# tusen-ai/MV2D

Hardware: AMD Instinct MI355X
Metric: multi-view samples/sec (6-cam frames) through the MV2D RoI-head hot path (higher is better)
Workload: dtype f16x3: every operand an fp16 hi + lo pair, three MFMAs per product, fp32 accumulation (fp32-class, index-exact route; the lo halves of the key / value rows are STORED as e4m3 bytes); 1 GPU; cfg2_s: MV2D-S head, 6 views 1408x512; global_batch=384, streams_per_gpu=4, samples_per_launch=16, pe_sine_branch=folded into a per-(weights, geometry) table, FLOPs not counted, parallelism=dp1, hipgraph=True

## Files before the change

include/mv2d_hip.h:

```cpp
#ifndef MV2D_HIP_H
#define MV2D_HIP_H
#ifdef __cplusplus
extern "C" {
#endif

const char* mv2d_last_error(void);
int mv2d_abi_version(void);
int mv2d_key16_format(void);
int mv2d_f32_to_key16(const float* x, void* hi, void* lo, long long n, void* stream);
int mv2d_device_arch(char* buf, int buflen);
int mv2d_spin(int usec, void* stream);


int mv2d_gemm_bf16(const void* A, const void* A2, int n_split, int a_mode, const void* W, const float* bias, int M, int N,
                   int K, int lda, const int* m_dev, int act, const float* mul, int ldmul, const float* add, int ldadd,
                   void* C, int c_bf16, int ldc, long long c_blk_stride, int c_blk_cols, void* C2, const float* add2,
                   int ldc2, int ldadd2, void* stream);
int mv2d_gemm_bf16_ex(const void* A, const void* A2, int n_split, int a_mode, const void* W, const float* bias, int M, int N, int K, int lda,
                      const int* m_dev, int act, const float* mul, int ldmul, const float* add, int ldadd, void* C, int c_bf16, int ldc,
                      long long c_blk_stride, int c_blk_cols, void* C2, const float* add2, int ldc2, int ldadd2, int c_split3, const int* add_idx , int add_period,
                      int k_splits , long long c_split_stride, void* stream);
int mv2d_split3_rows(const float* a, const float* b, void* out, int M, int cols, const int* m_dev, void* stream);

int mv2d_gemm_f32(const float* A, const float* A2, int n_split, const float* W, const float* bias, int M, int N, int K,
                  int lda, int ldw, int split_k, int act, float scale, float clamp, void* C, int c_bf16, int ldc,
                  long long c_slice_stride, int groups, long long a_gs, long long w_gs, long long b_gs, long long c_gs,
                  void* stream);

int mv2d_attn_out_fused(const float* ctx, const float* resid, const float* Wo, const float* bo, const float* ln_w, const float* ln_b,
                        float* x_out, const float* qpos, const float* Wq, const float* bq, float qscale, float* q_out, int M, float eps,
                        void* stream);

int mv2d_pe_fused_tab(const void* A1, const void* Xfb, const float* Xf32, const int* row_index, const int* m_dev, int M,
                      const void* W1a, const float* b1a, const void* W1b, const float* b1b,
                      const void* Wr, const float* br, const void* We, const float* be,
                      const float* sine_tab, int tab_period, float* pe, void* Xk, void* stream);
int mv2d_pe_fused_tab2(const void* A1, const void* Xfb, const float* Xf32, const int* row_index, const int* m_dev, int M,
                       const void* W1a, const float* b1a, const void* W1b, const float* b1b,
                       const void* Wr, const float* br, const void* We, const float* be,
                       const float* sine_tab, int tab_period, float* pe, void* Xk, int shape, void* stream);

int mv2d_pe_fused_tab_fmt(const void* A1, const void* Xfb, const void* Xf32, const int* row_index, const int* m_dev, int M,
                          const void* W1a, const float* b1a, const void* W1b, const float* b1b,
                          const void* Wr, const float* br, const void* We, const float* be,
                          const float* sine_tab, int tab_period, float* pe, void* Xk, int shape, int map_fmt, void* stream);

int mv2d_pe_fused_x3(const float* A1, const float* Xmap, const int* row_index, const int* m_dev, int M,
                     const void* W1a_hi, const void* W1a_lo, const float* b1a, const void* W1b_hi, const void* W1b_lo, const float* b1b,
                     const void* Wr_hi, const void* Wr_lo, const float* br, const void* We_hi, const void* We_lo, const float* be,
                     const float* sine_tab, int tab_period, float* pe, void* Xk_hi, void* Xk_lo, void* Xv_hi, void* Xv_lo, int lo_fmt, int pe_at_index,
                     int* lo8_flag, void* stream);
int mv2d_pe_fused_x3_fmt(const float* A1, const void* Xmap, const int* row_index, const int* m_dev, int M,
                         const void* W1a_hi, const void* W1a_lo, const float* b1a, const void* W1b_hi, const void* W1b_lo, const float* b1b,
                         const void* Wr_hi, const void* Wr_lo, const float* br, const void* We_hi, const void* We_lo, const float* be,
                         const float* sine_tab, int tab_period, float* pe, void* Xk_hi, void* Xk_lo, void* Xv_hi, void* Xv_lo, int lo_fmt, int pe_at_index,
                         int* lo8_flag, int map_fmt, void* stream);
int mv2d_pe_fused_x3_k(const float* A1, const void* Xmap, const int* row_index, const int* m_dev, int M,
                       const void* W1a_hi, const void* W1a_lo, const float* b1a, const void* W1b_hi, const void* W1b_lo, const float* b1b,
                       const void* Wr_hi, const void* Wr_lo, const float* br, const void* We_hi, const void* We_lo, const float* be,
                       const float* sine_tab, int tab_period, float* pe, void* Xk_hi, void* Xk_lo, void* Xv_hi, void* Xv_lo, int lo_fmt, int pe_at_index,
                       int* lo8_flag, int map_fmt, int Kp, void* stream);
int mv2d_pe_fused_x3_ng(const float* A1, const void* Xmap, const int* row_index, const int* m_dev, int M,
                        const void* W1a_hi, const void* W1a_lo, const float* b1a, const void* W1b_hi, const void* W1b_lo, const float* b1b,
                        const float* sine_tab, int tab_period, float* pe, void* Xk_hi, void* Xk_lo, void* Xv_hi, void* Xv_lo,
                        int lo_fmt, int pe_at_index, int* lo8_flag, int map_fmt, int Kp, void* stream);
int mv2d_pe_gate_x3(const float* Q, const void* Xmap, const int* row_index, const int* m_dev, int M,
                    const void* Wr_hi, const void* Wr_lo, const float* br, const void* We_hi, const void* We_lo, const float* be,
                    const float* sine_tab, int tab_period, float* pe, void* Xk_hi, void* Xk_lo, void* Xv_hi, void* Xv_lo, int pe_at_index,
                    int map_fmt, void* stream);
int mv2d_pe_gate_rows_x3(const float* Q, const void* Xmap, const int* row_index, const int* m_dev, int M,
                         const void* Wr_hi, const void* Wr_lo, const float* br, const void* We_hi, const void* We_lo, const float* be,
                         const float* sine_tab, int tab_period, float* pe, void* Xk_hi, void* Xk_lo, void* Xv_hi, void* Xv_lo, int lo_fmt,
                         int* lo8_flag, int map_fmt, const unsigned* view_mask, int hw, int take_set, void* stream);
int mv2d_pe_fused_x3_k_sel(const float* A1, const void* Xmap, const int* row_index, const int* m_dev, int M,
                           const void* W1a_hi, const void* W1a_lo, const float* b1a, const void* W1b_hi, const void* W1b_lo, const float* b1b,
                           const void* Wr_hi, const void* Wr_lo, const float* br, const void* We_hi, const void* We_lo, const float* be,
                           const float* sine_tab, int tab_period, float* pe, void* Xk_hi, void* Xk_lo, void* Xv_hi, void* Xv_lo, int lo_fmt,
                           int* lo8_flag, int map_fmt, int Kp, const unsigned* view_mask, int hw, int take_set, void* stream);
int mv2d_pe_fused_x3b(const float* A1, const float* Xmap, const int* row_index, const int* m_dev, int M,
                     const void* W1a_hi, const void* W1a_lo, const float* b1a, const void* W1b_hi, const void* W1b_lo, const float* b1b,
                     const void* Wr_hi, const void* Wr_lo, const float* br, const void* We_hi, const void* We_lo, const float* be,
                     const float* sine_tab, int tab_period, float* pe, void* Xk_hi, void* Xk_lo, void* Xv_hi, void* Xv_lo, int lo_fmt, int pe_at_index,
                     int* lo8_flag, void* stream);

int mv2d_pack_wfrag_bf16(const void* W, void* Wp, int N, int K, void* stream);
int mv2d_qg_conv_pool(const void* roi_feat, const void* W, const float* bias, float* out, int ld_out, int R, void* stream);
int mv2d_qg_conv_pool_x3(const void* roi_feat_hi, const void* roi_feat_lo, const void* W_hi, const void* W_lo, const float* bias, float* out,
                         int ld_out, int R, void* stream);
int mv2d_qg_conv_pool_s(const void* roi_feat, const void* W, const float* bias, float* out, int ld_out, int R, int roi_size, void* stream);
int mv2d_qg_conv_pool_x3_s(const void* roi_feat_hi, const void* roi_feat_lo, const void* W_hi, const void* W_lo, const float* bias, float* out,
                           int ld_out, int R, int roi_size, void* stream);

int mv2d_qg_conv_cells(const void* roi_feat, const void* W, const float* bias, void* out_hi, void* out_lo, float* out_f32, int R, int roi_size,
                       void* stream);
int mv2d_qg_conv_cells_x3(const void* roi_feat_hi, const void* roi_feat_lo, const void* W_hi, const void* W_lo, const float* bias, void* out_hi,
                          void* out_lo, float* out_f32, int R, int roi_size, void* stream);
int mv2d_avgpool_cells(const void* hi, const void* lo, float* out, int ld_out, int R, int cells, void* stream);

int mv2d_attn_out_fused_x3(const float* ctx, const float* resid, const void* Wo_hi, const void* Wo_lo, const float* bo,
                           const float* ln_w, const float* ln_b, float* x_out, const float* qpos, const void* Wq_hi,
                           const void* Wq_lo, const float* bq, float qscale, float* q_out, int M, float eps, void* stream);

int mv2d_sa_block_fused_x3(const float* qkv, const float* resid, const void* Wo_hi, const void* Wo_lo, const float* bo,
                           const float* ln_w, const float* ln_b, float* x_out, const float* qpos, const void* Wq_hi,
                           const void* Wq_lo, const float* bq, float qscale, float* q_out, int M, float eps, void* stream);

int mv2d_query_embed_fused_x3(const float* enc2, const float* Wc, const float* bc, const float* minv, const float* dim_t,
                              const float* pc_range, const void* W0_hi, const void* W0_lo, const float* b0, const void* W2_hi,
                              const void* W2_lo, const float* b2, float* center, float* xyz, float* ref, float* posemb,
                              float* qpos, int R, void* stream);

int mv2d_qg_tail_x3(const float* x2, const float* enc, int ld_enc, const void* fc_hi, const void* fc_lo, const float* fc_b,
                    const void* e0_hi, const void* e0_lo, const float* e0_b, const void* e2_hi, const void* e2_lo, const float* e2_b,
                    const float* Wc, const float* bc, const float* minv, const float* dim_t, const float* pc_range, const void* W0_hi,
                    const void* W0_lo, const float* b0, const void* W2_hi, const void* W2_lo, const float* b2, float* center, float* xyz,
                    float* ref, float* posemb, float* qpos, int R, void* stream);

int mv2d_ffn_out_fused_x3(const float* parts, int n_parts, long long part_stride, const float* b2, const float* resid,
                          const float* ln_w, const float* ln_b, const float* post_w, const float* post_b, float* x_out,
                          const float* qpos, float* xq_out, float* outs, const void* Win_hi, const void* Win_lo,
                          const float* b_in, float* qkv, int M, float eps, void* stream);

int mv2d_pack_wfrag_f32(const float* W, float* Wp, int N, int K, int ldw, void* stream);
int mv2d_heads_fused(const float* outs, const float* const* cls_w, const float* const* reg_w, const float* ref, float* cls, float* reg,
                     int M, int L, float eps, const float* pc_range, float dt, const float* dt_rows , void* stream);

int mv2d_linear_x3(const float* A, const float* A2, int n_split, int lda, const void* Whi, const void* Wlo, const float* bias,
                   float* C, int ldc, int M, int N, int K, int act, float clamp, int groups, long long a_gs, long long w_gs,
                   long long b_gs, long long c_gs, void* stream);
int mv2d_linear_x3_ex(const float* A, const float* A2, int n_split, int lda, const void* Whi, const void* Wlo, const float* bias,
                      float* C, int ldc, int M, int N, int K, int act, float clamp, int groups, long long a_gs, long long w_gs,
                      long long b_gs, long long c_gs, const int* m_dev, int conv3x3, const float* mul, const float* add, int ld_ma,
                      void* stream);
int mv2d_split_rows_key16(const float* a, const float* b, void* hi, void* lo, int M, int cols, const int* m_dev, void* stream);

int mv2d_heads_fused_x3(const float* outs, const void* const* cls_w, const void* const* reg_w, const float* ref, float* cls, float* reg,
                        int M, int L, float eps, const float* pc_range, float dt, const float* dt_rows, void* stream);
int mv2d_heads_fused_x3_nc(const float* outs, const void* const* cls_w, const void* const* reg_w, const float* ref, float* cls, float* reg,
                           int M, int L, int num_classes, float eps, const float* pc_range, float dt, const float* dt_rows, void* stream);
int mv2d_heads_cls_x3_nc(const float* outs, const void* const* cls_w, float* cls, int M, int L, int num_classes, float eps, void* stream);
int mv2d_reg_layer_x3(const float* outs, const void* const* w, const float* ref, float* reg, int M, int L, int n_groups, const int* group_dims,
                      const float* pc_range, float dt, const float* dt_rows, void* stream);

int mv2d_heads_depth_x3(const float* outs, const void* const* cls_w, const void* const* reg_w, const float* ref, float* cls, float* reg,
                        int M, int L, int n_fcs, int num_classes, float eps, const float* pc_range, float dt, const float* dt_rows, void* stream);
int mv2d_heads_cls_depth_x3(const float* outs, const void* const* cls_w, float* cls, int M, int L, int n_fcs, int num_classes, float eps,
                            void* stream);
int mv2d_reg_layer_depth_x3(const float* outs, const void* const* w, const float* ref, float* reg, int M, int L, int n_fcs, int n_groups,
                            const int* group_dims, const float* pc_range, float dt, const float* dt_rows, void* stream);

int mv2d_ffn_pack_weights(const float* W1, const float* W2, float* W1p, float* W2p, int hidden, void* stream);
int mv2d_ffn_fused(const float* X, const float* W1, const float* b1, const float* W2, float* slabs, int M, int hidden, void* stream);

int mv2d_ffn_fused_x3(const float* X, const void* W1hi, const void* W1lo, const float* b1, const void* W2hi, const void* W2lo,
                      float* slabs, int M, int hidden, int slices_per_block, void* stream);

int mv2d_split_bf16x2(const float* x, void* hi, void* lo, long long n, void* stream);
int mv2d_q16_format(void);
int mv2d_split_q16x2(const float* x, void* hi, void* lo, long long n, void* stream);


int mv2d_row_ln(const float* parts, int n_parts, long long part_stride, const float* bias, const float* residual,
                const float* ln_w, const float* ln_b, int relu, float* out, const float* addvec, float* out_plus,
                const float* ln2_w, const float* ln2_b, float* out2, int M, float eps, int rows_per_group, void* stream);

int mv2d_finalize_reg(float* reg, const float* ref, int L, int R, const float* pc_range, float dt, void* stream);

int mv2d_avgpool49(const float* x, float* out, int ld_out, int R, void* stream);

int mv2d_f32_to_bf16(const float* x, void* y, long long n, void* stream);

int mv2d_nchw_to_nhwc(const float* x, float* y, int V, int C, int HW, void* stream);
int mv2d_nchw_to_nhwc_masked(const float* x, float* y, const unsigned char* mask, int V, int C, int HW, void* stream);
int mv2d_nchw_to_nhwc_fmt(const void* x, void* y, int V, int C, int HW, int map_fmt, void* stream);
int mv2d_nchw_to_nhwc_masked_fmt(const void* x, void* y, const unsigned char* mask, int V, int C, int HW, int map_fmt, void* stream);

int mv2d_nchw_to_nhwc_bf16(const float* x, void* y, int V, int C, int HW, void* stream);
int mv2d_map_conv3x3(const void* in, const void* Wp, const float* bias, float* out, int V, int h, int w, void* stream);



int mv2d_self_attn_fwd(const float* qkv, float* ctx, int R, const int* grp_start, int n_samples, void* stream);

int mv2d_self_attn_x3_fwd(const float* qkv, float* ctx, int R, const int* grp_start, int n_samples, int max_grp_rows, int dn_pad,
                          int dn_single, void* stream);

int mv2d_self_attn_dn_fwd(const float* qkv, float* ctx, int R, int dn_pad, int dn_single, void* stream);

int mv2d_sparse_xattn_fwd(const float* q, const void* K, const void* V, const int* row_ptr, const int* col_idx, float* ctx,
                          float* dbg_logits, long long dbg_stride, int R, int empty_nan, void* stream);

int mv2d_xattn_qmap(const float* q, const void* WA_hi, const void* WA_lo, void* Qt, int R, void* stream);
int mv2d_xattn_tile_fwd(const void* Qt, const void* Xk, const void* Xv, const void* Xk_lo, const void* Xv_lo, const int* row_ptr,
                        const int* col_idx, float* z, float* dbg_logits, long long dbg_stride, int R, int empty_nan, int waves, void* stream);
int mv2d_xattn_tile_fwd_ordered(const void* Qt, const void* Xk, const void* Xv, const void* Xk_lo, const void* Xv_lo, const int* row_ptr,
                                const int* col_idx, float* z, float* dbg_logits, long long dbg_stride, int R, int empty_nan, int waves,
                                const int* order, int lo_fmt, void* stream);
int mv2d_xattn_fused_fwd(const float* q, const void* WA_hi, const void* WA_lo, const void* WB_hi, const void* WB_lo, const float* bv, const void* Xk,
                         const void* Xv, const void* Xk_lo, const void* Xv_lo, const int* row_ptr, const int* col_idx, float* ctx, int R, int empty_nan,
                         const int* order, int lo_fmt, void* stream);
int mv2d_xattn_fused_fwd_p(const float* q, const void* WA_hi, const void* WA_lo, const void* WB_hi, const void* WB_lo, const float* bv, const void* Xk,
                           const void* Xv, const void* Xk_lo, const void* Xv_lo, const int* row_ptr, const int* col_idx, float* ctx, int R, int empty_nan,
                           const int* order, int lo_fmt, int deal, void* stream);
int mv2d_xattn_group_max(int R, int n_samples);
int mv2d_xattn_group_tables(const int* row_ptr, const int* col_idx, const int* order, const int* grp_start, int n_samples, int R, int ng_max, int* g_slot,
                            int* g_cnt, int* g_ptr, int* g_len, int* ucol, unsigned char* umask, int ucap, int* u_total, int* flags, void* stream);
int mv2d_xattn_group_fwd(const float* q, const void* WA_hi, const void* WA_lo, const void* WB_hi, const void* WB_lo, const float* bv, const void* Xk,
                         const void* Xv, const void* Xk_lo, const void* Xv_lo, const int* row_ptr, const int* order, const int* g_slot, const int* g_cnt,
                         const int* g_ptr, const int* g_len, const int* ucol, const unsigned char* umask, float* ctx, int ng_max, int empty_nan,
                         void* stream);
int mv2d_xattn_ctxmap(const float* z, const void* WB_hi, const void* WB_lo, const float* bv, const int* row_ptr, float* ctx, int R,
                      int empty_nan, void* stream);

int mv2d_xattn_query_order(const int* row_ptr, const int* col_idx, const int* grp_start, int n_samples, int R, int* perm, int* flags, int stride,
                           void* stream);
int mv2d_attn_out_qmap_x3(const float* ctx, const float* resid, const void* Wo_hi, const void* Wo_lo, const float* bo, const float* ln_w,
                          const float* ln_b, float* x_out, const float* qpos, const void* Wq_hi, const void* Wq_lo, const float* bq,
                          float qscale, const void* WA_hi, const void* WA_lo, void* Qt, int M, float eps, void* stream);
int mv2d_attn_out_zmap_x3(const float* z, const void* WB_hi, const void* WB_lo, const float* bv, const int* row_ptr, int empty_nan,
                          const float* resid, const void* Wo_hi, const void* Wo_lo, const float* bo, const float* ln_w, const float* ln_b,
                          float* x_out, int M, float eps, void* stream);

int mv2d_sparse_xattn_bwd(const float* q, const void* K, const void* V, const int* row_ptr, const int* col_idx, const float* ctx,
                          const float* dctx, const int* key_ptr, const int* pair_idx, const int* pair_row, float* pair_ws,
                          float* dq, float* dK, float* dV, int R, int S, void* stream);
int mv2d_sparse_xattn_fwd_drop(const float* q, const void* K, const void* V, const int* row_ptr, const int* col_idx, float* ctx, float* dbg_logits,
                               long long dbg_stride, int R, int empty_nan, float p_drop, unsigned int seed, void* stream);
int mv2d_sparse_xattn_bwd_drop(const float* q, const void* K, const void* V, const int* row_ptr, const int* col_idx, const float* ctx,
                               const float* dctx, const int* key_ptr, const int* pair_idx, const int* pair_row, float* pair_ws, float* dq, float* dK,
                               float* dV, int R, int S, float p_drop, unsigned int seed, void* stream);
int mv2d_sparse_xattn_bwd_ex(const float* q, const void* K, const void* V, const int* row_ptr, const int* col_idx, const float* ctx, const float* dctx,
                             const int* key_ptr, const int* pair_idx, const int* pair_row, float* pair_ws, float* dq, float* dK, float* dV, int R,
                             int S, float p_drop, unsigned int seed, int long_rows, float dq_scale, void* stream);


int mv2d_box_params(const float* rois, const double* viewK, const double* viewE, double* K_roi, float* intr, int ld_intr,
                    float* minv, int R, float roi_size, float intr_scale, float min_size, void* stream);

int mv2d_refpoint_posemb(const float* center_pred, int ld_cp, const float* minv, const float* dim_t, float* xyz, float* ref,
                         float* posemb, int R, const float* pc_range, void* stream);

int mv2d_lidar2img_inverse(const double* K_roi, const double* E, float* minv, int R, void* stream);

int mv2d_posemb3d(const float* ref, const float* dim_t, float* posemb, int R, void* stream);

int mv2d_roi_align(const float* map0, const float* map1, const float* rois, void* out0, void* out1, float* out0_f32,
                   float* out1_f32, int R, int H, int W, int channels, float spatial_scale, int sampling_ratio,
                   const int* map1_index, int out1_is_sum, void* stream);
int mv2d_roi_align_ex(const float* map0, const float* map1, const float* rois, void* out0, void* out1, float* out0_f32, float* out1_f32,
                      int R, int H, int W, int channels, float spatial_scale, int sampling_ratio, const int* map1_index, int out1_is_sum,
                      void* out0_lo, void* out1_lo, void* out0_lo8, void* out1_lo8, int* lo8_flag, void* stream);
int mv2d_roi_align_s(const float* map0, const float* map1, const float* rois, void* out0, void* out1, float* out0_f32, float* out1_f32,
                     int R, int H, int W, int channels, float spatial_scale, int sampling_ratio, const int* map1_index, int out1_is_sum,
                     void* out0_lo, void* out1_lo, void* out0_lo8, void* out1_lo8, int* lo8_flag, int roi_size, void* stream);
int mv2d_roi_align_fmt(const void* map0, const float* map1, const float* rois, void* out0, void* out1, float* out0_f32, float* out1_f32,
                       int R, int H, int W, int channels, float spatial_scale, int sampling_ratio, const int* map1_index, int out1_is_sum,
                       void* out0_lo, void* out1_lo, void* out0_lo8, void* out1_lo8, int* lo8_flag, int roi_size, int map_fmt, void* stream);

int mv2d_box_correlation(const float* rois, const int* view_start, const double* trans, const float* lin, const float* depths,
                         int* match, int R, int V, int sample_size, int num_depth, int topk, int pad_h, int pad_w,
                         float depth_start, float iou_thr, float ratio, int max_per_view, void* stream);
int mv2d_frame_geometry(const float* rois, const double* viewK, const double* viewE, double* K_roi, float* intr, int ld_intr, float* minv,
                        float roi_size, float intr_scale, float min_size, const int* view_start, const double* trans, const float* lin,
                        const float* depths, int* match, int R, int V, int sample_size, int num_depth, int topk, int pad_h, int pad_w,
                        float depth_start, float iou_thr, float ratio, int max_per_view, void* zero_ptr, long long zero_bytes, void* stream);
int mv2d_box_correlation_ex(const float* rois, const int* view_start, const double* trans, const float* lin, const float* depths,
                            int* match, int R, int V, int sample_size, int num_depth, int topk, int pad_h, int pad_w,
                            double depth_start, float iou_thr, float ratio, int max_per_view, void* stream);
int mv2d_frame_geometry_ex(const float* rois, const double* viewK, const double* viewE, double* K_roi, float* intr, int ld_intr, float* minv,
                           float roi_size, float intr_scale, float min_size, const int* view_start, const double* trans, const float* lin,
                           const float* depths, int* match, int R, int V, int sample_size, int num_depth, int topk, int pad_h, int pad_w,
                           double depth_start, float iou_thr, float ratio, int max_per_view, void* zero_ptr, long long zero_bytes, void* stream);

long long mv2d_csr_workspace_bytes(int R, int V, int h, int w);

int mv2d_mask_compact(const float* rois, const int* match, const unsigned char* pad_mask, unsigned char* roi_mask, int* rect,
                      int* pos2s, int* s2pos, int* S_out, unsigned int* bits_ws, int* row_count, int* row_ptr, int* col_idx,
                      int* nnz_out, int col_cap, int R, int V, int h, int w, int topk, float stride, float expand_stride,
                      int n_samples , void* stream);

int mv2d_roi_positions(const float* rois, const unsigned char* pad_mask, unsigned char* roi_mask, int* rect, int* pos2s,
                       int* s2pos, int* S_out, int R, int V, int h, int w, float stride, float expand_stride, void* stream);

int mv2d_csr_from_corr(const int* match, int* row_ptr, int* col_idx, int* nnz_out, int R, int V, int topk, void* stream);
int mv2d_roi_positions_csr(const float* rois, const unsigned char* pad_mask, unsigned char* roi_mask, int* rect, int* pos2s, int* s2pos,
                           int* S_out, int R, int V, int h, int w, float stride, float expand_stride, const int* match, int* row_ptr,
                           int* col_idx, int* nnz_out, int Vg, int topk, const int* grp_start, int n_samples, int* order, int* order_flags, void* stream);
int mv2d_csr_from_corr_s(const int* match, int* row_ptr, int* col_idx, int* nnz_out, int R, int V, int topk, int roi_size, void* stream);
int mv2d_roi_positions_csr_s(const float* rois, const unsigned char* pad_mask, unsigned char* roi_mask, int* rect, int* pos2s, int* s2pos,
                             int* S_out, int R, int V, int h, int w, float stride, float expand_stride, const int* match, int* row_ptr,
                             int* col_idx, int* nnz_out, int Vg, int topk, const int* grp_start, int n_samples, int* order, int* order_flags,
                             int roi_size, void* stream);

int mv2d_pe_frustum_f32(const int* s2pos, const int* S_dev, int S_max, const double* img2lidar, const double* coords_w, const double* coords_h,
                        const double* coords_d, float* out, int V, int h, int w, int depth_num, const double* position_range, void* stream);
int mv2d_pe_frustum_f32_ld(const int* s2pos, const int* S_dev, int S_max, const double* img2lidar, const double* coords_w, const double* coords_h,
                           const double* coords_d, float* out, int V, int h, int w, int depth_num, const double* position_range, int ld, void* stream);
int mv2d_pe_frustum_f32_sel(const int* s2pos, const int* S_dev, int S_max, const double* img2lidar, const double* coords_w, const double* coords_h,
                            const double* coords_d, float* out, int V, int h, int w, int depth_num, const double* position_range, int ld,
                            const unsigned* view_mask, int tab_period, void* stream);

int mv2d_pe_inputs(const int* s2pos, const int* S_dev, int S_max, const float* featcl, const double* img2lidar,
                   const double* coords_w, const double* coords_h, const double* coords_d, const float* embeds,
                   const float* dim_t, void* A_frustum, void* A_sine, void* Xf_k16, float* Xf_f32, float* A_frustum_f32,
                   float* A_sine_f32, int V, int h, int w, int depth_num, const double* position_range, void* stream);
int mv2d_pe_inputs_fmt(const int* s2pos, const int* S_dev, int S_max, const void* featcl, const double* img2lidar,
                       const double* coords_w, const double* coords_h, const double* coords_d, const float* embeds,
                       const float* dim_t, void* A_frustum, void* A_sine, void* Xf_k16, float* Xf_f32, float* A_frustum_f32,
                       float* A_sine_f32, int V, int h, int w, int depth_num, const double* position_range, int map_fmt, void* stream);
int mv2d_pe_inputs_ld(const int* s2pos, const int* S_dev, int S_max, const void* featcl, const double* img2lidar,
                      const double* coords_w, const double* coords_h, const double* coords_d, const float* embeds,
                      const float* dim_t, void* A_frustum, void* A_sine, void* Xf_k16, float* Xf_f32, float* A_frustum_f32,
                      float* A_sine_f32, int V, int h, int w, int depth_num, const double* position_range, int map_fmt, int ld, void* stream);

int mv2d_decode_topk(const float* cls, const float* reg, int R, int num_classes, int max_num, const float* post_center_range,
                     float* boxes, float* scores, long long* labels, long long* bbox_index, int* count_out,
                     long long* topk_index_dbg, const int* grp_start, int n_samples, int max_grp_rows, float* payload, void* stream);

int mv2d_nms_bev(const float* boxes, const float* scores, const long long* labels, const int* count, float nms_thr, float* scores_out,
                 int n_samples, int in_stride, void* stream);

int mv2d_result_pack(const float* boxes, const float* scores, const long long* labels, const int* count, float score_thr, int max_num,
                     float* out_boxes, float* out_scores, long long* out_labels, int* out_count,
                     int n_samples , int in_stride,
                     void* stream);

int mv2d_pack_detections(const float* boxes, const float* scores, const long long* labels, const int* count, float* out, int n_samples,
                         int max_num, int in_stride, void* stream);

int mv2d_match_cost(const float* cls, const float* box, const float* gt, const int* gt_labels, float* cost, int n_layers, int R, int G,
                    int C, float cls_weight, float reg_weight, float alpha, float gamma, void* stream);

int mv2d_set_loss(const float* cls, const float* box, const int* match, const float* gt, const int* gt_labels, const float* code_weights,
                  const float* layer_weights, float* loss, float* dcls, float* dbox, int n_layers, int R, int G, int C,
                  float cls_avg_factor, float box_avg_factor, float alpha, float gamma, float loss_cls_weight, float loss_bbox_weight,
                  int skip_background_boxes, void* stream);

int mv2d_dn_queries(const float* gt, const int* gt_labels, const float* rnd, int G, int scalar, float noise_scale, float noise_trans, float split,
                    int num_classes, const float* pc_range_host, float eps, float* ref, long long* labels, float* boxes, void* stream);

int mv2d_colsum_scratch_rows(int rows);
int mv2d_colsum(const float* x, long long ld, int rows, int cols, float* out, float* scratch, void* stream);
int mv2d_layer_norm_bwd_blocks(int M);
int mv2d_layer_norm_bwd(const float* x, const float* dy, const float* w, float* dx, float* dw_part, float* db_part, float* dw, float* db, int M,
                        float eps, void* stream);
long long mv2d_gemm_f32x3_ws_bytes(int M, int N, int K);
int mv2d_gemm_f32x3(const float* A, long long lda, int trans_a, const float* B, long long ldb, int trans_b, const float* bias, int act, float* C,
                    long long ldc, int M, int N, int K, void* ws, long long ws_bytes, void* stream);
long long mv2d_linear_bwd_x3_ws_bytes(int M, int N, int K);
int mv2d_linear_bwd_x3(const float* x, const float* W, const float* y, const float* dy, float* dx, float* dW, float* db, int M, int N, int K, void* ws,
                       long long ws_bytes, void* stream);

int mv2d_gemm_f32x3_ex(const float* A, long long lda, int trans_a, const float* B, long long ldb, int trans_b, const float* bias, int act, float alpha,
                       int accumulate, int out_bf16, void* C, long long ldc, int M, int N, int K, void* ws, long long ws_bytes, void* stream);
int mv2d_colsum_add(const float* x, long long ld, int rows, int cols, float* out, float* scratch, const float* add, void* stream);
int mv2d_softmax_bwd_rows(const float* P, const float* Pd, float* dP, long long ld, int rows, int cols, float keep_scale, void* stream);
long long mv2d_gemm_f32x3_batched_ws_bytes(int M, int N, int K, int batch);
int mv2d_gemm_f32x3_batched(const float* A, long long lda, long long batch_a, int trans_a, const float* B, long long ldb, long long batch_b, int trans_b,
                            float* C, long long ldc, long long batch_c, int M, int N, int K, int batch, float alpha, void* ws, long long ws_bytes,
                            void* stream);
int mv2d_dgrad_relu_f32x3(const float* g, const float* W, const float* relu_y, float alpha, float* dx, int M, int N, int K, void* stream);
int mv2d_wgrad_f32x3(const float* g, const float* x, float* dW, float* db, int M, int N, int K, void* ws, long long ws_bytes, float* cs_scratch,
                     void* stream);

typedef struct mv2d_td_dims {
    int T, S, L, F;
    int sa_nnz, ca_nnz;
    float p_sa_attn, p_sa_out, p_ca_attn, p_ca_out, p_ffn_act, p_ffn_out;
    unsigned int seed;
    float eps;
    int pad, nk;
} mv2d_td_dims;
long long mv2d_train_decoder_act_bytes(const mv2d_td_dims* d);
long long mv2d_train_decoder_ws_bytes(const mv2d_td_dims* d, int backward);
int mv2d_train_decoder_fwd(const mv2d_td_dims* d, const float* const* params, const float* qpos, const float* key_in, const float* val_in,
                           const int* sa_row_ptr, const int* sa_col, const int* ca_row_ptr, const int* ca_col, const int* dn_keys, float* outs, void* act,
                           void* ws, void* stream);
int mv2d_train_decoder_bwd(const mv2d_td_dims* d, const float* const* params, float* const* grads, const float* qpos, const float* key_in,
                           const float* val_in, const int* sa_row_ptr, const int* sa_col, const int* sa_key_ptr, const int* sa_pair_idx,
                           const int* sa_pair_row, const int* ca_row_ptr, const int* ca_col, const int* ca_key_ptr, const int* ca_pair_idx,
                           const int* ca_pair_row, const int* dn_keys, const float* d_outs, const void* act, void* ws, float* d_qpos, float* d_key_in,
                           float* d_val_in, void* stream);

typedef struct mv2d_th_dims { int T, L, NC; float eps; } mv2d_th_dims;
long long mv2d_train_heads_act_bytes(const mv2d_th_dims* d);
long long mv2d_train_heads_ws_bytes(const mv2d_th_dims* d, int backward);
int mv2d_train_heads_fwd(const mv2d_th_dims* d, const float* const* params, const float* outs, float* cls, float* reg, void* act, void* ws,
                         void* stream);
int mv2d_train_heads_bwd(const mv2d_th_dims* d, const float* const* params, float* const* grads, const float* outs, const float* d_cls,
                         const float* d_reg, const void* act, void* ws, float* d_outs, void* stream);

int mv2d_box_code_fwd(const float* t, const float* ref, float* out, int L, int T, int pad, float dt, const float* pc_range, void* stream);
int mv2d_box_code_bwd(const float* g, const float* out, const float* ref, float* d_t, float* d_ref, int L, int T, int pad, float dt,
                      const float* pc_range, void* stream);

int mv2d_lsap_layers(const float* cost, int L, int R, int G, int* match, int threads);

int mv2d_im2col3x3(const float* x, float* cols, int R, void* stream);
int mv2d_col2im3x3(const float* dcols, float* dx, int R, void* stream);
int mv2d_im2col3x3_s(const float* x, float* cols, int R, int roi_size, void* stream);
int mv2d_col2im3x3_s(const float* dcols, float* dx, int R, int roi_size, void* stream);

int mv2d_center2lidar_fwd(const float* c, const float* minv, float* ref, int R, const float* pc_range, void* stream);
int mv2d_center2lidar_bwd(const float* g, const float* c, const float* minv, float* dc, int R, const float* pc_range, void* stream);

long long mv2d_dense_attn_ws_bytes(int n, int nk, int backward);
int mv2d_dense_attn_fwd(const float* q, const float* k, const float* v, int n, int nk, float p_drop, unsigned int seed, float* ctx, float* lse, void* ws,
                        void* stream);
int mv2d_dense_attn_bwd(const float* q, const float* k, const float* v, const float* ctx, const float* dctx, const float* lse, int n, int nk, float p_drop,
                        unsigned int seed, float dq_scale, float* dq, float* dk, float* dv, void* ws, void* stream);
int mv2d_dense_attn_bwd_parts(const float* q, const float* k, const float* v, const float* ctx, const float* dctx, const float* lse, int n, int nk,
                              float p_drop, unsigned int seed, float dq_scale, float* dq, float* dk, float* dv, void* ws, int parts, void* stream);

int mv2d_roi_align_bwd(const float* grad_out, const float* rois, float* grad_map, const int* index, int R, int H, int W, int channels,
                       float spatial_scale, int sampling_ratio, void* stream);
int mv2d_roi_align_bwd_s(const float* grad_out, const float* rois, float* grad_map, const int* index, int R, int H, int W, int channels,
                         float spatial_scale, int sampling_ratio, int roi_size, void* stream);

#ifdef __cplusplus
}
#endif
#endif
```

mv2d_amd/_lib.py:

```python
import ctypes as C
import os

HERE = os.path.dirname(os.path.abspath(__file__))
LIB_PATH = os.path.join(HERE, 'lib', 'libmv2d_hip.so')


class Mv2dHipError(RuntimeError):
    pass


P, I, LL, F, D = C.c_void_p, C.c_int, C.c_longlong, C.c_float, C.c_double
ABI_VERSION = 6

class TdDims(C.Structure):
    _fields_ = [('T', I), ('S', I), ('L', I), ('F', I), ('sa_nnz', I), ('ca_nnz', I), ('p_sa_attn', F), ('p_sa_out', F), ('p_ca_attn', F),
                ('p_ca_out', F), ('p_ffn_act', F), ('p_ffn_out', F), ('seed', C.c_uint), ('eps', F), ('pad', I), ('nk', I)]


class ThDims(C.Structure):
    _fields_ = [('T', I), ('L', I), ('NC', I), ('eps', F)]


SIGNATURES = {
    'mv2d_last_error': (C.c_char_p, []),
    'mv2d_abi_version': (I, []),
    'mv2d_device_arch': (I, [C.c_char_p, I]),
    'mv2d_spin': (I, [I, P]),
    'mv2d_gemm_bf16': (I, [P, P, I, I, P, P, I, I, I, I, P, I, P, I, P, I, P, I, I, LL, I, P, P, I, I, P]),
    'mv2d_gemm_bf16_ex': (I, [P, P, I, I, P, P, I, I, I, I, P, I, P, I, P, I, P, I, I, LL, I, P, P, I, I, I, P, I, I, LL, P]),
    'mv2d_split3_rows': (I, [P, P, P, I, I, P, P]),
    'mv2d_pe_fused_tab': (I, [P, P, P, P, P, I] + [P] * 9 + [I, P, P, P]),
    'mv2d_pe_fused_tab2': (I, [P, P, P, P, P, I] + [P] * 9 + [I, P, P, I, P]),
    'mv2d_pe_fused_x3': (I, [P, P, P, P, I] + [P] * 13 + [I] + [P] * 5 + [I, I, P, P]),
    'mv2d_pe_fused_tab_fmt': (I, [P, P, P, P, P, I] + [P] * 9 + [I, P, P, I, I, P]),
    'mv2d_pe_fused_x3_fmt': (I, [P, P, P, P, I] + [P] * 13 + [I] + [P] * 5 + [I, I, P, I, P]),
    'mv2d_pe_fused_x3_k': (I, [P, P, P, P, I] + [P] * 13 + [I] + [P] * 5 + [I, I, P, I, I, P]),
    'mv2d_pe_fused_x3_ng': (I, [P, P, P, P, I] + [P] * 7 + [I] + [P] * 5 + [I, I, P, I, I, P]),
    'mv2d_pe_gate_x3': (I, [P, P, P, P, I] + [P] * 7 + [I] + [P] * 5 + [I, I, P]),
    'mv2d_pe_gate_rows_x3': (I, [P, P, P, P, I] + [P] * 7 + [I] + [P] * 5 + [I, P, I, P, I, I, P]),
    'mv2d_pe_fused_x3_k_sel': (I, [P, P, P, P, I] + [P] * 13 + [I] + [P] * 5 + [I, P, I, I, P, I, I, P]),
    'mv2d_pe_fused_x3b': (I, [P, P, P, P, I] + [P] * 13 + [I] + [P] * 5 + [I, I, P, P]),
    'mv2d_key16_format': (I, []),
    'mv2d_f32_to_key16': (I, [P, P, P, LL, P]),
    'mv2d_split_rows_key16': (I, [P, P, P, P, I, I, P, P]),
    'mv2d_qg_conv_pool': (I, [P, P, P, P, I, I, P]),
    'mv2d_qg_conv_pool_x3': (I, [P, P, P, P, P, P, I, I, P]),
    'mv2d_qg_conv_pool_s': (I, [P, P, P, P, I, I, I, P]),
    'mv2d_qg_conv_pool_x3_s': (I, [P, P, P, P, P, P, I, I, I, P]),
    'mv2d_qg_conv_cells': (I, [P, P, P, P, P, P, I, I, P]),
    'mv2d_qg_conv_cells_x3': (I, [P, P, P, P, P, P, P, P, I, I, P]),
    'mv2d_avgpool_cells': (I, [P, P, P, I, I, I, P]),
    'mv2d_pack_wfrag_bf16': (I, [P, P, I, I, P]),
    'mv2d_gemm_f32': (I, [P, P, I, P, P, I, I, I, I, I, I, I, F, F, P, I, I, LL, I, LL, LL, LL, LL, P]),
    'mv2d_attn_out_fused': (I, [P, P, P, P, P, P, P, P, P, P, F, P, I, F, P]),
    'mv2d_sa_block_fused_x3': (I, [P, P, P, P, P, P, P, P, P, P, P, P, F, P, I, F, P]),
    'mv2d_query_embed_fused_x3': (I, [P] * 17 + [I, P]),
    'mv2d_qg_tail_x3': (I, [P, P, I] + [P] * 25 + [I, P]),
    'mv2d_ffn_out_fused_x3': (I, [P, I, LL, P, P, P, P, P, P, P, P, P, P, P, P, P, P, I, F, P]),
    'mv2d_attn_out_fused_x3': (I, [P, P, P, P, P, P, P, P, P, P, P, P, F, P, I, F, P]),
    'mv2d_pack_wfrag_f32': (I, [P, P, I, I, I, P]),
    'mv2d_heads_fused': (I, [P, P, P, P, P, P, I, I, F, P, F, P, P]),
    'mv2d_linear_x3': (I, [P, P, I, I, P, P, P, P, I, I, I, I, I, F, I, LL, LL, LL, LL, P]),
    'mv2d_linear_x3_ex': (I, [P, P, I, I, P, P, P, P, I, I, I, I, I, F, I, LL, LL, LL, LL, P, I, P, P, I, P]),
    'mv2d_heads_fused_x3': (I, [P, P, P, P, P, P, I, I, F, P, F, P, P]),
    'mv2d_heads_fused_x3_nc': (I, [P, P, P, P, P, P, I, I, I, F, P, F, P, P]),
    'mv2d_heads_cls_x3_nc': (I, [P, P, P, I, I, I, F, P]),
    'mv2d_reg_layer_x3': (I, [P, P, P, P, I, I, I, P, P, F, P, P]),
    'mv2d_heads_depth_x3': (I, [P, P, P, P, P, P, I, I, I, I, F, P, F, P, P]),
    'mv2d_heads_cls_depth_x3': (I, [P, P, P, I, I, I, I, F, P]),
    'mv2d_reg_layer_depth_x3': (I, [P, P, P, P, I, I, I, I, P, P, F, P, P]),
    'mv2d_ffn_fused': (I, [P, P, P, P, P, I, I, P]),
    'mv2d_ffn_pack_weights': (I, [P, P, P, P, I, P]),
    'mv2d_ffn_fused_x3': (I, [P, P, P, P, P, P, P, I, I, I, P]),
    'mv2d_split_bf16x2': (I, [P, P, P, LL, P]),
    'mv2d_split_q16x2': (I, [P, P, P, LL, P]),
    'mv2d_q16_format': (I, []),
    'mv2d_row_ln': (I, [P, I, LL, P, P, P, P, I, P, P, P, P, P, P, I, F, I, P]),
    'mv2d_finalize_reg': (I, [P, P, I, I, P, F, P]),
    'mv2d_avgpool49': (I, [P, P, I, I, P]),
    'mv2d_f32_to_bf16': (I, [P, P, LL, P]),
    'mv2d_nchw_to_nhwc': (I, [P, P, I, I, I, P]),
    'mv2d_nchw_to_nhwc_masked': (I, [P, P, P, I, I, I, P]),
    'mv2d_nchw_to_nhwc_fmt': (I, [P, P, I, I, I, I, P]),
    'mv2d_nchw_to_nhwc_masked_fmt': (I, [P, P, P, I, I, I, I, P]),
    'mv2d_nchw_to_nhwc_bf16': (I, [P, P, I, I, I, P]),
    'mv2d_map_conv3x3': (I, [P, P, P, P, I, I, I, P]),
    'mv2d_self_attn_fwd': (I, [P, P, I, P, I, P]),
    'mv2d_self_attn_dn_fwd': (I, [P, P, I, I, I, P]),
    'mv2d_self_attn_x3_fwd': (I, [P, P, I, P, I, I, I, I, P]),
    'mv2d_dn_queries': (I, [P, P, P, I, I, F, F, F, I, P, F, P, P, P, P]),
    'mv2d_sparse_xattn_fwd': (I, [P, P, P, P, P, P, P, LL, I, I, P]),
    'mv2d_sparse_xattn_bwd': (I, [P] * 14 + [I, I, P]),
    'mv2d_sparse_xattn_fwd_drop': (I, [P, P, P, P, P, P, P, LL, I, I, F, C.c_uint, P]),
    'mv2d_sparse_xattn_bwd_drop': (I, [P] * 14 + [I, I, F, C.c_uint, P]),
    'mv2d_sparse_xattn_bwd_ex': (I, [P] * 14 + [I, I, F, C.c_uint, I, F, P]),
    'mv2d_dgrad_relu_f32x3': (I, [P, P, P, F, P, I, I, I, P]),
    'mv2d_xattn_qmap': (I, [P, P, P, P, I, P]),
    'mv2d_attn_out_qmap_x3': (I, [P] * 12 + [F, P, P, P, I, F, P]),
    'mv2d_attn_out_zmap_x3': (I, [P, P, P, P, P, I, P, P, P, P, P, P, P, I, F, P]),
    'mv2d_xattn_tile_fwd': (I, [P, P, P, P, P, P, P, P, P, LL, I, I, I, P]),
    'mv2d_xattn_tile_fwd_ordered': (I, [P, P, P, P, P, P, P, P, P, LL, I, I, I, P, I, P]),
    'mv2d_xattn_fused_fwd': (I, [P, P, P, P, P, P, P, P, P, P, P, P, P, I, I, P, I, P]),
    'mv2d_xattn_fused_fwd_p': (I, [P, P, P, P, P, P, P, P, P, P, P, P, P, I, I, P, I, I, P]),
    'mv2d_xattn_group_max': (I, [I, I]),
    'mv2d_xattn_group_tables': (I, [P, P, P, P, I, I, I, P, P, P, P, P, P, I, P, P, P]),
    'mv2d_xattn_group_fwd': (I, [P] * 19 + [I, I, P]),
    'mv2d_xattn_query_order': (I, [P, P, P, I, I, P, P, I, P]),
    'mv2d_xattn_ctxmap': (I, [P, P, P, P, P, P, I, I, P]),
    'mv2d_box_params': (I, [P, P, P, P, P, I, P, I, F, F, F, P]),
    'mv2d_refpoint_posemb': (I, [P, I, P, P, P, P, P, I, P, P]),
    'mv2d_lidar2img_inverse': (I, [P, P, P, I, P]),
    'mv2d_posemb3d': (I, [P, P, P, I, P]),
    'mv2d_roi_align': (I, [P, P, P, P, P, P, P, I, I, I, I, F, I, P, I, P]),
    'mv2d_roi_align_ex': (I, [P, P, P, P, P, P, P, I, I, I, I, F, I, P, I, P, P, P, P, P, P]),
    'mv2d_roi_align_s': (I, [P, P, P, P, P, P, P, I, I, I, I, F, I, P, I, P, P, P, P, P, I, P]),
    'mv2d_roi_align_fmt': (I, [P, P, P, P, P, P, P, I, I, I, I, F, I, P, I, P, P, P, P, P, I, I, P]),
    'mv2d_box_correlation': (I, [P, P, P, P, P, P, I, I, I, I, I, I, I, F, F, F, I, P]),
    'mv2d_box_correlation_ex': (I, [P, P, P, P, P, P, I, I, I, I, I, I, I, D, F, F, I, P]),
    'mv2d_csr_workspace_bytes': (LL, [I, I, I, I]),
    'mv2d_mask_compact': (I, [P, P, P, P, P, P, P, P, P, P, P, P, P, I, I, I, I, I, I, F, F, I, P]),
    'mv2d_roi_positions': (I, [P, P, P, P, P, P, P, I, I, I, I, F, F, P]),
    'mv2d_csr_from_corr': (I, [P, P, P, P, I, I, I, P]),
    'mv2d_csr_from_corr_s': (I, [P, P, P, P, I, I, I, I, P]),
    'mv2d_roi_positions_csr': (I, [P, P, P, P, P, P, P, I, I, I, I, F, F, P, P, P, P, I, I, P, I, P, P, P]),
    'mv2d_roi_positions_csr_s': (I, [P, P, P, P, P, P, P, I, I, I, I, F, F, P, P, P, P, I, I, P, I, P, P, I, P]),
    'mv2d_frame_geometry': (I, [P, P, P, P, P, I, P, F, F, F, P, P, P, P, P, I, I, I, I, I, I, I, F, F, F, I, P, LL, P]),
    'mv2d_frame_geometry_ex': (I, [P, P, P, P, P, I, P, F, F, F, P, P, P, P, P, I, I, I, I, I, I, I, D, F, F, I, P, LL, P]),
    'mv2d_pe_inputs': (I, [P, P, I, P, P, P, P, P, P, P, P, P, P, P, P, P, I, I, I, I, P, P]),
    'mv2d_pe_inputs_fmt': (I, [P, P, I, P, P, P, P, P, P, P, P, P, P, P, P, P, I, I, I, I, P, I, P]),
    'mv2d_pe_frustum_f32': (I, [P, P, I, P, P, P, P, P, I, I, I, I, P, P]),
    'mv2d_pe_frustum_f32_ld': (I, [P, P, I, P, P, P, P, P, I, I, I, I, P, I, P]),
    'mv2d_pe_frustum_f32_sel': (I, [P, P, I, P, P, P, P, P, I, I, I, I, P, I, P, I, P]),
    'mv2d_pe_inputs_ld': (I, [P, P, I, P, P, P, P, P, P, P, P, P, P, P, P, P, I, I, I, I, P, I, I, P]),
    'mv2d_result_pack': (I, [P, P, P, P, F, I, P, P, P, P, I, I, P]),
    'mv2d_nms_bev': (I, [P, P, P, P, F, P, I, I, P]),
    'mv2d_pack_detections': (I, [P, P, P, P, P, I, I, I, P]),
    'mv2d_roi_align_bwd': (I, [P, P, P, P, I, I, I, I, F, I, P]),
    'mv2d_roi_align_bwd_s': (I, [P, P, P, P, I, I, I, I, F, I, I, P]),
    'mv2d_colsum_scratch_rows': (I, [I]),
    'mv2d_colsum': (I, [P, LL, I, I, P, P, P]),
    'mv2d_gemm_f32x3_ws_bytes': (LL, [I, I, I]),
    'mv2d_gemm_f32x3': (I, [P, LL, I, P, LL, I, P, I, P, LL, I, I, I, P, LL, P]),
    'mv2d_gemm_f32x3_ex': (I, [P, LL, I, P, LL, I, P, I, F, I, I, P, LL, I, I, I, P, LL, P]),
    'mv2d_colsum_add': (I, [P, LL, I, I, P, P, P, P]),
    'mv2d_softmax_bwd_rows': (I, [P, P, P, LL, I, I, F, P]),
    'mv2d_gemm_f32x3_batched_ws_bytes': (LL, [I, I, I, I]),
    'mv2d_gemm_f32x3_batched': (I, [P, LL, LL, I, P, LL, LL, I, P, LL, LL, I, I, I, I, F, P, LL, P]),
    'mv2d_wgrad_f32x3': (I, [P, P, P, P, I, I, I, P, LL, P, P]),
    'mv2d_train_decoder_act_bytes': (LL, [P]),
    'mv2d_train_decoder_ws_bytes': (LL, [P, I]),
    'mv2d_train_decoder_fwd': (I, [P] * 14),
    'mv2d_train_decoder_bwd': (I, [P] * 24),
    'mv2d_box_code_fwd': (I, [P, P, P, I, I, I, F, P, P]),
    'mv2d_box_code_bwd': (I, [P, P, P, P, P, I, I, I, F, P, P]),
    'mv2d_im2col3x3': (I, [P, P, I, P]),
    'mv2d_col2im3x3': (I, [P, P, I, P]),
    'mv2d_im2col3x3_s': (I, [P, P, I, I, P]),
    'mv2d_col2im3x3_s': (I, [P, P, I, I, P]),
    'mv2d_center2lidar_fwd': (I, [P, P, P, I, P, P]),
    'mv2d_center2lidar_bwd': (I, [P, P, P, P, I, P, P]),
    'mv2d_dense_attn_ws_bytes': (LL, [I, I, I]),
    'mv2d_dense_attn_fwd': (I, [P, P, P, I, I, F, C.c_uint, P, P, P, P]),
    'mv2d_dense_attn_bwd': (I, [P, P, P, P, P, P, I, I, F, C.c_uint, F, P, P, P, P, P]),
    'mv2d_dense_attn_bwd_parts': (I, [P, P, P, P, P, P, I, I, F, C.c_uint, F, P, P, P, P, I, P]),
    'mv2d_lsap_layers': (I, [P, I, I, I, P, I]),
    'mv2d_train_heads_act_bytes': (LL, [P]),
    'mv2d_train_heads_ws_bytes': (LL, [P, I]),
    'mv2d_train_heads_fwd': (I, [P] * 8),
    'mv2d_train_heads_bwd': (I, [P] * 10),
    'mv2d_linear_bwd_x3_ws_bytes': (LL, [I, I, I]),
    'mv2d_linear_bwd_x3': (I, [P, P, P, P, P, P, P, I, I, I, P, LL, P]),
    'mv2d_layer_norm_bwd_blocks': (I, [I]),
    'mv2d_layer_norm_bwd': (I, [P, P, P, P, P, P, P, P, I, F, P]),
    'mv2d_match_cost': (I, [P, P, P, P, P, I, I, I, I, F, F, F, F, P]),
    'mv2d_set_loss': (I, [P, P, P, P, P, P, P, P, P, P, I, I, I, I, F, F, F, F, F, F, I, P]),
    'mv2d_decode_topk': (I, [P, P, I, I, I, P, P, P, P, P, P, P, P, I, I, P, P]),
}

_lib = None


def load(path=None):
    global _lib
    if _lib is not None:
        return _lib
    path = path or os.environ.get('MV2D_HIP_LIB', LIB_PATH)
    if not os.path.exists(path):
        raise Mv2dHipError(
            f'{path} not found: the MV2D HIP extension is not built.  Run `python -m mv2d_amd.build` '
            '(or __graft_entry__.build()).  There is no CPU/PyTorch fallback for the product path.')
    lib = C.CDLL(path)
    for name, (res, args) in SIGNATURES.items():
        fn = getattr(lib, name, None)
        if fn is None:
            raise Mv2dHipError(f'{path} does not export {name}; rebuild with `python -m mv2d_amd.build --force`')
        fn.restype = res
        fn.argtypes = args
    if lib.mv2d_abi_version() != ABI_VERSION:
        raise Mv2dHipError(f'{path} implements ABI version {lib.mv2d_abi_version()}, this package needs {ABI_VERSION}: rebuild with `python -m mv2d_amd.build --force`')
    _lib = lib
    return lib


def check(rc, what):
    if rc != 0:
        msg = load().mv2d_last_error()
        raise Mv2dHipError(f'{what} failed (rc={rc}): {msg.decode() if msg else ""}')
```

mv2d_amd/csrc/xattn_fused.hip:

```cpp
#include "xattn_walk.h"
#include <stdlib.h>
#ifndef MV2D_XF_QB_DEFAULT
#define MV2D_XF_QB_DEFAULT 8
#endif
enum { XF_DEAL_ROUNDS = 1, XF_DEAL_FULL = 2 };
#ifndef MV2D_XF_DEAL_DEFAULT
#define MV2D_XF_DEAL_DEFAULT XF_DEAL_FULL
#endif
constexpr int XF_DEAL_DEFAULT = MV2D_XF_DEAL_DEFAULT;

#ifdef MV2D_XF_TRACE
__device__ long long g_xf_trace[32];
#define XF_STAMP(i) do { if (blockIdx.x == MV2D_XF_TRACE && threadIdx.x == 0) g_xf_trace[i] = (long long)__builtin_amdgcn_s_memtime(); } while (0)
#else
#define XF_STAMP(i) do {} while (0)
#endif

namespace {

constexpr int WAVE_LDS = 16384;

template <int XLO, int QB>
__global__ __launch_bounds__(64 * QB, 2) void xattn_fused_kernel(const float* __restrict__ q, const uint4* __restrict__ WA_hi, const uint4* __restrict__ WA_lo,
                                                                const uint4* __restrict__ WB_hi, const uint4* __restrict__ WB_lo, const float* __restrict__ bv,
                                                                const unsigned short* __restrict__ Xk, const unsigned short* __restrict__ Xv,
                                                                const unsigned short* __restrict__ Xk_lo, const unsigned short* __restrict__ Xv_lo,
                                                                const int* __restrict__ row_ptr, const int* __restrict__ col_idx, float* __restrict__ ctx,
                                                                int R, int empty_nan, const int* __restrict__ order, int nblk) {
    constexpr int SMEM = QB * WAVE_LDS + QB * 512 + QB * HEADS * 4 + 3 * QB * 4;
    __shared__ __attribute__((aligned(16))) unsigned char smem[SMEM];
    const int tid = threadIdx.x, lane = tid & 63, wave = tid >> 6, n = lane & 15, g = lane >> 4;
    float* lsum = reinterpret_cast<float*>(smem + QB * WAVE_LDS + QB * 512);
    int* rq = reinterpret_cast<int*>(smem + QB * WAVE_LDS + QB * 512 + QB * HEADS * 4);
    int* rbeg = rq + QB;
    int* rend = rq + 2 * QB;
    const int blk = xcd_chunked(blockIdx.x, nblk);
    const int slot0 = (int)((long long)blk * R / nblk), nq = (int)((long long)(blk + 1) * R / nblk) - slot0;
    if (nq <= 0) return;
    XF_STAMP(0);
    if (tid < QB) {
        const int s = slot0 + min(tid, nq - 1);
        const int r_ = order ? order[s] : s;
        rq[tid] = r_;
        rbeg[tid] = row_ptr[r_];
        rend[tid] = row_ptr[r_ + 1];
    }
    __syncthreads();
    XF_STAMP(1);
    const int beg = rbeg[wave], end = rend[wave];
    const int ntile = wave < nq ? (end - beg + 15) >> 4 : 0;
    int idx_next = ntile > 0 ? col_idx[min(beg + n, end - 1)] : 0;
    typedef XattnWalk<XLO, false> Walk;
    Walk walk(Xk, Xv, Xk_lo, Xv_lo, lane, beg, end, reinterpret_cast<uint4*>(smem + wave * WAVE_LDS), reinterpret_cast<uint4*>(smem + wave * WAVE_LDS) + 512,
           reinterpret_cast<float*>(smem + QB * WAVE_LDS) + wave * 128);
    typename Walk::KRows k0;
    for (int h = wave; h < HEADS; h += QB) {
        const int r = rq[n & (QB - 1)];
        const float* qp = q + (long long)r * C + 32 * h + 8 * g;
        const float4 q0 = *reinterpret_cast<const float4*>(qp), q1 = *reinterpret_cast<const float4*>(qp + 4);
        const uint4* wh = WA_hi + (long long)h * 16 * 64 + lane;
        const uint4* wl = WA_lo + (long long)h * 16 * 64 + lane;
        uint4* qt = reinterpret_cast<uint4*>(smem + (n & (QB - 1)) * WAVE_LDS) + h * 64;
        u32x4 wa_h[16], wa_l[16];
#pragma unroll
        for (int t = 0; t < 16; ++t) {
            wa_h[t] = *reinterpret_cast<const u32x4*>(wh + t * 64);
            wa_l[t] = *reinterpret_cast<const u32x4*>(wl + t * 64);
        }
        __builtin_amdgcn_sched_barrier(0);
        XF_STAMP(20);
        Frag bh, bl;
        split8(q0, q1, bh, bl);
#pragma unroll
        for (int u = 0; u < 8; ++u) {
            if (u == 1) XF_STAMP(21);
            if (u == 4) XF_STAMP(22);
            f32x4_t a[2];
#pragma unroll
            for (int k = 0; k < 2; ++k) {
                f32x4_t c = {0.f, 0.f, 0.f, 0.f};
                c = mfma_q16_16x16x32(wa_l[2 * u + k], bh.v, c);
                c = mfma_q16_16x16x32(wa_h[2 * u + k], bl.v, c);
                c = mfma_q16_16x16x32(wa_h[2 * u + k], bh.v, c);
                a[k] = c;
            }
            Frag hi, lo;
            split8_k16(make_float4(a[0][0], a[0][1], a[0][2], a[0][3]), make_float4(a[1][0], a[1][1], a[1][2], a[1][3]), hi, lo);
            if (n < QB) {
                qt[u * 8 + g * 2] = hi.u;
                qt[u * 8 + g * 2 + 1] = lo.u;
            }
            if (u == (XLO ? 5 : 3) && h == wave && ntile > 0) walk.request_k(idx_next, k0);
        }
    }
    XF_STAMP(23);
    asm volatile("s_waitcnt lgkmcnt(0)" ::: "memory");
    __builtin_amdgcn_s_barrier();
    XF_STAMP(2);
    {
        const uint4* qp = reinterpret_cast<const uint4*>(smem + wave * WAVE_LDS) + (n & 7) * 64 + g * 2 + (n >> 3);
#pragma unroll
        for (int s = 0; s < 8; ++s) walk.qa[s].u = qp[s * 8];
    }
    walk.reset();
    if (ntile > 0) walk.stage_k(k0);
#pragma nounroll
    for (int tt = 0; tt < ntile; ++tt) {
        const int myidx = idx_next;
        if (tt + 1 < ntile) idx_next = col_idx[min(beg + 16 * (tt + 1) + n, end - 1)];
        typename Walk::VRows v;
        walk.gather(myidx, tt > 0, v);
        XF_STAMP(3 + 2 * min(tt, 5));
        walk.compute(tt, v);
        XF_STAMP(4 + 2 * min(tt, 5));
    }
    walk.row_sums();
    if (n == 0 && g < 2) {
#pragma unroll
        for (int i = 0; i < 4; ++i) lsum[wave * HEADS + 4 * g + i] = walk.l_run[i];
    }
    walk.store_z(reinterpret_cast<float*>(smem + wave * WAVE_LDS));
    XF_STAMP(15);
    __syncthreads();
    XF_STAMP(16);
    for (int h = wave; h < HEADS; h += QB) {
        const int j = n & (QB - 1);
        const float* zp = reinterpret_cast<const float*>(smem + j * WAVE_LDS) + h * C + 8 * g;
        const float rl = __builtin_amdgcn_rcpf(lsum[j * HEADS + h]);
        const uint4* wh = WB_hi + (long long)h * 16 * 64 + lane;
        const uint4* wl = WB_lo + (long long)h * 16 * 64 + lane;
        f32x4_t acc[2] = {{0.f, 0.f, 0.f, 0.f}, {0.f, 0.f, 0.f, 0.f}};
        u32x4 wb_h[16], wb_l[16];
#pragma unroll
        for (int t = 0; t < 16; ++t) {
            wb_h[t] = *reinterpret_cast<const u32x4*>(wh + t * 64);
            wb_l[t] = *reinterpret_cast<const u32x4*>(wl + t * 64);
        }
        int rr_[4], rp0_[4], rp1_[4];
#pragma unroll
        for (int i = 0; i < 4; ++i) {
            rr_[i] = rq[(4 * g + i) & (QB - 1)];
            rp0_[i] = rbeg[(4 * g + i) & (QB - 1)];
            rp1_[i] = rend[(4 * g + i) & (QB - 1)];
        }
        const float bv0 = bv[32 * h + n], bv1 = bv[32 * h + 16 + n];
        __builtin_amdgcn_sched_barrier(0);
#pragma unroll
        for (int s = 0; s < 8; ++s) {
            float4 x0 = *reinterpret_cast<const float4*>(zp + 32 * s);
            float4 x1 = *reinterpret_cast<const float4*>(zp + 32 * s + 4);
            x0 = make_float4(x0.x * rl, x0.y * rl, x0.z * rl, x0.w * rl);
            x1 = make_float4(x1.x * rl, x1.y * rl, x1.z * rl, x1.w * rl);
            Frag ah, al;
            split8(x0, x1, ah, al);
#pragma unroll
            for (int nt = 0; nt < 2; ++nt) {
                acc[nt] = mfma_q16_16x16x32(al.v, wb_h[s * 2 + nt], acc[nt]);
                acc[nt] = mfma_q16_16x16x32(ah.v, wb_l[s * 2 + nt], acc[nt]);
                acc[nt] = mfma_q16_16x16x32(ah.v, wb_h[s * 2 + nt], acc[nt]);
            }
        }
        if (4 * g < QB) {
#pragma unroll
            for (int i = 0; i < 4; ++i) {
                const int js = 4 * g + i;
                if (js < nq) {
                    const int rr = rr_[i];
                    const bool empty = rp1_[i] <= rp0_[i];
#pragma unroll
                    for (int nt = 0; nt < 2; ++nt) {
                        const int col = 32 * h + 16 * nt + n;
                        float v = acc[nt][i] + (nt ? bv1 : bv0);
                        if (empty) v = empty_nan ? __uint_as_float(0x7fc00000u) : 0.f;
                        ctx[(long long)rr * C + col] = v;
                    }
                }
            }
        }
    }
    XF_STAMP(17);
}

}

#ifdef MV2D_XF_TRACE
extern "C" int mv2d_xf_trace_read(long long* host, int n) { return hipMemcpyFromSymbol(host, HIP_SYMBOL(g_xf_trace), n * sizeof(long long)) == hipSuccess ? 0 : -2; }
#endif

extern "C" int mv2d_xattn_fused_fwd_p(const float* q, const void* WA_hi, const void* WA_lo, const void* WB_hi, const void* WB_lo, const float* bv,
                                      const void* Xk, const void* Xv, const void* Xk_lo, const void* Xv_lo, const int* row_ptr, const int* col_idx,
                                      float* ctx, int R, int empty_nan, const int* order, int lo_fmt, int deal, void* stream) {
    MV2D_CHECK_ARG(deal >= 0 && deal <= 2, "mv2d_xattn_fused_fwd_p: deal is 0 (default), 1 (whole rounds) or 2 (full blocks)");
    MV2D_CHECK_ARG(lo_fmt == 0 || (lo_fmt == 1 && Xk_lo), "mv2d_xattn_fused_fwd: lo_fmt is 0 (key16 lo rows) or 1 (e4m3 lo rows; needs the lo rows)");
    MV2D_CHECK_ARG(q && WA_hi && WA_lo && WB_hi && WB_lo && bv && Xk && Xv && row_ptr && col_idx && ctx && R >= 0, "mv2d_xattn_fused_fwd: bad args");
    MV2D_CHECK_ARG((Xk_lo == nullptr) == (Xv_lo == nullptr), "mv2d_xattn_fused_fwd: Xk_lo and Xv_lo come together");
    MV2D_CHECK_ARG(((uintptr_t)q & 15) == 0 && ((uintptr_t)WA_hi & 15) == 0 && ((uintptr_t)WA_lo & 15) == 0 && ((uintptr_t)WB_hi & 15) == 0 &&
                       ((uintptr_t)WB_lo & 15) == 0 && ((uintptr_t)Xk & 15) == 0 && ((uintptr_t)Xv & 15) == 0 && ((uintptr_t)Xk_lo & 15) == 0 &&
                       ((uintptr_t)Xv_lo & 15) == 0, "mv2d_xattn_fused_fwd: operands must be 16-byte aligned");
    if (R == 0) return MV2D_OK;
    static int n_cu = 0;
    if (n_cu == 0) {
        hipDeviceProp_t prop;
        int dev = 0;
        n_cu = (hipGetDevice(&dev) == hipSuccess && hipGetDeviceProperties(&prop, dev) == hipSuccess && prop.multiProcessorCount > 0) ? prop.multiProcessorCount : 256;
    }
    static const int qb_env = [] { const char* e = getenv("MV2D_XF_QB"); return e ? atoi(e) : 0; }();
    const int QB = qb_env == 4 || qb_env == 8 ? qb_env : MV2D_XF_QB_DEFAULT;
    const int slots = n_cu * (QB == 4 ? 2 : 1);
    int nblk = (R + QB - 1) / QB;
    if (nblk > slots) {
        static const int deal_env = [] { const char* e = getenv("MV2D_XF_DEAL"); return e ? atoi(e) : 0; }();
        const int policy = deal ? deal : (deal_env == XF_DEAL_ROUNDS || deal_env == XF_DEAL_FULL ? deal_env : XF_DEAL_DEFAULT);
        if (policy == XF_DEAL_ROUNDS) {
            const int up = (nblk + slots - 1) / slots * slots;
            if ((long long)up * (QB / 2) <= R) nblk = up;
        }
    } else {
        const int spread = R / 2 < n_cu ? R / 2 : n_cu;
        if (spread > nblk) nblk = spread;
    }
    const dim3 grid(nblk), block(64 * QB);
#define MV2D_XF(XLO_, QB_) hipLaunchKernelGGL((xattn_fused_kernel<XLO_, QB_>), grid, block, 0, (hipStream_t)stream, q, (const uint4*)WA_hi, (const uint4*)WA_lo, \
                                              (const uint4*)WB_hi, (const uint4*)WB_lo, bv, (const unsigned short*)Xk, (const unsigned short*)Xv,                     \
                                              (const unsigned short*)Xk_lo, (const unsigned short*)Xv_lo, row_ptr, col_idx, ctx, R, empty_nan, order, nblk)
    if (Xk_lo && lo_fmt == 1) { if (QB == 4) MV2D_XF(2, 4); else MV2D_XF(2, 8); }
    else if (Xk_lo) { if (QB == 4) MV2D_XF(1, 4); else MV2D_XF(1, 8); }
    else { if (QB == 4) MV2D_XF(0, 4); else MV2D_XF(0, 8); }
#undef MV2D_XF
    MV2D_LAUNCH_CHECK();
    return MV2D_OK;
}

extern "C" int mv2d_xattn_fused_fwd(const float* q, const void* WA_hi, const void* WA_lo, const void* WB_hi, const void* WB_lo, const float* bv,
                                    const void* Xk, const void* Xv, const void* Xk_lo, const void* Xv_lo, const int* row_ptr, const int* col_idx,
                                    float* ctx, int R, int empty_nan, const int* order, int lo_fmt, void* stream) {
    return mv2d_xattn_fused_fwd_p(q, WA_hi, WA_lo, WB_hi, WB_lo, bv, Xk, Xv, Xk_lo, Xv_lo, row_ptr, col_idx, ctx, R, empty_nan, order, lo_fmt, 0, stream);
}
```

mv2d_amd/csrc/xattn_walk.h:

```cpp
#pragma once
#include "common.h"
#include <type_traits>

namespace {

constexpr int C = 256, HEADS = 8;
constexpr float LOG2E = 1.4426950408889634f;

typedef q16x8_t q16x8;
union Frag { uint4 u; q16x8 v; };
typedef unsigned int u32x4 __attribute__((ext_vector_type(4)));
typedef unsigned int u32x2 __attribute__((ext_vector_type(2)));

__device__ __forceinline__ void split8(const float4& x0, const float4& x1, Frag& hi, Frag& lo) {
    const float f[8] = {x0.x, x0.y, x0.z, x0.w, x1.x, x1.y, x1.z, x1.w};
    unsigned int h[4], l[4];
#pragma unroll
    for (int i = 0; i < 4; ++i) split_q16x2(f[2 * i], f[2 * i + 1], h[i], l[i]);
    hi.u = make_uint4(h[0], h[1], h[2], h[3]);
    lo.u = make_uint4(l[0], l[1], l[2], l[3]);
}
__device__ __forceinline__ void split8_k16(const float4& x0, const float4& x1, Frag& hi, Frag& lo) {
    const float f[8] = {x0.x, x0.y, x0.z, x0.w, x1.x, x1.y, x1.z, x1.w};
    unsigned int h[4], l[4];
#pragma unroll
    for (int i = 0; i < 4; ++i) split_k16x2(f[2 * i], f[2 * i + 1], h[i], l[i]);
    hi.u = make_uint4(h[0], h[1], h[2], h[3]);
    lo.u = make_uint4(l[0], l[1], l[2], l[3]);
}

__device__ __forceinline__ unsigned int lo_pair(unsigned int a, unsigned int b) { return __builtin_amdgcn_perm(b, a, 0x05040100u); }
__device__ __forceinline__ unsigned int hi_pair(unsigned int a, unsigned int b) { return __builtin_amdgcn_perm(b, a, 0x07060302u); }

#define XATTN_DPP(v, ctrl) __uint_as_float((unsigned)__builtin_amdgcn_update_dpp(0, (int)__float_as_uint(v), ctrl, 0xF, 0xF, true))
__device__ __forceinline__ float row16_max(float v) {
    v = fmaxf(v, XATTN_DPP(v, 0xB1));
    v = fmaxf(v, XATTN_DPP(v, 0x4E));
    v = fmaxf(v, XATTN_DPP(v, 0x141));
    v = fmaxf(v, XATTN_DPP(v, 0x140));
    return v;
}

template <int XLO, bool DBG>
struct XattnWalk {
    typedef std::conditional_t<XLO == 2, u32x2, u32x4> lo_t;
    struct KRows { u32x4 hi[8]; lo_t lo[XLO ? 8 : 1]; };
    struct VRows { u32x4 hi[4][2]; lo_t lo[XLO ? 4 : 1][2]; };

    const unsigned short *Xk, *Xv, *Xk_lo, *Xv_lo;
    int lane, n, g, beg, end;
    uint4 *kt, *kt2;
    float* pl;
    float* dbg_logits;
    long long dbg_stride;
    Frag qa[8];
    float m_run[4], l_run[4];
    f32x4_t Z[16];

    __device__ __forceinline__ XattnWalk(const unsigned short* Xk_, const unsigned short* Xv_, const unsigned short* Xk_lo_, const unsigned short* Xv_lo_,
                                         int lane_, int beg_, int end_, uint4* kt_, uint4* kt2_, float* pl_, float* dbg_logits_ = nullptr,
                                         long long dbg_stride_ = 0)
        : Xk(Xk_), Xv(Xv_), Xk_lo(Xk_lo_), Xv_lo(Xv_lo_), lane(lane_), n(lane_ & 15), g(lane_ >> 4), beg(beg_), end(end_), kt(kt_), kt2(kt2_), pl(pl_),
          dbg_logits(dbg_logits_), dbg_stride(dbg_stride_) {}

    __device__ __forceinline__ void reset() {
#pragma unroll
        for (int i = 0; i < 4; ++i) { m_run[i] = -INFINITY; l_run[i] = 0.f; }
#pragma unroll
        for (int u = 0; u < 16; ++u) Z[u] = f32x4_t{0.f, 0.f, 0.f, 0.f};
    }

    __device__ __forceinline__ void load_v(const unsigned short* V_, int myidx, u32x4 (&dst)[4][2]) const {
#pragma unroll
        for (int e = 0; e < 4; ++e) {
            const unsigned int vidx = (unsigned int)__shfl(myidx, 4 * g + e, 64);
            const char* vp = reinterpret_cast<const char*>(V_) + ((vidx << 9) + 16u * (unsigned)n);
            dst[e][0] = *reinterpret_cast<const u32x4*>(vp);
            dst[e][1] = *reinterpret_cast<const u32x4*>(vp + 256);
        }
    }
    __device__ __forceinline__ void load_k(const unsigned short* K_, int myidx, u32x4 (&dst)[8]) const {
#pragma unroll
        for (int i = 0; i < 8; ++i) {
            const unsigned int ridx = (unsigned int)__shfl(myidx, 2 * i + (lane >> 5), 64);
            dst[i] = *reinterpret_cast<const u32x4*>(reinterpret_cast<const char*>(K_) + ((ridx << 9) + (unsigned)(lane & 31) * 16u));
        }
    }
    __device__ __forceinline__ void store_k(uint4* tile, const u32x4 (&src)[8]) const {
#pragma unroll
        for (int i = 0; i < 8; ++i) {
            const int rowi = 2 * i + (lane >> 5);
            reinterpret_cast<u32x4*>(tile)[rowi * 32 + ((lane & 31) ^ (rowi & 15))] = src[i];
        }
    }
    __device__ __forceinline__ void load_v8(const unsigned short* V_, int myidx, u32x2 (&dst)[4][2]) const {
#pragma unroll
        for (int e = 0; e < 4; ++e) {
            const unsigned int vidx = (unsigned int)__shfl(myidx, 4 * g + e, 64);
            const char* vp = reinterpret_cast<const char*>(V_) + ((vidx << 8) + 8u * (unsigned)n);
            dst[e][0] = *reinterpret_cast<const u32x2*>(vp);
            dst[e][1] = *reinterpret_cast<const u32x2*>(vp + 128);
        }
    }
    __device__ __forceinline__ void load_k8(const unsigned short* K_, int myidx, u32x2 (&dst)[8]) const {
#pragma unroll
        for (int i = 0; i < 8; ++i) {
            const unsigned int ridx = (unsigned int)__shfl(myidx, 2 * i + (lane >> 5), 64);
            dst[i] = *reinterpret_cast<const u32x2*>(reinterpret_cast<const char*>(K_) + ((ridx << 8) + (unsigned)(lane & 31) * 8u));
        }
    }
    __device__ __forceinline__ void store_k8(uint4* tile, const u32x2 (&src)[8]) const {
#pragma unroll
        for (int i = 0; i < 8; ++i) {
            const int rowi = 2 * i + (lane >> 5);
            tile[rowi * 32 + ((lane & 31) ^ (rowi & 15))] = lo8_chunk(make_uint2(src[i].x, src[i].y));
        }
    }
    __device__ __forceinline__ void request_k(int myidx, KRows& k) const {
        load_k(Xk, myidx, k.hi);
        if constexpr (XLO == 1) load_k(Xk_lo, myidx, k.lo);
        if constexpr (XLO == 2) load_k8(Xk_lo, myidx, k.lo);
    }
    __device__ __forceinline__ void stage_k(const KRows& k) const {
        store_k(kt, k.hi);
        if constexpr (XLO == 1) store_k(kt2, k.lo);
        if constexpr (XLO == 2) store_k8(kt2, k.lo);
    }
    __device__ __forceinline__ void request_v(int myidx, VRows& v) const {
        load_v(Xv, myidx, v.hi);
        if constexpr (XLO == 1) load_v(Xv_lo, myidx, v.lo);
        if constexpr (XLO == 2) load_v8(Xv_lo, myidx, v.lo);
    }

    __device__ __forceinline__ void gather(int myidx, bool with_k, VRows& v) const {
        if constexpr (XLO != 0) {
            if (with_k) {
                KRows k;
                request_k(myidx, k);
                stage_k(k);
            }
            request_v(myidx, v);
        } else if (with_k) {
            KRows k;
            request_k(myidx, k);
            request_v(myidx, v);
            stage_k(k);
        } else {
            request_v(myidx, v);
        }
        __builtin_amdgcn_wave_barrier();
    }

    __device__ __forceinline__ void compute(int tt, const VRows& v) {
        const int kbase = beg + 16 * tt;
        f32x4_t sacc = {0.f, 0.f, 0.f, 0.f};
#pragma unroll
        for (int s = 0; s < 8; ++s) {
            Frag kb;
            kb.u = kt[n * 32 + ((4 * s + g) ^ n)];
            sacc = mfma_k16_16x16x32(qa[s].u, kb.u, sacc);
            if (XLO) {
                Frag kl, qh;
                kl.u = kt2[n * 32 + ((4 * s + g) ^ n)];
                qh.u = n < 8 ? qa[s].u : make_uint4(0u, 0u, 0u, 0u);
                sacc = mfma_k16_16x16x32(qh.u, kl.u, sacc);
            }
        }
        const bool valid = kbase + n < end;
        float sv[4], p[4], alpha[4];
#pragma unroll
        for (int i = 0; i < 4; ++i) {
            const auto sw = __builtin_amdgcn_permlane32_swap(__float_as_uint(sacc[i]), __float_as_uint(sacc[i]), false, false);
            const float full = __uint_as_float(sw[0]) + __uint_as_float(sw[1]);
            if (DBG && dbg_logits && g < 2 && valid) dbg_logits[(long long)(4 * g + i) * dbg_stride + kbase + n] = full;
            sv[i] = valid ? full * LOG2E : -INFINITY;
        }
#pragma unroll
        for (int i = 0; i < 4; ++i) {
            float tm = sv[i];
            tm = row16_max(tm);
            const float m_new = fmaxf(m_run[i], tm);
            alpha[i] = __builtin_amdgcn_exp2f(m_run[i] - m_new);
            p[i] = __builtin_amdgcn_exp2f(sv[i] - m_new);
            l_run[i] = l_run[i] * alpha[i] + p[i];
            m_run[i] = m_new;
        }
        if (g < 2) {
#pragma unroll
            for (int i = 0; i < 4; ++i) pl[(4 * g + i) * 16 + n] = p[i];
        }
        __builtin_amdgcn_wave_barrier();
        uint2 pa, pah;
        {
            const float4 pv = *reinterpret_cast<const float4*>(pl + (n & 7) * 16 + 4 * g);
            unsigned int h0, h1, l0, l1;
            split_k16x2_bounded(pv.x, pv.y, h0, l0);
            split_k16x2_bounded(pv.z, pv.w, h1, l1);
            pa = n < 8 ? make_uint2(h0, h1) : make_uint2(l0, l1);
            pah = n < 8 ? make_uint2(h0, h1) : make_uint2(0u, 0u);
        }
#pragma unroll
        for (int u = 0; u < 16; ++u)
#pragma unroll
            for (int i = 0; i < 4; ++i) Z[u][i] *= alpha[i];
#pragma unroll
        for (int H = 0; H < 2; ++H) {
            const unsigned int r0[4] = {v.hi[0][H].x, v.hi[0][H].y, v.hi[0][H].z, v.hi[0][H].w};
            const unsigned int r1[4] = {v.hi[1][H].x, v.hi[1][H].y, v.hi[1][H].z, v.hi[1][H].w};
            const unsigned int r2[4] = {v.hi[2][H].x, v.hi[2][H].y, v.hi[2][H].z, v.hi[2][H].w};
            const unsigned int r3[4] = {v.hi[3][H].x, v.hi[3][H].y, v.hi[3][H].z, v.hi[3][H].w};
#pragma unroll
            for (int w = 0; w < 8; ++w) {
                const int d = w >> 1;
                const uint2 vb = (w & 1) ? make_uint2(hi_pair(r0[d], r1[d]), hi_pair(r2[d], r3[d]))
                                         : make_uint2(lo_pair(r0[d], r1[d]), lo_pair(r2[d], r3[d]));
                f32x4_t zc = Z[H * 8 + w];
                zc = mfma_k16_16x16x16(pa, vb, zc);
                if constexpr (XLO != 0) {
                    auto lo_pair_of = [&](int e) -> unsigned int {
                        if constexpr (XLO == 2) {
                            const unsigned int b = v.lo[e][H][d >> 1];
                            return (d & 1) ? lo8_pair<1>(b) : lo8_pair<0>(b);
                        } else {
                            return v.lo[e][H][d];
                        }
                    };
                    const unsigned int q0 = lo_pair_of(0), q1 = lo_pair_of(1), q2 = lo_pair_of(2), q3 = lo_pair_of(3);
                    const uint2 vl = (w & 1) ? make_uint2(hi_pair(q0, q1), hi_pair(q2, q3)) : make_uint2(lo_pair(q0, q1), lo_pair(q2, q3));
                    zc = mfma_k16_16x16x16(pah, vl, zc);
                }
                Z[H * 8 + w] = zc;
            }
        }
        __builtin_amdgcn_wave_barrier();
    }

    __device__ __forceinline__ void row_sums() {
#pragma unroll
        for (int i = 0; i < 4; ++i) {
            float l = l_run[i];
            l += __shfl_xor(l, 1, 64);
            l += __shfl_xor(l, 2, 64);
            l += __shfl_xor(l, 4, 64);
            l += __shfl_xor(l, 8, 64);
            l_run[i] = l;
        }
    }
    __device__ __forceinline__ void store_z(float* szw) const {
#pragma unroll
        for (int H = 0; H < 2; ++H)
#pragma unroll
            for (int i = 0; i < 4; ++i) {
                float v[4];
#pragma unroll
                for (int w = 0; w < 4; ++w) {
                    const auto sw = __builtin_amdgcn_permlane32_swap(__float_as_uint(Z[H * 8 + w][i]), __float_as_uint(Z[H * 8 + w + 4][i]), false, false);
                    v[w] = __uint_as_float(sw[0]) + __uint_as_float(sw[1]);
                }
                float* dst = szw + (4 * (g & 1) + i) * C + 128 * H + 8 * n + 4 * (g >> 1);
                *reinterpret_cast<float4*>(dst) = make_float4(v[0], v[1], v[2], v[3]);
            }
    }
};

}
```

mv2d_amd/engine.py:

```python
import math
import os

import numpy as np
import torch

from . import calib, ops, pe_cache, qg_shape, route

BF16 = torch.bfloat16
F32 = torch.float32
C = 256
L_DEFAULT = 6


def _t(x, device, dtype=None):
    if isinstance(x, np.ndarray):
        x = torch.from_numpy(np.ascontiguousarray(x))
    x = x.detach()
    if dtype is not None:
        x = x.to(dtype)
    return x.to(device).contiguous()


def native_map(feat):
    return feat if feat.dtype in ops.MAP_FMT else feat.float()
# ... 593 lines not shown
            ev = torch.cuda.Event(enable_timing=True)
            ev.record()
            self.prof.setdefault(name, []).append(ev)

    def _enqueue(self, ws, feat, R, V, h, w, sc):
        o, W_, rt = ops, self.w, ws['route']
        P, L, T = ws['P'], self.L, ws['tab']
        B, Vg = ws['B'], ws['Vg']
        grp = ws['grp_start']
        tk = self._tick
        tk('h2d')
        rois = ws['rois']
        forked = rt.forked
        masked = (rt.masked and (rt.kind == 'S' or self.expand >= 1.0) and (h * w) % 4 == 0 and not (torch.is_tensor(feat) and feat.is_contiguous(memory_format=torch.channels_last) and not feat.is_contiguous()))

        def transpose(mask):
            if isinstance(feat, (list, tuple)):
                fcl, Pg = ws['featcl'], P // B
                for b_, f in enumerate(feat):
                    o.nchw_to_nhwc(f, fcl[b_ * Pg:(b_ + 1) * Pg], mask=None if mask is None else mask[b_ * Pg:(b_ + 1) * Pg])
                return fcl
            if feat.is_contiguous(memory_format=torch.channels_last) and not feat.is_contiguous():
                return feat.permute(0, 2, 3, 1).reshape(P, C)
            return o.nchw_to_nhwc(feat, ws['featcl'], mask=mask)
        tk('transpose')
        featcl = ws['featcl'] if masked else transpose(None)
        ws['featcl_cur'], ws['map_shape'], ws['max_rows'] = featcl, (V, h, w), sc['max_rows']
        ws['feat_in'], ws['featcl_masked'] = feat, masked
        tk('box_params'); tk('box_corr')
        o.frame_geometry(rois, T['viewK'], T['viewE'], ws['intr'], ws['ld_intr'], ws['minv'], ws['view_start'], T['trans'], self.const['lin'],
                         self.const['depths'], ws['match'], Vg, self.topk, sc['pad_h'], sc['pad_w'], sc['max_per_view'], iou_thr=self.iou_thr,
                         ratio=self.ratio, zero=ws['zbuf'], roi_size=float(self.roi_size), intr_scale=self.intrins_feat_scale,
                         sample_size=self.sample_size, num_depth=self.num_depth, depth_start=self.corr_depth_start)
        tk('csr')
        if forked:
            side = ws.get('side_stream')
            if side is None:
                side = ws['side_stream'] = torch.cuda.Stream(device=self.dev)
            side.wait_stream(torch.cuda.current_stream())
            with torch.cuda.stream(side):
                o.roi_align(featcl, rois, h, w, out0=ws['roi_feat'], R=R, roi_size=self.roi_size)
                self._enqueue_qg(ws, R)
        order = ws['q_order']
        if rt.kind == 'T':
            o.mask_compact(rois, ws['match'], T['pad_mask'], ws['roi_mask'], ws['rect'], ws['pos2s'], ws['s2pos'], ws['S_dev'],
                           ws['bits'], ws['row_count'], ws['row_ptr'], ws['col_idx'], ws['nnz'], R, Vg, h, w, self.topk,
                           self.stride, self.expand, col_cap=ws['col_cap'], n_samples=B)
            if rt.q_order:
                o.xattn_query_order(ws['row_ptr'], ws['col_idx'], grp, R, order, ws['qt_ctl'][1:])
        else:
            if rt.force_nc is not None:
                fm = ws.get('forced_match')
                if fm is None or fm.shape != ws['match'].shape:
                    assert rt.force_nc - 1 <= Vg * self.topk, 'raise corr_topk for this n_c'
                    fmh = torch.full((R, Vg * self.topk), -1, dtype=torch.int32)
                    ar = torch.arange(R, dtype=torch.int32)
                    for j in range(1, rt.force_nc):
                        fmh[:, j - 1] = (ar + 37 * j) % R
                    fm = ws['forced_match'] = fmh.view(R, Vg, self.topk).to(self.dev)
                ws['match'].copy_(fm)
            o.roi_positions_csr(rois, ws['zero_mask'], ws['roi_mask'], ws['rect'], ws['pos2s'], ws['s2pos'], ws['S_dev'], R, V, h, w, ws['match'],
                                ws['row_ptr'], ws['col_idx'], ws['nnz'], Vg, self.topk, stride=self.stride, expand_stride=-1.0, grp_start=grp,
                                order=order, order_flags=ws['qt_ctl'][1:] if rt.q_order else None, roi_size=self.roi_size)
        if rt.grouped:
            o.xattn_group_tables(ws['row_ptr'], ws['col_idx'], grp, R, ws['grp_tab'], order=order)
        if masked:
            transpose(ws['roi_mask'])
        if rt.kind == 'T' and not forked:
            tk('roi_align')
            o.roi_align(featcl, rois, h, w, out0=ws['roi_feat'], out0_lo=ws['roi_lo'] if rt.conv_x3 else None, R=R, roi_size=self.roi_size)
        md = ws['S_dev']
        if rt.pe_x3:
            tk('pe_inputs'); tk('pe_fused')
            self._exact_pe(ws, featcl, P, V, h, w)
        else:
            tk('pe_inputs')
            o.pe_inputs(ws['s2pos'], md, P, featcl, T['img2lidar'], T['coords_w'], T['coords_h'], T['coords_d'], T['embeds'],
                        self.const['dim_t'], ws['A1'], ws['A2'] if rt.keep_sine_rows else None, ws['Xf_b'], None,
                        V, h, w, self.depth_num, self.pe_range_h64, ld=self.pe_kp)
            tk('pe_fused')
            dbg = rt.stages or rt.exact
            o.pe_fused_tab(ws['A1'], ws['Xf_b'], featcl, md, W_['pe_pack'], ws['shared']['sine_tab'], ws['shared']['sine_period'],
                           ws['pe'] if (rt.kind == 'S' or dbg) else None, ws['Xk'] if (rt.kind == 'T' or dbg) else None, M=P,
                           row_index=ws['s2pos'])
        if rt.kind == 'S':
            tk('roi_align')
            pe_map, pe_idx = (ws['pe_pos'], None) if rt.pe_at_pos else (ws['pe'], ws['pos2s'])
            if rt.lo8:
                lo = dict(out0_lo=ws['roi_lo'] if rt.conv_x3 else None, out0_lo8=ws['xv_lo'], out1_lo8=ws['xk_lo'], lo8_flag=ws['lo8_flag'])
            else:
                lo = dict(out0_lo=ws['xv_lo'], out1_lo=ws['xk_lo']) if rt.exact else {}
            o.roi_align(featcl, rois, h, w, map1=pe_map, out0=ws['roi_feat'], out1=ws['roi_sum'], map1_index=pe_idx, out1_is_sum=True, R=R,
                        roi_size=self.roi_size, **lo)
        if rt.ablate_zero_lo:
            zero = rt.ablate_zero_lo
            for c_ in 'vk':
                if c_ in zero:
                    ws[f'x{c_}_lo'].zero_()
            if '8' in zero:
                for t in (ws['xk_lo'], ws['xv_lo']):
                    if '8f' in zero:
                        t.copy_(((t.float() * 4096.0).clamp(-448.0, 448.0).to(torch.float8_e4m3fn).float() / 4096.0).to(t.dtype))
                        continue
                    f8 = torch.float8_e4m3fnuz if '8z' in zero else torch.float8_e5m2fnuz
                    m = t.float().abs().max().clamp_min(1e-30)
                    q8 = torch.exp2(torch.floor(torch.log2((100.0 if f8 == torch.float8_e4m3fnuz else 16000.0) / m)))
                    t.copy_(((t.float() * q8).to(f8).float() / q8).to(t.dtype))
        if forked:
            torch.cuda.current_stream().wait_stream(side)
        else:
            self._enqueue_qg(ws, R)
        if rt.stop_before_decoder:
            tk('end')
            return
        tk('decoder')
        self._enqueue_decoder(ws, R)
        tk('heads')
        self._enqueue_heads(ws, R, sc['dt'])
        tk('decode')
        o.decode_topk(ws['cls'][L - 1], ws['reg'][L - 1], R, self.num_classes, self.max_num, self.post_range_h, ws['boxes'], ws['scores'],
                      ws['labels'], ws['bbox_index'], ws['count'], grp_start=grp, max_grp_rows=sc['max_rows'], payload=ws.get('payload_out'))
        tk('end')

    def _exact_pe(self, ws, featcl, P, V, h, w):
        o, W_, T, rt = ops, self.w, ws['tab'], ws['route']
        md = ws['S_dev']
        if ws.get('pe_hit') and rt.pe_cache_views:
            sh = ws['shared']
            hw, period, vm = h * w, sh['sine_period'], sh['pe_vmask']
            flag = ws['lo8_flag'] if rt.lo8 else None
            o.pe_frustum_f32(ws['s2pos'], md, P, T['img2lidar'], T['coords_w'], T['coords_h'], T['coords_d'], ws['xa1'], V, h, w, self.depth_num,
                             self.pe_range_h64, ld=self.pe_kp, view_mask=vm, tab_period=period)
            o.pe_fused_x3(ws['xa1'], featcl, md, W_['pe_x3'], sh['sine_tab'], period, Xk=(ws['Xk'], ws['xk_lo']), Xv=(ws['Xf_b'], ws['xv_lo']), M=P,
                          row_index=ws['s2pos'], lo8_flag=flag, Kp=self.pe_kp, view_mask=vm, hw=hw)
            o.pe_gate_rows_x3(sh['pe_q'], featcl, md, W_['pe_x3'], sh['sine_tab'], period, (ws['Xk'], ws['xk_lo']), (ws['Xf_b'], ws['xv_lo']), P, vm, hw,
                              row_index=ws['s2pos'], lo8_flag=flag)
            return
        if ws.get('pe_hit'):
            sh = ws['shared']
            o.pe_gate_x3(sh['pe_q'], featcl, md, W_['pe_x3'], sh['sine_tab'], sh['sine_period'], ws['pe_pos'] if rt.pe_at_pos else ws['pe'], P,
                         row_index=ws['s2pos'], pe_at_index=rt.pe_at_pos)
            return
        if rt.keep_sine_rows:
            o.pe_inputs(ws['s2pos'], md, P, featcl, T['img2lidar'], T['coords_w'], T['coords_h'], T['coords_d'], T['embeds'],
                        self.const['dim_t'], ws['A1'], ws['A2'], ws['Xf_b'], None, V, h, w, self.depth_num,
                        self.pe_range_h64, A_frustum_f32=ws['xa1'], A_sine_f32=ws['xa2'], ld=self.pe_kp)
        else:
            o.pe_frustum_f32(ws['s2pos'], md, P, T['img2lidar'], T['coords_w'], T['coords_h'], T['coords_d'], ws['xa1'], V, h, w, self.depth_num,
                             self.pe_range_h64, ld=self.pe_kp)
        sh = ws['shared']
        rows = rt.kind == 'T'
        at_pos = rt.pe_at_pos
        size = {} if rt.pe_rows_in_waves else dict(Kp=self.pe_kp, gate=self.with_fpe)
        (o.pe_fused_x3b if rt.pe_rows_in_waves else o.pe_fused_x3)(
            ws['xa1'], featcl, md, W_['pe_x3'], sh['sine_tab'], sh['sine_period'], pe=(ws['pe_pos'] if at_pos else ws['pe']) if (not rows or rt.stages) else None,
            Xk=(ws['Xk'], ws['xk_lo']) if rows else None, Xv=(ws['Xf_b'], ws['xv_lo']) if rows else None, M=P, row_index=ws['s2pos'], pe_at_index=at_pos, lo8_flag=ws['lo8_flag'] if (rows and rt.lo8) else None,
            **size)

    def _build_pe_q(self, ws, sh, Pt, V, h, w):
        T, o, d = ws['tab'], ops, self.dev
        a1 = torch.zeros((Pt, self.pe_kp), device=d, dtype=F32)
        o.pe_frustum_f32(torch.arange(Pt, dtype=torch.int32, device=d), torch.tensor([Pt], dtype=torch.int32, device=d), Pt, T['img2lidar'], T['coords_w'],
                         T['coords_h'], T['coords_d'], a1, V, h, w, self.depth_num, self.pe_range_h64, ld=self.pe_kp)
        q = sh.get('pe_q')
        if q is None or tuple(q.shape) != (Pt, C):
            if q is not None:
                sh['pe_q_gen'] = sh.get('pe_q_gen', 0) + 1
            q = sh['pe_q'] = torch.empty((Pt, C), device=d, dtype=F32)
        if sh.get('pe_q_zero') is None:
            sh['pe_q_zero'] = torch.zeros((1, C), device=d, dtype=F32)
        o.pe_fused_x3(a1, None, None, self.w['pe_x3'], sh['pe_q_zero'], 1, pe=q, M=Pt, Kp=self.pe_kp, gate=False)
        self.pe_cache_builds = getattr(self, 'pe_cache_builds', 0) + 1

    def _build_pe_q_views(self, ws, sh, Pt, V, h, w, views):
        T, o, d, hw = ws['tab'], ops, self.dev, h * w
        pos = torch.cat([torch.arange(v * hw, (v + 1) * hw, dtype=torch.int32) for v in views]).to(d)
        n = int(pos.numel())
        a1 = torch.empty((n, self.pe_kp), device=d, dtype=F32)
        o.pe_frustum_f32(pos, torch.tensor([n], dtype=torch.int32, device=d), n, T['img2lidar'], T['coords_w'], T['coords_h'], T['coords_d'], a1, V, h, w,
                         self.depth_num, self.pe_range_h64, ld=self.pe_kp)
        q = sh.get('pe_q')
        if q is None or tuple(q.shape) != (Pt, C):
            if q is not None:
                sh['pe_q_gen'] = sh.get('pe_q_gen', 0) + 1
            q = sh['pe_q'] = torch.zeros((Pt, C), device=d, dtype=F32)
        if sh.get('pe_q_zero') is None:
            sh['pe_q_zero'] = torch.zeros((1, C), device=d, dtype=F32)
        o.pe_fused_x3(a1, None, None, self.w['pe_x3'], sh['pe_q_zero'], 1, pe=q, M=n, row_index=pos, pe_at_index=True, Kp=self.pe_kp, gate=False)
        self.pe_cache_builds = getattr(self, 'pe_cache_builds', 0) + 1

    def pe_input_rows(self, ws, positions, V, h, w, f32=False):
        n = int(positions.numel())
        T, d = ws['tab'], self.dev
        a1 = torch.empty((n, self.pe_kp), device=d, dtype=self.K16)
        a2 = None if self.no_sin_enc else torch.empty((n, 384), device=d, dtype=self.K16)
        xb = torch.empty((n, C), device=d, dtype=self.K16)
        a1f = torch.empty((n, self.pe_kp), device=d, dtype=F32) if f32 else None
        a2f = torch.empty((n, 384), device=d, dtype=F32) if (f32 and not self.no_sin_enc) else None
        ops.pe_inputs(positions.contiguous(), torch.tensor([n], dtype=torch.int32, device=d), n, ws['featcl'], T['img2lidar'], T['coords_w'],
                      T['coords_h'], T['coords_d'], T['embeds'], self.const['dim_t'], a1, a2, xb, None, V, h, w, self.depth_num, self.pe_range_h64,
                      A_frustum_f32=a1f, A_sine_f32=a2f, ld=self.pe_kp)
        return (a1f, a2f) if f32 else (a1, a2)

    def _enqueue_qg(self, ws, R):
        o, W_, tk = ops, self.w, self._tick
        if not self.qg.is_default:
            return self._enqueue_qg_shape(ws, R)
        tk('qg_conv_gemm')
        if ws['route'].conv_x3:
            o.qg_conv_pool_x3(ws['roi_feat'], ws['roi_lo'], W_['qg_conv_wx3'], W_['qg_conv_b'], ws['x2'], R=R, roi_size=self.roi_size)
        else:
            o.qg_conv_pool(ws['roi_feat'], W_['qg_conv_wp'], W_['qg_conv_b'], ws['x2'], R=R, roi_size=self.roi_size)
        tk('qg_rest')
        rt = ws['route']
        if rt.qg_tail_fused and self._qg_tail_dims and not rt.keep_sine_rows:
            o.qg_tail_x3(ws['x2'], ws['enc'], W_['qg_fc_wx'], W_['qg_fc_b'], W_['qg_e0_wx'], W_['qg_e0_b'], W_['qg_e2_wx'], W_['qg_e2_b'],
                         W_['qg_c_w'], W_['qg_c_b'], ws['minv'], self.const['dim_t'], self.pc_range_h, W_['qe_w0x'], W_['qe_b0'], W_['qe_w2x'],
                         W_['qe_b2'], ws['center'], ws['xyz'], ws['ref'], ws['posemb'], ws['qpos'], R=R)
            return
        o.linear_x3(ws['x2'], W_['qg_fc_wx'], W_['qg_fc_b'], N=1024, K=256, act=1, clamp=5e3, out=ws['enc'], ldc=1056, M=R)
        o.linear_x3(ws['enc'], W_['qg_e0_wx'], W_['qg_e0_b'], N=512, K=1056, act=1, out=ws['enc1'], M=R)
        o.linear_x3(ws['enc1'], W_['qg_e2_wx'], W_['qg_e2_b'], N=256, K=512, act=1, out=ws['enc2'], M=R)
        o.query_embed_fused_x3(ws['enc2'], W_['qg_c_w'], W_['qg_c_b'], ws['minv'], self.const['dim_t'], self.pc_range_h, W_['qe_w0x'],
                               W_['qe_b0'], W_['qe_w2x'], W_['qe_b2'], ws['center'], ws['xyz'], ws['ref'], ws['posemb'], ws['qpos'], R=R)

    def _enqueue_qg_shape(self, ws, R):
        o, W_, tk, qs, s = ops, self.w, self._tick, self.qg, self.roi_size
        tk('qg_conv_gemm')
        hi, lo = ws['roi_feat'], ws['roi_lo']
        for i, (wx3, b) in enumerate(W_['qg_convs']):
            if i < qs.convs - 1:
                nh, nl = ws[f'qg_cells_hi{i & 1}'], ws[f'qg_cells_lo{i & 1}']
                o.qg_conv_cells(hi, lo, wx3, b, out_hi=nh, out_lo=nl, R=R, roi_size=s)
                hi, lo = nh, nl
            elif qs.pooled:
                o.qg_conv_pool_x3(hi, lo, wx3, b, ws['x2'], R=R, roi_size=s)
            else:
                o.qg_conv_cells(hi, lo, wx3, b, out_f32=ws['qg_flat'], R=R, roi_size=s)
        if qs.convs == 0:
            if qs.pooled:
                o.avgpool_cells(hi, lo, ws['x2'], R, self.cells)
            else:
                o.avgpool_cells(hi, lo, ws['qg_flat'].view(R * self.cells, C), R * self.cells, 1)
        tk('qg_rest')
        for l in W_['qg_lin']:
            o.linear_x3(ws[l['src']], l['wx'], l['b'], N=l['N'], K=l['K'], act=1, clamp=l['clamp'], out=ws[l['dst']], ldc=l['ldc'], M=R)
        last = ws[W_['qg_last']]
        if qs.center_in == C:
            o.query_embed_fused_x3(last, W_['qg_c_w'], W_['qg_c_b'], ws['minv'], self.const['dim_t'], self.pc_range_h, W_['qe_w0x'],
                                   W_['qe_b0'], W_['qe_w2x'], W_['qe_b2'], ws['center'], ws['xyz'], ws['ref'], ws['posemb'], ws['qpos'], R=R)
            return
        o.linear_x3(last, W_['qg_c_wx'], W_['qg_c_b16'], N=16, K=last.shape[1], out=ws['qg_center16'], M=R)
        o.refpoint_posemb(ws['qg_center16'], 16, ws['minv'], self.const['dim_t'], ws['xyz'], ws['ref'], ws['posemb'], R, self.pc_range_h)
        o.linear_x3(ws['posemb'], W_['qe_w0x'], W_['qe_b0'], N=C, K=384, act=1, out=ws['qe1'], M=R)
        o.linear_x3(ws['qe1'], W_['qe_w2x'], W_['qe_b2'], N=C, K=C, out=ws['qpos'], M=R)

    def _enqueue_decoder(self, ws, R):
        o, W_, L, rt = ops, self.w, self.L, ws['route']
        x = ws['x']
        dn = ws.get('dn')
        dbg = ws['dbg_logits'] if rt.debug_attn else None
        maps_fused = not (rt.grouped or rt.xattn_fused) and rt.maps_fused(R)
        xk_rows, xv_rows = ws['xk_rows'], ws['xv_rows']
        lo_k, lo_v = (ws['xk_lo'], ws['xv_lo']) if rt.attn_lo else (None, None)
        rows = dict(Xk_lo=lo_k, Xv_lo=lo_v, empty_nan=self.empty_nan, order=ws['q_order'] if rt.q_order else None)

        def tile_attn(i):
            if dbg is not None:
                ws['dbg_q'][i].copy_(ws['q'])
            o.xattn_tile(ws['Qt'], xk_rows, xv_rows, ws['row_ptr'], ws['col_idx'], ws['zh'], R, waves=rt.xattn_waves,
                         dbg_logits=None if dbg is None else dbg[i], **rows)

        x_in, xq_in = ws['zero_rows'], ws['qpos']
        fold0 = rt.fold_sa0
        if fold0 and ws.get('sa0_ver') != self._weights_version:
            ws['sa0_ctx'].copy_(W_['sa_in_b0'][2 * C:].expand(ws['sa0_ctx'].shape[0], C))
            ws['sa0_ver'] = self._weights_version
        for i in range(L):
            if i == 1:
                x_in = x
            sa_ctx = ws['ctx']
            if i == 0 and fold0:
                sa_ctx = ws['sa0_ctx']
            else:
                if i == 0:
                    o.linear_x3(xq_in, W_['sa_in_wx0'], W_['sa_in_b0'], N=3 * C, K=C, A2=x_in, n_split=2 * C, out=ws['qkv'], M=R)
                if dn:
                    o.self_attn_dn(ws['qkv'], dn[0], dn[1], out=ws['ctx'])
                else:
                    o.self_attn(ws['qkv'], ws['ctx'], R, grp_start=ws['grp_start'], max_grp_rows=ws.get('max_rows', 0))
            sa_args = (sa_ctx, x_in, W_[f'sa_out_wx{i}'], W_[f'sa_out_b{i}'], (W_[f'ln0_w{i}'], W_[f'ln0_b{i}']), ws['x1'])
            q_args = dict(qpos=ws['qpos'], Wq_x3=W_[f'ca_q_wx{i}'], bq=W_[f'ca_q_b{i}'], qscale=ops.SCALE_Q, M=R)
            out_args = (ws['x1'], W_[f'ca_out_wx{i}'], W_[f'ca_out_b{i}'], (W_[f'ln1_w{i}'], W_[f'ln1_b{i}']), ws['x2'])
            mapA, mapB, bv = W_[f'ca_mapA{i}'], W_[f'ca_mapB{i}'], W_[f'ca_v_b{i}']
            if maps_fused:
                o.attn_out_qmap_x3(*sa_args, WA=mapA, Qt=ws['Qt'], **q_args)
                tile_attn(i)
                o.attn_out_zmap_x3(ws['zh'], mapB, bv, ws['row_ptr'], *out_args, empty_nan=self.empty_nan, M=R)
            else:
                o.attn_out_fused_x3(*sa_args, q_out=ws['q'], **q_args)
                if rt.grouped:
                    o.xattn_group(ws['q'], mapA, mapB, bv, xk_rows, xv_rows, ws['row_ptr'], ws['grp_tab'], out=ws['ctx'], R=R, **rows)
                elif rt.xattn_fused:
                    o.xattn_fused(ws['q'], mapA, mapB, bv, xk_rows, xv_rows, ws['row_ptr'], ws['col_idx'], out=ws['ctx'], R=R, deal=rt.xattn_deal, **rows)
                else:
                    o.xattn_qmap(ws['q'], mapA, ws['Qt'], R=R)
                    tile_attn(i)
                    o.xattn_ctxmap(ws['zh'], mapB, bv, ws['row_ptr'], ws['ctx'], R, empty_nan=self.empty_nan)
                o.attn_out_fused_x3(ws['ctx'], *out_args, M=R)
            G = ops.FFN_GROUPS
            parts = ws['parts']
            o.ffn_fused_x3(ws['x2'], W_[f'ffn_w1x{i}'], W_[f'ffn_b1{i}'], W_[f'ffn_w2x{i}'], parts, R, groups=G)
            nxt = i + 1 < L
            o.ffn_out_fused_x3(parts, W_[f'ffn_b2{i}'], ws['x2'], (W_[f'ln2_w{i}'], W_[f'ln2_b{i}']), (W_['post_w'], W_['post_b']),
                               x, ws['qpos'], None, outs=ws['outs'][i], Win_x3=W_[f'sa_in_wx{i + 1}'] if nxt else None,
                               b_in=W_[f'sa_in_b{i + 1}'] if nxt else None, qkv=ws['qkv'] if nxt else None, M=R)

    def _enqueue_heads(self, ws, R, dt):
        dt_rows = ws['dt_rows'] if self.kind == 'T' else None
        last = ws['route'].last_stage_heads
        ll, n = (self.L - 1, 1) if last else (0, self.L)
        cls_p, reg_p = (self.cls_ptrs_x3_last, self.reg_ptrs_x3_last) if last else (self.cls_ptrs_x3, self.reg_ptrs_x3)
        outs, cls, reg = ws['outs'][ll:], ws['cls'][ll:], ws['reg'][ll:]
        nf = self.num_reg_fcs
        if self.use_reg_layer:
            ops.heads_cls_depth_x3(outs, cls_p, cls, R, n, nf, num_classes=self.num_classes)
            ops.reg_layer_depth_x3(outs, reg_p, ws['ref'], reg, R, n, nf, self.group_reg_dims, self.pc_range_h, dt, dt_rows=dt_rows)
        else:
            ops.heads_depth_x3(outs, cls_p, reg_p, ws['ref'], cls, reg, R, n, nf, self.pc_range_h, dt, dt_rows=dt_rows, num_classes=self.num_classes)

    def _result(self, ws, R, batch=False):
        sel = (lambda t: t) if batch else (lambda t: t[0])
        out = dict(R=R, ws=ws, cls=ws['cls'][:, :R], reg=ws['reg'][:, :R], boxes=sel(ws['boxes']), scores=sel(ws['scores']), labels=sel(ws['labels']),
                   bbox_index=sel(ws['bbox_index']), count=ws['count'] if batch else ws['count'][:1], grp_start=ws['grp_start_h'].clone(),
                   pe_cache=ws.get('pe_cache_state', 'off'),
                   pe_cache_views=ws.get('pe_views', ()))
        if ws['route'].stages:
            rows0 = ('rois', 'minv', 'enc', 'roi_feat', 'center', 'xyz', 'ref', 'posemb', 'qpos', 'match')
            st = {}
            for kk in rows0 + ('roi_mask', 'pos2s', 's2pos', 'S_dev', 'col_idx', 'pe', 'Xk', 'Xf_b', 'dbg_logits', 'dbg_q'):
                if ws.get(kk) is not None:
                    st[kk] = (ws[kk][:R] if kk in rows0 else ws[kk]).clone()
            for kk in ('outs', 'cls', 'reg'):
                st[kk] = ws[kk][:, :R].clone()
            st['row_ptr'] = ws['row_ptr'][:R + 1].clone()
            st['nnz'] = torch.stack([ws['row_ptr'][R], ws['nnz'][1]])
            out['stages'] = st
        return out

    def run(self, feat, proposals, img_metas, keep_stages=False, use_graph=False, payload=None):
        return self._run([feat], [proposals], [img_metas], keep_stages, use_graph, batch=False, payload=payload)

    def run_batch(self, feats, proposals_list, metas_list, keep_stages=False, use_graph=False, payload=None):
        return self._run(feats, proposals_list, metas_list, keep_stages, use_graph, batch=True, payload=payload)

    def _run(self, feats, proposals_list, metas_list, keep_stages, use_graph, batch, payload=None):
        B = len(proposals_list)
        if payload is not None:
            assert payload.is_cuda and payload.dtype == F32 and payload.is_contiguous() and tuple(payload.shape) == (B, self.max_num * 11 + 1), \
                'payload: fp32 [samples, max_num * 11 + 1] on the GPU'
        stacked = torch.is_tensor(feats)
        fl = [feats] if stacked else list(feats)
        for f in fl:
            assert f.is_cuda and f.dim() == 4 and f.shape[1] == C
        map_dtype = fl[0].dtype
        ops.map_format(map_dtype)
        if any(f.dtype != map_dtype for f in fl):
            raise ValueError(f'mv2d engine: the feature maps of a batch must share one dtype, got {sorted({str(f.dtype) for f in fl})}')
        rt = route.resolve(self, self.kind, self.exact, self.depth_num, map_dtype, keep_stages, use_graph,
                           pe_options=dict(with_fpe=self.with_fpe, no_sin_enc=self.no_sin_enc, LID=self.LID))
        if not self.qg.is_default and not rt.conv_x3:
            raise ValueError('mv2d engine: a query generator of other than the shipped shape runs on the index-exact route only (exact=True, the default, '
                             "without 'conv' in exact_skip): the engine has no key16-mode plan for " + repr(tuple(self.qg)))
        if stacked or B == 1:
            feat = fl[0]
            if not (feat.is_contiguous(memory_format=torch.channels_last) and not feat.is_contiguous()):
                feat = feat.contiguous()
            V, _, h, w = feat.shape
            ptrs = (feat.data_ptr(),)
        else:
            assert len(fl) == B
            feat = [f.contiguous() for f in fl]
            Vg, _, h, w = feat[0].shape
            assert all(tuple(f.shape) == tuple(feat[0].shape) for f in feat), 'samples of a batch share one map shape'
            V = Vg * B
            ptrs = tuple(f.data_ptr() for f in feat)
        assert V % B == 0
        ws, R, sc = self._host_prepare(proposals_list, metas_list, V, h, w, rt)
        ws['dyn_d'].copy_(ws['dyn_h'], non_blocking=True)
        ws['payload_out'], ws['route'] = payload, rt
        Rc = sc['cap']
        if rt.debug_attn:
            ws['dbg_logits'] = torch.zeros((self.L, 8, ws['col_cap']), device=self.dev, dtype=F32)
            ws['dbg_q'] = torch.zeros((self.L, Rc, C), device=self.dev, dtype=F32)
        else:
            ws.pop('dbg_logits', None); ws.pop('dbg_q', None)
        if not use_graph:
            self._enqueue(ws, feat, Rc, V, h, w, sc)
            self._mark_done(ws)
            return dict(self._result(ws, R, batch), dt=sc['dt'])
        gkey = (ptrs, 0 if payload is None else payload.data_ptr(), sc['pad_h'], sc['pad_w'], sc['max_rows'], self.num_classes, self.roi_size,
                self.use_reg_layer, self.group_reg_dims, self.num_reg_fcs, self._weights_version, rt)
        graphs = ws.setdefault('graphs', {})
        g = graphs.get(gkey)
        hit, parked = ws['pe_hit'], ws.setdefault('graphs_other_pe_form', {})
        if g is not None and g[2] != hit:
            other = parked.pop(gkey, None)
            if len(parked) >= 32:
                parked.pop(next(iter(parked)))
            parked[gkey] = graphs.pop(gkey)
            g = other
            if g is not None:
                graphs[gkey] = g
        if ws.pop('graph_stale', False):
            graphs.clear(); parked.clear()
            g = None
        if g is None:
            prof, self.prof = self.prof, None
            side = torch.cuda.Stream()
            side.wait_stream(torch.cuda.current_stream())
            with torch.cuda.stream(side):
                self._enqueue(ws, feat, Rc, V, h, w, sc)
            torch.cuda.current_stream().wait_stream(side)
            torch.cuda.synchronize()
            g = torch.cuda.CUDAGraph()
            with torch.cuda.graph(g, capture_error_mode='thread_local'):
                self._enqueue(ws, feat, Rc, V, h, w, sc)
            self.prof = prof
            if len(graphs) >= 32:
                graphs.pop(next(iter(graphs)))
            graphs[gkey] = (g, feat, hit)
        else:
            g = g[0]
        g.replay()
        self._mark_done(ws)
        return dict(self._result(ws, R, batch), dt=sc['dt'])

    def train_forward(self, out, dn_ref=None, dn_single=0):
        ws, R = out['ws'], out['R']
        L, d, o, W_ = self.L, self.dev, ops, self.w
        if ws['B'] != 1:
            raise ValueError('train_forward: one sample per run (the reference asserts the same, RH/mv2d_s_head.py:249)')
        row_ptr = ws['row_ptr'][:R + 1]
        nnz = int(row_ptr[R].item())
        if int(ws['nnz'][1].item()) != 0:
            raise RuntimeError('mv2d engine: CSR capacity exceeded (raise col_cap_per_query)')
        col_fb = None
        if self.kind == 'T' and bool((row_ptr[1:] == row_ptr[:-1]).any().item()):
            from .train import fallback_key_csr
            s0 = int(ws['pos2s'][0].item())
            if s0 < 0:
                s0 = int(ws['S_dev'].item())
                V_, h_, w_ = ws['map_shape']
                a1f, a2f = self.pe_input_rows(ws, torch.zeros(1, dtype=torch.int32, device=d), V_, h_, w_, f32=True)
                fin = ws['feat_in']
                fin0 = fin[0] if isinstance(fin, (list, tuple)) else fin
                if fin0.is_contiguous(memory_format=torch.channels_last) and not fin0.is_contiguous():
                    f0 = fin0.permute(0, 2, 3, 1).reshape(-1, C)[:1].float().contiguous()
                else:
                    f0 = fin0[0, :, 0, 0].reshape(1, C).float().contiguous()
                def mlp1(x32, n1, n2, **kw):
                    h3 = o.gemm_bf16(o.split3_rows(x32), self._c3(n1), W_['pe_b' + n1[1:]], act=1, split3=True)
                    return o.gemm_bf16(h3, self._c3(n2), W_['pe_b' + n2[1:]], out_dtype=F32, **kw)
                pg = mlp1(a1f, 'w1a', 'w1b', **(dict(mul=mlp1(f0, 'wr', 'we', act=2)) if self.with_fpe else {}))
                pe0 = pg if self.no_sin_enc else mlp1(a2f, 'w2a', 'w2b', add=pg)
                ws['Xk'][s0:s0 + 1].copy_(o.f32_to_key16(pe0 + f0)); ws['Xf_b'][s0:s0 + 1].copy_(o.f32_to_key16(f0))
            row_ptr, col_fb, _ = fallback_key_csr(row_ptr.clone(), ws['col_idx'][:int(row_ptr[R].item())].clone(), s0)
        no_dn = dn_ref is None or dn_ref.shape[0] == 0
        if no_dn and col_fb is None:
            return ws['cls'][:, :R].clone(), ws['reg'][:, :R].clone()
        if no_dn:
            dn_ref = torch.zeros((0, 3), device=d, dtype=F32)
        pad = int(dn_ref.shape[0])
        T = pad + R
        col = ws['col_idx'][:nnz] if col_fb is None else col_fb
        nnz = int(col.numel())
        keys = torch.unique(col).to(torch.int32)
        nk = int(keys.numel())
        e = lambda *shape: torch.empty(shape, device=d, dtype=F32)
        posemb = o.posemb3d(dn_ref.to(F32).contiguous(), self.const['dim_t'])
        q1 = o.linear_x3(posemb, W_['qe_w0x'], W_['qe_b0'], N=C, K=384, act=1)
        qdn = o.linear_x3(q1, W_['qe_w2x'], W_['qe_b2'], N=C, K=C)
        tws = dict(B=1, Vg=ws['Vg'], dn=(pad, max(int(dn_single), 1)), route=ws['route'].denoising(), grp_start=None, xk_rows=ws['xk_rows'], xv_rows=ws['xv_rows'],
                   Qt=torch.empty((T, 16 * C), device=d, dtype=self.K16), zh=e(T, 8 * C),
                   row_ptr=torch.cat([torch.arange(pad, device=d, dtype=torch.int32) * nk, row_ptr + pad * nk]),
                   col_idx=torch.cat([keys.repeat(pad), col]).contiguous(),
                   ref=torch.cat([dn_ref.to(F32), ws['ref'][:R]]).contiguous(), qpos=torch.cat([qdn, ws['qpos'][:R]]).contiguous(),
                   zero_rows=torch.zeros(T, C, device=d), qkv=e(T, 3 * C), parts=e(self.ffn_slabs, T, C), outs=e(L, T, C), cls=e(L, T, self.num_classes),
                   reg=e(L, T, 10), dt_rows=torch.cat([torch.zeros(pad, device=d), torch.full((R,), float(out.get('dt', 0.0)), device=d)]))
        for n in ('x', 'x1', 'x2', 'ctx', 'q'):
            tws[n] = e(T, C)
        self._enqueue_decoder(tws, T)
        self._enqueue_heads(tws, T, float(out.get('dt', 0.0)))
        return tws['cls'], tws['reg']

    @staticmethod
    def _mark_done(ws):
        sh = ws['shared']
        if 'done_ev' not in sh:
            sh['done_ev'] = torch.cuda.Event()
        sh['done_ev'].record()

    def clone_shared(self):
        other = object.__new__(HeadEngine)
        other.__dict__.update(self.__dict__)
        other._ws = {}
        other._ws_base = {}
        other._shape_cache = self._shape_cache
        other.prof = None
        return other

    @staticmethod
    def _check_capacity(ws):
        _, nnz_over, _, _, _, grp_over, lo8_sat, _ = ws['ctl'].tolist()
        if nnz_over != 0:
            raise RuntimeError('mv2d engine: CSR capacity exceeded (raise col_cap_per_query)')
        if grp_over != 0:
            raise RuntimeError('mv2d engine: union-list capacity of the shared-tile cross attention exceeded (a CSR row lists a key twice?)')
        if lo8_sat != 0:
            import warnings
            warnings.warn('mv2d engine: key / value rows beyond +-224 in this frame: their 8-bit lo halves saturated (those elements keep key16 precision); '
                          'set HeadEngine.lo8_rows = False for fp16 lo rows', RuntimeWarning, stacklevel=3)

    def results(self, out):
        n = int(out['count'][0].item())
        self._check_capacity(out['ws'])
        return out['boxes'][:n], out['scores'][:n], out['labels'][:n]

    def results_batch(self, out):
        counts = out['count'].tolist()
        self._check_capacity(out['ws'])
        return [(out['boxes'][b, :n], out['scores'][b, :n], out['labels'][b, :n]) for b, n in enumerate(counts)]
```

mv2d_amd/ops.py:

```python
import math
import numbers

import numpy as np
import torch

from . import _lib
from ._lib import check

BF16 = torch.bfloat16
_K16 = None


def key16_dtype():
    global _K16
    if _K16 is None:
        _K16 = torch.float16 if _lib.load().mv2d_key16_format() == 1 else torch.bfloat16
    return _K16


_RAW_STREAM, _GET_DEV = getattr(torch._C, '_cuda_getCurrentRawStream', None), getattr(torch._C, '_cuda_getDevice', None)


def _stream():
    if _RAW_STREAM is not None and _GET_DEV is not None:
# ... 592 lines not shown


def pe_fused_x3(A1, Xmap, m_dev, wx, sine_tab, tab_period, pe=None, Xk=None, Xv=None, M=None, row_index=None, pe_at_index=False, lo8_flag=None,
                map_fmt=None, Kp=None, gate=True, view_mask=None, hw=None, take_set=False):
    _req(A1, torch.float32, 'A1'); _req(sine_tab, torch.float32, 'sine_tab'); _req(pe, torch.float32, 'pe')
    fmt = 0 if (Xmap is None and not gate) else _req_map(Xmap, 'Xmap', map_fmt)
    _req(row_index, torch.int32, 'row_index'); _req(m_dev, torch.int32, 'm_dev')
    for pair in (Xk, Xv):
        if pair is not None:
            _req16(pair[0], 'hi')
    lo_fmt = _lo_fmt(Xk[1] if Xk else None, Xv[1] if Xv else None)
    for k in ('w1a', 'w1b', 'wr', 'we') if gate else ('w1a', 'w1b'):
        _req(wx[k][0], q16_dtype(), k); _req(wx[k][1], q16_dtype(), k)
    M = A1.shape[0] if M is None else M
    xk, xv = Xk or (None, None), Xv or (None, None)
    Kp = A1.shape[-1] if Kp is None else Kp
    if A1.dim() != 2 or A1.shape[1] != Kp or wx['w1a'][0].numel() != 1024 * Kp:
        raise _lib.Mv2dHipError(f'pe_fused_x3: A1 {tuple(A1.shape)} / w1a ({wx["w1a"][0].numel()} elements) do not have Kp = {Kp} columns')
    rows = (_p(A1), _p(Xmap), _p(row_index), _p(m_dev), M, _p(wx['w1a'][0]), _p(wx['w1a'][1]), _p(wx['b1a']), _p(wx['w1b'][0]), _p(wx['w1b'][1]), _p(wx['b1b']))
    if view_mask is not None:
        name = 'mv2d_pe_fused_x3_k_sel'
        vm, hw = _view_sel(name, view_mask, hw, tab_period)
        if not gate or Xk is None or Xv is None or pe_at_index:
            raise _lib.Mv2dHipError(name + ': the filtered form is the gated kernel with key / value row outputs (Xk and Xv), pe in row order')
        check(_lib.load().mv2d_pe_fused_x3_k_sel(*rows, _p(wx['wr'][0]), _p(wx['wr'][1]), _p(wx['br']), _p(wx['we'][0]), _p(wx['we'][1]), _p(wx['be']),
                                                 _p(sine_tab), int(tab_period), _p(pe), _p(xk[0]), _p(xk[1]), _p(xv[0]), _p(xv[1]), lo_fmt, _p(lo8_flag), fmt,
                                                 int(Kp), vm, hw, 1 if take_set else 0, _stream()), name)
        return pe
    outs = (_p(sine_tab), int(tab_period), _p(pe), _p(xk[0]), _p(xk[1]), _p(xv[0]), _p(xv[1]), lo_fmt, 1 if (pe_at_index and row_index is not None) else 0,
            _p(lo8_flag), fmt, int(Kp), _stream())
    if gate:
        check(_lib.load().mv2d_pe_fused_x3_k(*rows, _p(wx['wr'][0]), _p(wx['wr'][1]), _p(wx['br']), _p(wx['we'][0]), _p(wx['we'][1]), _p(wx['be']), *outs),
              'mv2d_pe_fused_x3')
    else:
        check(_lib.load().mv2d_pe_fused_x3_ng(*rows, *outs), 'mv2d_pe_fused_x3_ng')
    return pe


def pe_gate_x3(Q, Xmap, m_dev, wx, sine_tab, tab_period, pe, M, row_index=None, pe_at_index=False, map_fmt=None, Xk=None, Xv=None):
    name = 'mv2d_pe_gate_x3'
    _req(Q, torch.float32, name + ': Q'); _req(sine_tab, torch.float32, name + ': sine_tab'); _req(pe, torch.float32, name + ': pe')
    if Q is None or pe is None or Xmap is None:
        raise _lib.Mv2dHipError(name + ': Q, Xmap and pe are required')
    fmt = _req_map(Xmap, name + ': Xmap', map_fmt)
    _req(row_index, torch.int32, name + ': row_index'); _req(m_dev, torch.int32, name + ': m_dev')
    for k in ('wr', 'we'):
        _req(wx[k][0], q16_dtype(), name + ': ' + k); _req(wx[k][1], q16_dtype(), name + ': ' + k)
    if int(tab_period) > 0 and (tuple(Q.shape) != (int(tab_period), 256) or sine_tab.dim() != 2 or sine_tab.shape[0] < int(tab_period) or sine_tab.shape[1] != 256):
        raise _lib.Mv2dHipError(f'{name}: Q {tuple(Q.shape)} / sine_tab {tuple(sine_tab.shape)} do not hold tab_period = {tab_period} rows of 256')
    xk, xv = Xk or (None, None), Xv or (None, None)
    check(_lib.load().mv2d_pe_gate_x3(_p(Q), _p(Xmap), _p(row_index), _p(m_dev), int(M), _p(wx['wr'][0]), _p(wx['wr'][1]), _p(wx['br']), _p(wx['we'][0]),
                                      _p(wx['we'][1]), _p(wx['be']), _p(sine_tab), int(tab_period), _p(pe), _p(xk[0]), _p(xk[1]), _p(xv[0]), _p(xv[1]),
                                      1 if (pe_at_index and row_index is not None) else 0, fmt, _stream()), name)
    return pe


def pe_gate_rows_x3(Q, Xmap, m_dev, wx, sine_tab, tab_period, Xk, Xv, M, view_mask, hw, row_index=None, pe=None, lo8_flag=None, map_fmt=None, take_set=True):
    name = 'mv2d_pe_gate_rows_x3'
    _req(Q, torch.float32, name + ': Q'); _req(sine_tab, torch.float32, name + ': sine_tab'); _req(pe, torch.float32, name + ': pe')
    if Q is None or Xmap is None or Xk is None or Xv is None:
        raise _lib.Mv2dHipError(name + ': Q, Xmap, Xk and Xv are required')
    fmt = _req_map(Xmap, name + ': Xmap', map_fmt)
    _req(row_index, torch.int32, name + ': row_index'); _req(m_dev, torch.int32, name + ': m_dev')
    for pair in (Xk, Xv):
        _req16(pair[0], name + ': hi rows')
    lo_fmt = _lo_fmt(Xk[1], Xv[1])
    for k in ('wr', 'we'):
        _req(wx[k][0], q16_dtype(), name + ': ' + k); _req(wx[k][1], q16_dtype(), name + ': ' + k)
    vm, hw = _view_sel(name, view_mask, hw, tab_period)
    if tuple(Q.shape) != (int(tab_period), 256) or sine_tab.dim() != 2 or sine_tab.shape[0] < int(tab_period) or sine_tab.shape[1] != 256:
        raise _lib.Mv2dHipError(f'{name}: Q {tuple(Q.shape)} / sine_tab {tuple(sine_tab.shape)} do not hold tab_period = {tab_period} rows of 256')
    check(_lib.load().mv2d_pe_gate_rows_x3(_p(Q), _p(Xmap), _p(row_index), _p(m_dev), int(M), _p(wx['wr'][0]), _p(wx['wr'][1]), _p(wx['br']), _p(wx['we'][0]),
                                           _p(wx['we'][1]), _p(wx['be']), _p(sine_tab), int(tab_period), _p(pe), _p(Xk[0]), _p(Xk[1]), _p(Xv[0]), _p(Xv[1]),
                                           lo_fmt, _p(lo8_flag), fmt, vm, hw, 1 if take_set else 0, _stream()), name)


def pe_fused_x3b(A1, Xmap, m_dev, wx, sine_tab, tab_period, pe=None, Xk=None, Xv=None, M=None, row_index=None, pe_at_index=False, lo8_flag=None):
    _req(A1, torch.float32, 'A1'); _req(Xmap, torch.float32, 'Xmap (pe_fused_x3b has no 16-bit-map instance)'); _req(sine_tab, torch.float32, 'sine_tab'); _req(pe, torch.float32, 'pe')
    _req(row_index, torch.int32, 'row_index'); _req(m_dev, torch.int32, 'm_dev')
    for pair in (Xk, Xv):
        if pair is not None:
            _req16(pair[0], 'hi')
    lo_fmt = _lo_fmt(Xk[1] if Xk else None, Xv[1] if Xv else None)
    for k in ('w1a_p', 'w1b', 'wr_p', 'we'):
        _req(wx[k][0], q16_dtype(), k); _req(wx[k][1], q16_dtype(), k)
    M = A1.shape[0] if M is None else M
    xk, xv = Xk or (None, None), Xv or (None, None)
    check(_lib.load().mv2d_pe_fused_x3b(_p(A1), _p(Xmap), _p(row_index), _p(m_dev), M, _p(wx['w1a_p'][0]), _p(wx['w1a_p'][1]), _p(wx['b1a']),
                                        _p(wx['w1b'][0]), _p(wx['w1b'][1]), _p(wx['b1b']), _p(wx['wr_p'][0]), _p(wx['wr_p'][1]), _p(wx['br']),
                                        _p(wx['we'][0]), _p(wx['we'][1]), _p(wx['be']), _p(sine_tab), int(tab_period), _p(pe), _p(xk[0]), _p(xk[1]),
                                        _p(xv[0]), _p(xv[1]), lo_fmt, 1 if (pe_at_index and row_index is not None) else 0, _p(lo8_flag), _stream()), 'mv2d_pe_fused_x3b')
    return pe


def pack_wfrag(W):
    if W.dtype not in (BF16, torch.float16):
        raise _lib.Mv2dHipError(f'pack_wfrag: expected a 16-bit weight, got {W.dtype}')
    _req(W, W.dtype, 'W')
    N, K = W.shape
    Wp = torch.empty(N * K, device=W.device, dtype=W.dtype)
    check(_lib.load().mv2d_pack_wfrag_bf16(_p(W), _p(Wp), N, K, _stream()), 'mv2d_pack_wfrag_bf16')
    return Wp


def _roi_size(s):
    s = int(s)
    if not 1 <= s <= 14:
        raise ValueError(f'roi_size must be in [1, 14], got {s}')
    return s


def qg_conv_pool(roi_feat, W, bias, out, R=None, ld_out=None, roi_size=7):
    _req16(roi_feat, 'roi_feat'); _req16(W, 'W'); _req(bias, torch.float32, 'bias'); _req(out, torch.float32, 'out')
    R = roi_feat.shape[0] if R is None else R
    s = _roi_size(roi_size)
    check(_lib.load().mv2d_qg_conv_pool_s(_p(roi_feat), _p(W), _p(bias), _p(out), out.stride(0) if ld_out is None else ld_out, R, s, _stream()),
          'mv2d_qg_conv_pool')
    return out


def qg_conv_pool_x3(roi_hi, roi_lo, W_x3, bias, out, R=None, ld_out=None, roi_size=7):
    _req16(roi_hi, 'roi_hi'); _req16(roi_lo, 'roi_lo'); _req16(W_x3[0], 'W_hi'); _req16(W_x3[1], 'W_lo'); _req(bias, torch.float32, 'bias'); _req(out, torch.float32, 'out')
    R = roi_hi.shape[0] if R is None else R
    s = _roi_size(roi_size)
    check(_lib.load().mv2d_qg_conv_pool_x3_s(_p(roi_hi), _p(roi_lo), _p(W_x3[0]), _p(W_x3[1]), _p(bias), _p(out),
                                             out.stride(0) if ld_out is None else ld_out, R, s, _stream()), 'mv2d_qg_conv_pool_x3')
    return out


def qg_conv_cells(roi_hi, roi_lo, W, bias, out_hi=None, out_lo=None, out_f32=None, R=None, roi_size=7):
    _req16(roi_hi, 'roi_hi'); _req16(roi_lo, 'roi_lo'); _req(bias, torch.float32, 'bias')
    _req16(out_hi, 'out_hi'); _req16(out_lo, 'out_lo'); _req(out_f32, torch.float32, 'out_f32')
    for w_, n_ in ((W, 'W'),) if roi_lo is None else ((W[0], 'W_hi'), (W[1], 'W_lo')):
        _req16(w_, n_)
    R = roi_hi.shape[0] if R is None else R
    s = _roi_size(roi_size)
    n = R * s * s * 256
    ins = [t for t in (roi_hi, roi_lo) if t is not None]
    for t in ins:
        if not t.is_contiguous() or t.numel() < n:
            raise ValueError('qg_conv_cells: the RoI cells are contiguous [R, s*s, 256] key16 tensors')
    if bias.numel() < 256:
        raise ValueError('qg_conv_cells: bias holds 256 values')
    for t in (out_hi, out_lo, out_f32):
        if t is None:
            continue
        if not t.is_contiguous() or t.numel() < n:
            raise ValueError('qg_conv_cells: outputs are contiguous [R, s*s, 256] tensors, key16 (out_hi, out_lo) / fp32 (out_f32)')
        if any(t.untyped_storage().data_ptr() == i.untyped_storage().data_ptr() for i in ins):
            raise ValueError('qg_conv_cells: an output may not share storage with the input cells')
    if roi_lo is None:
        check(_lib.load().mv2d_qg_conv_cells(_p(roi_hi), _p(W), _p(bias), _p(out_hi), _p(out_lo), _p(out_f32), R, s, _stream()), 'mv2d_qg_conv_cells')
    else:
        check(_lib.load().mv2d_qg_conv_cells_x3(_p(roi_hi), _p(roi_lo), _p(W[0]), _p(W[1]), _p(bias), _p(out_hi), _p(out_lo), _p(out_f32), R, s, _stream()),
              'mv2d_qg_conv_cells_x3')


def avgpool_cells(hi, lo, out, R, cells, ld_out=None):
    _req16(hi, 'hi'); _req16(lo, 'lo'); _req(out, torch.float32, 'out')
    if not hi.is_contiguous() or (lo is not None and not lo.is_contiguous()):
        raise ValueError('avgpool_cells: hi / lo are contiguous key16 rows')
    if hi.numel() < R * cells * 256 or (lo is not None and lo.numel() < R * cells * 256):
        raise ValueError('avgpool_cells: hi / lo hold R * cells rows of 256 channels')
    ld = out.stride(0) if ld_out is None else ld_out
    if out.dtype != torch.float32 or out.numel() < (R - 1) * ld + 256:
        raise ValueError('avgpool_cells: out is an fp32 [R, ld_out >= 256] tensor')
    check(_lib.load().mv2d_avgpool_cells(_p(hi), 0 if lo is None else _p(lo), _p(out), ld, R, cells, _stream()), 'mv2d_avgpool_cells')
    return out


def avgpool49(x, out, ld_out, R):
    check(_lib.load().mv2d_avgpool49(_p(x), _p(out), ld_out, R, _stream()), 'mv2d_avgpool49')
    return out


def f32_to_bf16(x, out=None):
    _req(x, torch.float32, 'x')
    if out is None:
        out = torch.empty(x.shape, device=x.device, dtype=BF16)
    check(_lib.load().mv2d_f32_to_bf16(_p(x), _p(out), x.numel(), _stream()), 'mv2d_f32_to_bf16')
    return out


def nchw_to_nhwc_bf16(x, out=None):
    _req(x, torch.float32, 'x')
    V, Cn, h, w = x.shape
    if out is None:
        out = torch.empty((V * h * w, Cn), device=x.device, dtype=BF16)
    check(_lib.load().mv2d_nchw_to_nhwc_bf16(_p(x), _p(out), V, Cn, h * w, _stream()), 'mv2d_nchw_to_nhwc_bf16')
    return out


def map_conv3x3(x_cl, Wp, bias, V, h, w, out=None):
    _req(x_cl, BF16, 'x_cl'); _req(Wp, BF16, 'Wp'); _req(bias, torch.float32, 'bias')
    if out is None:
        out = torch.empty((V * h * w, 256), device=x_cl.device, dtype=torch.float32)
    check(_lib.load().mv2d_map_conv3x3(_p(x_cl), _p(Wp), _p(bias), _p(out), V, h, w, _stream()), 'mv2d_map_conv3x3')
    return out


def nchw_to_nhwc(x, out=None, mask=None, map_fmt=None):
    fmt = _req_map(x, 'x', map_fmt)
    _req(mask, torch.uint8, 'mask')
    V, Cn, h, w = x.shape
    if out is None:
        if mask is not None:
            raise _lib.Mv2dHipError('nchw_to_nhwc: the masked form writes into a caller-owned buffer')
        out = torch.empty((V * h * w, Cn), device=x.device, dtype=x.dtype)
    _req(out, x.dtype, 'out')
    if mask is not None:
        check(_lib.load().mv2d_nchw_to_nhwc_masked_fmt(_p(x), _p(out), _p(mask), V, Cn, h * w, fmt, _stream()), 'mv2d_nchw_to_nhwc_masked')
    else:
        check(_lib.load().mv2d_nchw_to_nhwc_fmt(_p(x), _p(out), V, Cn, h * w, fmt, _stream()), 'mv2d_nchw_to_nhwc')
    return out


def self_attn(qkv, out=None, R=None, grp_start=None, max_grp_rows=0, impl=None):
    _req(qkv, torch.float32, 'qkv')
    R = qkv.shape[0] if R is None else R
    if out is None:
        out = torch.empty((R, 256), device=qkv.device, dtype=torch.float32)
    n = 0 if grp_start is None else grp_start.numel() - 1
    if (impl or 'x3') == 'x3':
        check(_lib.load().mv2d_self_attn_x3_fwd(_p(qkv), _p(out), R, _p(grp_start), n, int(max_grp_rows), 0, 1, _stream()), 'mv2d_self_attn_x3_fwd')
    else:
        check(_lib.load().mv2d_self_attn_fwd(_p(qkv), _p(out), R, _p(grp_start), n, _stream()), 'mv2d_self_attn_fwd')
    return out


def self_attn_dn(qkv, dn_pad, dn_single, out=None, impl='f32'):
    _req(qkv, torch.float32, 'qkv')
    R = qkv.shape[0]
    if out is None:
        out = torch.empty((R, 256), device=qkv.device, dtype=torch.float32)
    if impl == 'x3':
        check(_lib.load().mv2d_self_attn_x3_fwd(_p(qkv), _p(out), R, None, 0, 0, int(dn_pad), max(int(dn_single), 1), _stream()), 'mv2d_self_attn_x3_fwd')
    else:
        check(_lib.load().mv2d_self_attn_dn_fwd(_p(qkv), _p(out), R, int(dn_pad), int(dn_single), _stream()), 'mv2d_self_attn_dn_fwd')
    return out


def dn_queries(gt, gt_labels, rnd, scalar, noise_scale, noise_trans, split, num_classes, pc_range, eps=1e-4):
    import ctypes
    G = gt.shape[0]
    n = G * scalar
    ref = torch.empty(n, 3, device=gt.device, dtype=torch.float32)
    labels = torch.empty(n, device=gt.device, dtype=torch.int64)
    boxes = torch.empty(n, 9, device=gt.device, dtype=torch.float32)
    rng = (ctypes.c_float * 6)(*[float(x) for x in pc_range])
    check(_lib.load().mv2d_dn_queries(_p(gt), _p(gt_labels), _p(rnd), G, int(scalar), float(noise_scale), float(noise_trans), float(split),
                                      int(num_classes), ctypes.cast(rng, ctypes.c_void_p), float(eps), _p(ref), _p(labels), _p(boxes),
                                      _stream()), 'mv2d_dn_queries')
    return ref, labels, boxes


def sparse_xattn(q, K, V, row_ptr, col_idx, out=None, R=None, dbg_logits=None, empty_nan=True, p_drop=0.0, seed=0):
    _req(q, torch.float32, 'q'); _req(K, BF16, 'K'); _req(V, BF16, 'V')
    _req(row_ptr, torch.int32, 'row_ptr'); _req(col_idx, torch.int32, 'col_idx')
    R = q.shape[0] if R is None else R
    if out is None:
        out = torch.empty((R, 256), device=q.device, dtype=torch.float32)
    check(_lib.load().mv2d_sparse_xattn_fwd_drop(_p(q), _p(K), _p(V), _p(row_ptr), _p(col_idx), _p(out), _p(dbg_logits),
                                                 dbg_logits.stride(0) if dbg_logits is not None else 0, R, 1 if empty_nan else 0, float(p_drop),
                                                 int(seed) & 0xffffffff, _stream()), 'mv2d_sparse_xattn_fwd')
    return out



def pack_xattn_maps(Wk, Wv):
    _req(Wk, torch.float32, 'Wk'); _req(Wv, torch.float32, 'Wv')
    d = Wk.device
    ar = lambda n_: torch.arange(n_, device=d)
    h, t, g, m, e = torch.meshgrid(ar(8), ar(16), ar(4), ar(16), ar(8), indexing='ij')
    wa = Wk[32 * h + 8 * g + e, 32 * (t >> 1) + 8 * (m >> 2) + 4 * (t & 1) + (m & 3)].contiguous()
    h, s, nt, g, n_, e = torch.meshgrid(ar(8), ar(8), ar(2), ar(4), ar(16), ar(8), indexing='ij')
    wb = Wv[32 * h + 16 * nt + n_, 32 * s + 8 * g + e].contiguous()
    return split_q16x2(wa.view(-1)), split_q16x2(wb.view(-1))


def xattn_qmap(q, WA, Qt=None, R=None):
    _req(q, torch.float32, 'q'); _req(WA[0], q16_dtype(), 'WA_hi'); _req(WA[1], q16_dtype(), 'WA_lo')
    R = q.shape[0] if R is None else R
    if Qt is None:
        Qt = torch.empty((R, 4096), device=q.device, dtype=key16_dtype())
    _req16(Qt, 'Qt')
    check(_lib.load().mv2d_xattn_qmap(_p(q), _p(WA[0]), _p(WA[1]), _p(Qt), R, _stream()), 'mv2d_xattn_qmap')
    return Qt


def xattn_tile(Qt, Xk, Xv, row_ptr, col_idx, out=None, R=None, dbg_logits=None, empty_nan=True, waves=0, Xk_lo=None, Xv_lo=None, order=None):
    _req16(Qt, 'Qt'); _req16(Xk, 'Xk'); _req16(Xv, 'Xv')
    lo_fmt = _lo_fmt(Xk_lo, Xv_lo)
    _req(row_ptr, torch.int32, 'row_ptr'); _req(col_idx, torch.int32, 'col_idx'); _req(dbg_logits, torch.float32, 'dbg_logits')
    R = Qt.shape[0] if R is None else R
    if out is None:
        out = torch.empty((R, 8, 256), device=Qt.device, dtype=torch.float32)
    _req(order, torch.int32, 'order')
    check(_lib.load().mv2d_xattn_tile_fwd_ordered(_p(Qt), _p(Xk), _p(Xv), _p(Xk_lo), _p(Xv_lo), _p(row_ptr), _p(col_idx), _p(out), _p(dbg_logits),
                                                  dbg_logits.stride(0) if dbg_logits is not None else 0, R, 1 if empty_nan else 0, int(waves),
                                                  _p(order), lo_fmt, _stream()), 'mv2d_xattn_tile_fwd')
    return out


def xattn_fused(q, WA, WB, bv, Xk, Xv, row_ptr, col_idx, out=None, R=None, empty_nan=True, Xk_lo=None, Xv_lo=None, order=None, deal=0):
    _req(q, torch.float32, 'q'); _req(bv, torch.float32, 'bv'); _req(row_ptr, torch.int32, 'row_ptr'); _req(col_idx, torch.int32, 'col_idx')
    for t, n_ in ((WA[0], 'WA_hi'), (WA[1], 'WA_lo'), (WB[0], 'WB_hi'), (WB[1], 'WB_lo')):
        _req(t, q16_dtype(), n_)
    _req16(Xk, 'Xk'); _req16(Xv, 'Xv'); _req(order, torch.int32, 'order')
    lo_fmt = _lo_fmt(Xk_lo, Xv_lo)
    R = q.shape[0] if R is None else R
    if out is None:
        out = torch.empty((R, 256), device=q.device, dtype=torch.float32)
    _req(out, torch.float32, 'out')
    check(_lib.load().mv2d_xattn_fused_fwd_p(_p(q), _p(WA[0]), _p(WA[1]), _p(WB[0]), _p(WB[1]), _p(bv), _p(Xk), _p(Xv), _p(Xk_lo), _p(Xv_lo), _p(row_ptr),
                                             _p(col_idx), _p(out), R, 1 if empty_nan else 0, _p(order), lo_fmt, int(deal), _stream()),
          'mv2d_xattn_fused_fwd_p')
    return out


def xattn_group_max(R, n_samples):
    return (R + 7) // 8 + n_samples + 1


def xattn_group_alloc(R, n_samples, col_cap, device):
    ng = xattn_group_max(R, n_samples)
    ucap = col_cap + 16 * ng
    return dict(ng=ng, g=torch.zeros((4, ng), device=device, dtype=torch.int32), ucol=torch.zeros(ucap, device=device, dtype=torch.int32),
                umask=torch.zeros(ucap, device=device, dtype=torch.uint8), ucap=ucap, ctl=torch.zeros(2, device=device, dtype=torch.int32))


def xattn_group_tables(row_ptr, col_idx, grp_start, R, tab, order=None):
    _req(row_ptr, torch.int32, 'row_ptr'); _req(col_idx, torch.int32, 'col_idx'); _req(grp_start, torch.int32, 'grp_start'); _req(order, torch.int32, 'order')
    g, ctl = tab['g'], tab['ctl']
    check(_lib.load().mv2d_xattn_group_tables(_p(row_ptr), _p(col_idx), _p(order), _p(grp_start), grp_start.numel() - 1, R, tab['ng'], _p(g[0]), _p(g[1]),
                                              _p(g[2]), _p(g[3]), _p(tab['ucol']), _p(tab['umask']), tab['ucap'], _p(ctl[:1]), _p(ctl[1:]), _stream()),
          'mv2d_xattn_group_tables')
    return tab


def xattn_group(q, WA, WB, bv, Xk, Xv, row_ptr, tab, out=None, R=None, empty_nan=True, Xk_lo=None, Xv_lo=None, order=None):
    _req(q, torch.float32, 'q'); _req(bv, torch.float32, 'bv'); _req(row_ptr, torch.int32, 'row_ptr'); _req(order, torch.int32, 'order')
    for t, n_ in ((WA[0], 'WA_hi'), (WA[1], 'WA_lo'), (WB[0], 'WB_hi'), (WB[1], 'WB_lo')):
        _req(t, q16_dtype(), n_)
    _req16(Xk, 'Xk'); _req16(Xv, 'Xv'); _req16(Xk_lo, 'Xk_lo'); _req16(Xv_lo, 'Xv_lo')
    R = q.shape[0] if R is None else R
    if out is None:
        out = torch.empty((R, 256), device=q.device, dtype=torch.float32)
    _req(out, torch.float32, 'out')
    g = tab['g']
    check(_lib.load().mv2d_xattn_group_fwd(_p(q), _p(WA[0]), _p(WA[1]), _p(WB[0]), _p(WB[1]), _p(bv), _p(Xk), _p(Xv), _p(Xk_lo), _p(Xv_lo), _p(row_ptr),
                                           _p(order), _p(g[0]), _p(g[1]), _p(g[2]), _p(g[3]), _p(tab['ucol']), _p(tab['umask']), _p(out), tab['ng'],
                                           1 if empty_nan else 0, _stream()), 'mv2d_xattn_group_fwd')
    return out


def xattn_query_order(row_ptr, col_idx, grp_start, R, perm, flags, stride=0):
    check(_lib.load().mv2d_xattn_query_order(_p(row_ptr), _p(col_idx), _p(grp_start), grp_start.numel() - 1, R, _p(perm), _p(flags), int(stride), _stream()),
          'mv2d_xattn_query_order')
    return perm


def xattn_ctxmap(z, WB, bv, row_ptr, out=None, R=None, empty_nan=True):
    _req(z, torch.float32, 'z'); _req(WB[0], q16_dtype(), 'WB_hi'); _req(WB[1], q16_dtype(), 'WB_lo'); _req(bv, torch.float32, 'bv')
    _req(row_ptr, torch.int32, 'row_ptr')
    R = z.shape[0] if R is None else R
    if out is None:
        out = torch.empty((R, 256), device=z.device, dtype=torch.float32)
    check(_lib.load().mv2d_xattn_ctxmap(_p(z), _p(WB[0]), _p(WB[1]), _p(bv), _p(row_ptr), _p(out), R, 1 if empty_nan else 0, _stream()),
          'mv2d_xattn_ctxmap')
    return out


def csr_transpose(row_ptr, col_idx, S):
    nnz = col_idx.numel()
    R = row_ptr.numel() - 1
    counts = (row_ptr[1:] - row_ptr[:-1]).long()
    pair_row = torch.repeat_interleave(torch.arange(R, device=col_idx.device, dtype=torch.int32), counts, output_size=nnz)
    pair_idx = torch.sort(col_idx.long(), stable=True).indices.to(torch.int32)
    key_ptr = torch.zeros(S + 1, device=col_idx.device, dtype=torch.int32)
    key_ptr[1:] = torch.bincount(col_idx.long(), minlength=S).cumsum(0).to(torch.int32)
    return key_ptr, pair_idx, pair_row


def attn_drop_mask(nnz, seed, p_drop):
    import numpy as np
    if p_drop <= 0:
        return np.ones((nnz, 8), np.float32)
    pf = np.float32(p_drop)
    t = float(pf) * 4294967296.0
    thr = (0xffffffff if t >= 4294967295.0 else int(t)) or 1
    with np.errstate(over='ignore'):
        u = (np.arange(nnz * 8, dtype=np.uint64) * np.uint64(0x9E3779B1)).astype(np.uint32) ^ np.uint32(seed & 0xffffffff)
        u ^= u >> np.uint32(16); u = (u.astype(np.uint64) * np.uint64(0x85EBCA6B)).astype(np.uint32)
        u ^= u >> np.uint32(13); u = (u.astype(np.uint64) * np.uint64(0xC2B2AE35)).astype(np.uint32)
        u ^= u >> np.uint32(16)
    return np.where(u >= np.uint32(thr), np.float32(1.0) / (np.float32(1.0) - pf), np.float32(0)).reshape(nnz, 8)


def sparse_xattn_bwd(q, K, V, row_ptr, col_idx, ctx, dctx, R=None, transposed=None, p_drop=0.0, seed=0, long_rows=None, dq_scale=1.0):
    _req(q, torch.float32, 'q'); _req(K, BF16, 'K'); _req(V, BF16, 'V'); _req(ctx, torch.float32, 'ctx'); _req(dctx, torch.float32, 'dctx')
    R = q.shape[0] if R is None else R
    S = K.shape[0]
    nnz = col_idx.numel()
    key_ptr, pair_idx, pair_row = transposed if transposed is not None else csr_transpose(row_ptr, col_idx[:nnz], S)
    dq = torch.empty((R, 256), device=q.device, dtype=torch.float32)
    dK = torch.empty((S, 256), device=q.device, dtype=torch.float32)
    dV = torch.empty((S, 256), device=q.device, dtype=torch.float32)
    pair_ws = torch.empty((max(nnz, 1), 16), device=q.device, dtype=torch.float32)
    if long_rows is None:
        long_rows = 1 if (nnz >= 64 * max(R, 1) and nnz >= 64 * max(S, 1)) else 0
    check(_lib.load().mv2d_sparse_xattn_bwd_ex(_p(q), _p(K), _p(V), _p(row_ptr), _p(col_idx), _p(ctx), _p(dctx.contiguous()), _p(key_ptr), _p(pair_idx),
                                               _p(pair_row), _p(pair_ws), _p(dq), _p(dK), _p(dV), R, S, float(p_drop), int(seed) & 0xffffffff, int(bool(long_rows)),
                                               float(dq_scale), _stream()), 'mv2d_sparse_xattn_bwd')
    return dq, dK, dV


class SparseCrossAttention(torch.autograd.Function):

    @staticmethod
    def forward(fctx, q, K, V, row_ptr, col_idx, empty_nan=False, transposed=None, p_drop=0.0, seed=0):
        fctx.kv_dtypes = (K.dtype, V.dtype)
        q, K, V = q.contiguous(), K.to(BF16).contiguous(), V.to(BF16).contiguous()
        out = sparse_xattn(q, K, V, row_ptr, col_idx, R=q.shape[0], empty_nan=empty_nan, p_drop=p_drop, seed=seed)
        fctx.save_for_backward(q, K, V, row_ptr, col_idx, out)
        fctx.transposed = transposed
        fctx.drop = (float(p_drop), int(seed))
        return out

    @staticmethod
    def backward(fctx, dout):
        q, K, V, row_ptr, col_idx, out = fctx.saved_tensors
        dq, dK, dV = sparse_xattn_bwd(q, K, V, row_ptr, col_idx, out, dout.float().contiguous(), transposed=fctx.transposed, p_drop=fctx.drop[0],
                                      seed=fctx.drop[1])
        return dq, dK.to(fctx.kv_dtypes[0]), dV.to(fctx.kv_dtypes[1]), None, None, None, None, None, None


def box_params(rois, viewK, viewE, intr, ld_intr, minv, K_roi=None, roi_size=7.0, intr_scale=0.1, min_size=4.0):
    _req(rois, torch.float32, 'rois'); _req(viewK, torch.float64, 'viewK'); _req(viewE, torch.float64, 'viewE')
    check(_lib.load().mv2d_box_params(_p(rois), _p(viewK), _p(viewE), _p(K_roi), _p(intr), ld_intr, _p(minv), rois.shape[0],
                                      roi_size, intr_scale, min_size, _stream()), 'mv2d_box_params')


def refpoint_posemb(center_pred, ld_cp, minv, dim_t, xyz, ref, posemb, R, pc_range_host):
    check(_lib.load().mv2d_refpoint_posemb(_p(center_pred), ld_cp, _p(minv), _p(dim_t), _p(xyz), _p(ref), _p(posemb), R,
                                           pc_range_host.data_ptr(), _stream()), 'mv2d_refpoint_posemb')


def lidar2img_inverse(K_roi, E, out=None):
    _req(K_roi, torch.float64, 'K_roi'); _req(E, torch.float64, 'E')
    R = K_roi.shape[0]
    if out is None:
        out = torch.empty((R, 16), device=K_roi.device, dtype=torch.float32)
    check(_lib.load().mv2d_lidar2img_inverse(_p(K_roi), _p(E), _p(out), R, _stream()), 'mv2d_lidar2img_inverse')
    return out


def posemb3d(ref, dim_t, out=None):
    _req(ref, torch.float32, 'ref')
    R = ref.shape[0]
    if out is None:
        out = torch.empty((R, 384), device=ref.device, dtype=torch.float32)
    check(_lib.load().mv2d_posemb3d(_p(ref), _p(dim_t), _p(out), R, _stream()), 'mv2d_posemb3d')
    return out


def roi_align(map0, rois, H, W, *, map1=None, out0=None, out1=None, out0_f32=None, out1_f32=None, spatial_scale=1.0 / 16,
              sampling_ratio=-1, map1_index=None, out1_is_sum=False, R=None, out0_lo=None, out1_lo=None, out0_lo8=None, out1_lo8=None, lo8_flag=None,
              roi_size=7, map_fmt=None):
    fmt = _req_map(map0, 'map0', map_fmt)
    _req(map1, torch.float32, 'map1'); _req(rois, torch.float32, 'rois')
    _req16(out0, 'out0'); _req16(out1, 'out1'); _req16(out0_lo, 'out0_lo'); _req16(out1_lo, 'out1_lo')
    _req(out0_lo8, torch.uint8, 'out0_lo8'); _req(out1_lo8, torch.uint8, 'out1_lo8'); _req(lo8_flag, torch.int32, 'lo8_flag')
    s = _roi_size(roi_size)
    check(_lib.load().mv2d_roi_align_fmt(_p(map0), _p(map1), _p(rois), _p(out0), _p(out1), _p(out0_f32), _p(out1_f32),
                                         rois.shape[0] if R is None else R, H, W, map0.shape[-1], spatial_scale, sampling_ratio,
                                         _p(map1_index), 1 if out1_is_sum else 0, _p(out0_lo), _p(out1_lo), _p(out0_lo8), _p(out1_lo8), _p(lo8_flag), s,
                                         fmt, _stream()), 'mv2d_roi_align')


def box_correlation(rois, view_start, trans, lin, depths, match, V, topk, pad_h, pad_w, max_per_view, sample_size=4,
                    num_depth=8, depth_start=0.5, iou_thr=0.0, ratio=0.0):
    _req(rois, torch.float32, 'rois'); _req(view_start, torch.int32, 'view_start'); _req(trans, torch.float64, 'trans')
    _req(match, torch.int32, 'match')
    check(_lib.load().mv2d_box_correlation_ex(_p(rois), _p(view_start), _p(trans), _p(lin), _p(depths), _p(match), rois.shape[0], V,
                                              int(sample_size), int(num_depth), topk, pad_h, pad_w, float(depth_start), iou_thr, ratio, max_per_view,
                                              _stream()), 'mv2d_box_correlation')


def frame_geometry(rois, viewK, viewE, intr, ld_intr, minv, view_start, trans, lin, depths, match, V, topk, pad_h, pad_w, max_per_view,
                   K_roi=None, roi_size=7.0, intr_scale=0.1, min_size=4.0, sample_size=4, num_depth=8, depth_start=0.5, iou_thr=0.0, ratio=0.0, zero=None, R=None):
    _req(rois, torch.float32, 'rois'); _req(viewK, torch.float64, 'viewK'); _req(viewE, torch.float64, 'viewE'); _req(view_start, torch.int32, 'view_start')
    _req(trans, torch.float64, 'trans'); _req(match, torch.int32, 'match'); _req(zero, torch.uint8, 'zero')
    check(_lib.load().mv2d_frame_geometry_ex(_p(rois), _p(viewK), _p(viewE), _p(K_roi), _p(intr), ld_intr, _p(minv), roi_size, intr_scale, min_size,
                                             _p(view_start), _p(trans), _p(lin), _p(depths), _p(match), rois.shape[0] if R is None else R, V,
                                             int(sample_size), int(num_depth), topk, pad_h, pad_w, float(depth_start), iou_thr, ratio, max_per_view,
                                             _p(zero), zero.numel() if zero is not None else 0, _stream()), 'mv2d_frame_geometry')


def csr_workspace_bytes(R, V, h, w):
    return _lib.load().mv2d_csr_workspace_bytes(R, V, h, w)


def mask_compact(rois, match, pad_mask, roi_mask, rect, pos2s, s2pos, S_out, bits_ws, row_count, row_ptr, col_idx, nnz_out,
                 R, V, h, w, topk, stride=16.0, expand_stride=2.0, col_cap=None, n_samples=1):
    col_cap = col_idx.numel() if col_cap is None else col_cap
    check(_lib.load().mv2d_mask_compact(_p(rois), _p(match), _p(pad_mask), _p(roi_mask), _p(rect), _p(pos2s), _p(s2pos), _p(S_out),
                                        _p(bits_ws), _p(row_count), _p(row_ptr), _p(col_idx), _p(nnz_out), col_cap, R, V, h, w, topk,
                                        float(stride), float(expand_stride), n_samples, _stream()), 'mv2d_mask_compact')


def roi_positions(rois, pad_mask, roi_mask, rect, pos2s, s2pos, S_out, R, V, h, w, stride=16.0, expand_stride=1.0):
    check(_lib.load().mv2d_roi_positions(_p(rois), _p(pad_mask), _p(roi_mask), _p(rect), _p(pos2s), _p(s2pos), _p(S_out), R, V, h, w,
                                         float(stride), float(expand_stride), _stream()), 'mv2d_roi_positions')


def roi_positions_csr(rois, pad_mask, roi_mask, rect, pos2s, s2pos, S_out, R, V, h, w, match, row_ptr, col_idx, nnz_out, Vg, topk, stride=16.0,
                      expand_stride=1.0, grp_start=None, order=None, order_flags=None, roi_size=7):
    _req(order, torch.int32, 'order'); _req(grp_start, torch.int32, 'grp_start'); _req(order_flags, torch.int32, 'order_flags')
    s = _roi_size(roi_size)
    check(_lib.load().mv2d_roi_positions_csr_s(_p(rois), _p(pad_mask), _p(roi_mask), _p(rect), _p(pos2s), _p(s2pos), _p(S_out), R, V, h, w, float(stride),
                                               float(expand_stride), _p(match), _p(row_ptr), _p(col_idx), _p(nnz_out), Vg, topk, _p(grp_start),
                                               grp_start.numel() - 1 if grp_start is not None else 0, _p(order), _p(order_flags), s, _stream()),
          'mv2d_roi_positions_csr')


def csr_from_corr(match, row_ptr, col_idx, nnz_out, R, V, topk, roi_size=7):
    s = _roi_size(roi_size)
    check(_lib.load().mv2d_csr_from_corr_s(_p(match), _p(row_ptr), _p(col_idx), _p(nnz_out), R, V, topk, s, _stream()), 'mv2d_csr_from_corr')


def pe_inputs(s2pos, S_dev, S_max, featcl, img2lidar, coords_w, coords_h, coords_d, embeds, dim_t, A_frustum, A_sine, Xf_k16,
              Xf_f32, V, h, w, depth_num, position_range_host, A_frustum_f32=None, A_sine_f32=None, map_fmt=None, ld=None):
    _req16(A_frustum, 'A_frustum'); _req16(A_sine, 'A_sine'); _req16(Xf_k16, 'Xf_k16')
    _req(A_frustum_f32, torch.float32, 'A_frustum_f32'); _req(A_sine_f32, torch.float32, 'A_sine_f32'); _req(Xf_f32, torch.float32, 'Xf_f32')
    fmt = _req_map(featcl, 'featcl', map_fmt)
    ld = 3 * depth_num if ld is None else int(ld)
    for t in (A_frustum, A_frustum_f32):
        if t is not None and (t.dim() != 2 or t.shape[1] != ld):
            raise _lib.Mv2dHipError(f'pe_inputs: frustum rows {tuple(t.shape)} do not have {ld} columns')
    check(_lib.load().mv2d_pe_inputs_ld(_p(s2pos), _p(S_dev), S_max, _p(featcl), _p(img2lidar), _p(coords_w), _p(coords_h), _p(coords_d),
                                        _p(embeds), _p(dim_t), _p(A_frustum), _p(A_sine), _p(Xf_k16), _p(Xf_f32), _p(A_frustum_f32),
                                        _p(A_sine_f32), V, h, w, depth_num, position_range_host.data_ptr(), fmt, ld, _stream()), 'mv2d_pe_inputs')


def pe_frustum_f32(s2pos, S_dev, S_max, img2lidar, coords_w, coords_h, coords_d, out, V, h, w, depth_num, position_range_host, ld=None,
                   view_mask=None, tab_period=None):
    _req(s2pos, torch.int32, 's2pos'); _req(S_dev, torch.int32, 'S_dev'); _req(out, torch.float32, 'out')
    for t, n_ in ((img2lidar, 'img2lidar'), (coords_w, 'coords_w'), (coords_h, 'coords_h'), (coords_d, 'coords_d')):
        _req(t, torch.float64, n_)
    ld = 3 * depth_num if ld is None else int(ld)
    if out.dim() != 2 or out.shape[1] != ld:
        raise _lib.Mv2dHipError(f'pe_frustum_f32: out {tuple(out.shape)} does not have {ld} columns')
    if view_mask is not None:
        name = 'mv2d_pe_frustum_f32_sel'
        vm, _ = _view_sel(name, view_mask, h * w, 0 if tab_period is None else tab_period)
        check(_lib.load().mv2d_pe_frustum_f32_sel(_p(s2pos), _p(S_dev), S_max, _p(img2lidar), _p(coords_w), _p(coords_h), _p(coords_d), _p(out), V, h, w,
                                                  depth_num, position_range_host.data_ptr(), ld, vm, int(tab_period), _stream()), name)
        return out
    check(_lib.load().mv2d_pe_frustum_f32_ld(_p(s2pos), _p(S_dev), S_max, _p(img2lidar), _p(coords_w), _p(coords_h), _p(coords_d), _p(out), V, h, w,
                                             depth_num, position_range_host.data_ptr(), ld, _stream()), 'mv2d_pe_frustum_f32')
    return out


def decode_topk(cls, reg, R, num_classes, max_num, post_center_range_host, boxes, scores, labels, bbox_index, count, topk_dbg=None,
                grp_start=None, max_grp_rows=0, payload=None):
    _req(cls, torch.float32, 'cls'); _req(reg, torch.float32, 'reg'); _req(payload, torch.float32, 'payload')
    n = 0 if grp_start is None else grp_start.numel() - 1
    check(_lib.load().mv2d_decode_topk(_p(cls), _p(reg), R, num_classes, max_num, post_center_range_host.data_ptr(), _p(boxes),
                                       _p(scores), _p(labels), _p(bbox_index), _p(count), _p(topk_dbg), _p(grp_start), n, max_grp_rows,
                                       _p(payload), _stream()), 'mv2d_decode_topk')


def result_pack(boxes, scores, labels, count, score_thr, max_num, out_boxes, out_scores, out_labels, out_count, n_samples=1, in_stride=0):
    check(_lib.load().mv2d_result_pack(_p(boxes), _p(scores), _p(labels), _p(count), float(score_thr), max_num, _p(out_boxes), _p(out_scores),
                                       _p(out_labels), _p(out_count), n_samples, in_stride, _stream()), 'mv2d_result_pack')


def nms_bev(boxes, scores, labels, count, nms_thr, n_samples=1):
    out = torch.empty_like(scores)
    check(_lib.load().mv2d_nms_bev(_p(boxes.contiguous()), _p(scores.contiguous()), _p(labels.contiguous()), _p(count), float(nms_thr), _p(out),
                                   int(n_samples), int(scores.shape[-1]), _stream()), 'mv2d_nms_bev')
    return out


def pack_detections(boxes, scores, labels, count, out, max_num=300):
    n = count.numel()
    in_stride = scores.shape[-1]
    check(_lib.load().mv2d_pack_detections(_p(boxes), _p(scores), _p(labels), _p(count), _p(out), n, max_num, in_stride, _stream()),
          'mv2d_pack_detections')
    return out


class RoIAlignRows(torch.autograd.Function):

    @staticmethod
    def forward(ctx, rows, index, rois, H, W, full=None, roi_size=7):
        R, s = rois.shape[0], _roi_size(roi_size)
        out = torch.empty((R, s * s, 256), device=rows.device, dtype=torch.float32)
        rows_c = rows.contiguous()
        if index is None:
            roi_align(rows_c, rois, H, W, out0_f32=out, R=R, roi_size=s)
        else:
            scratch = torch.empty_like(out)
            roi_align(full.contiguous(), rois, H, W, map1=rows_c, out0_f32=scratch, out1_f32=out, map1_index=index, R=R, roi_size=s)
        ctx.save_for_backward(rois, index if index is not None else torch.empty(0, dtype=torch.int32, device=rows.device))
        ctx.meta = (H, W, rows.shape[0], index is not None, s)
        return out

    @staticmethod
    def backward(ctx, gout):
        rois, index = ctx.saved_tensors
        H, W, n, indexed, s = ctx.meta
        gmap = torch.zeros((n, 256), device=gout.device, dtype=torch.float32)
        check(_lib.load().mv2d_roi_align_bwd_s(_p(gout.contiguous().float()), _p(rois), _p(gmap), _p(index) if indexed else None, rois.shape[0], H, W,
                                               256, 1.0 / 16, -1, s, _stream()), 'mv2d_roi_align_bwd')
        return gmap, None, None, None, None, None, None


def match_cost(cls, box, gt, gt_labels, cls_weight=2.0, reg_weight=0.25, alpha=0.25, gamma=2.0):
# ... 25 lines not shown
```

mv2d_amd/route.py:

```python
import os
from collections import namedtuple
from typing import NamedTuple

import torch


def default_options():
    env = os.environ.get
    return dict(
        prof=None,
        fork_qg=True, fuse_maps={'0': False, '1': True}.get(env('MV2D_FUSE_MAPS', ''), None), fuse_xattn=None, group_xattn=None,
        xattn_waves=int(env('MV2D_XATTN_WAVES', '2')), q_order=True, fold_sa0=True, masked_transpose=True, last_stage_heads=False,
        exact_skip=frozenset({'conv'}), lo8_rows=True, pe_at_positions=env('MV2D_PE_AT_POS', '1') != '0', pe_rows_in_waves=False,
        ablate_zero_lo=frozenset(), keep_sine_rows=False, stop_before_decoder=False, force_nc=None, debug_attn=False,
        fuse_qg_tail=env('MV2D_QG_TAIL', '1') != '0', pe_cache=env('MV2D_PE_CACHE', '1') != '0', pe_cache_views=env('MV2D_PE_CACHE_VIEWS', '0') == '1',
        xattn_deal=0)


OPTIONS = tuple(default_options())


class Route(NamedTuple):
    kind: str
    exact: bool
    lo8: bool
    pe_pos: bool
    group_tab: bool
    q_order: bool
    map_dtype: torch.dtype
    stages: bool
    pe_x3: bool
    conv_x3: bool
    attn_lo: bool
    pe_at_pos: bool
    pe_rows_in_waves: bool
    keep_sine_rows: bool
    grouped: bool
    xattn_fused: bool
    xattn_fused_forced: bool
    fuse_maps: object
    xattn_waves: int
    fold_sa0: bool
    forked: bool
    masked: bool
    last_stage_heads: bool
    debug_attn: bool
    stop_before_decoder: bool
    force_nc: object
    ablate_zero_lo: frozenset
    qg_tail_fused: bool
    pe_cache: bool
    pe_cache_views: bool
    xattn_deal: int

    @property
    def storage(self):
        return Storage(*self[:6])

    def maps_fused(self, R):
        return ((R <= 512) if self.fuse_maps is None else bool(self.fuse_maps)) and not self.debug_attn

    def denoising(self):
        return self._replace(attn_lo=False, grouped=False, xattn_fused=self.xattn_fused_forced, q_order=False, fold_sa0=False, debug_attn=False)


Storage = namedtuple('Storage', Route._fields[:6])


def resolve(opts, kind, exact, depth_num, map_dtype=torch.float32, keep_stages=False, use_graph=False, pe_options=None):
    o, stages = opts, bool(keep_stages)
    skip, debug, group = o.exact_skip, bool(o.debug_attn), bool(o.group_xattn)
    pe_x3 = exact and 'pe' not in skip
    if depth_num != 64 and not pe_x3:
        raise ValueError(f'mv2d engine: the key16 mode\'s PE kernel (csrc/pe_tab96.hip) is built for depth_num = 64 only; run the index-exact route (exact=True, the default) with depth_num = {depth_num}')
    if depth_num != 64 and o.pe_rows_in_waves:
        raise ValueError(f'mv2d engine: pe_rows_in_waves (csrc/pe_x3b.hip) is built for depth_num = 64 only; unset it for depth_num = {depth_num}')
    for key, shipped in (('with_fpe', True), ('no_sin_enc', False), ('LID', True)):
        v = (pe_options or {}).get(key, shipped)
        if v != shipped and not pe_x3:
            raise ValueError(f'mv2d engine: the key16 mode\'s PE kernel (csrc/pe_tab96.hip) is built for {key}={shipped} only; run the index-exact route (exact=True, the default) with {key}={v}')
        if v != shipped and o.pe_rows_in_waves:
            raise ValueError(f'mv2d engine: pe_rows_in_waves (csrc/pe_x3b.hip) is built for {key}={shipped} only; unset it for {key}={v}')
    if map_dtype != torch.float32 and o.pe_rows_in_waves and pe_x3:
        raise ValueError('mv2d engine: pe_rows_in_waves (csrc/pe_x3b.hip) reads fp32 feature maps only; unset it for a torch.float16 / torch.bfloat16 map')
    lo8 = bool(o.lo8_rows) and exact and not group
    if o.ablate_zero_lo and lo8:
        raise ValueError('ablate_zero_lo works on key16 lo rows: set lo8_rows = False')
    assert not (debug and use_graph), 'debug_attn: eager runs only'
    if int(o.xattn_deal) not in (0, 1, 2):
        raise ValueError('mv2d engine: xattn_deal is 0 (the library\'s policy), 1 (whole rounds) or 2 (full blocks)')
    pe_pos = kind == 'S' and exact and bool(o.pe_at_positions)
    pe_opt = lambda key, shipped: (pe_options or {}).get(key, shipped)
    pe_cache_ok = (pe_x3 and bool(pe_opt('with_fpe', True)) and not pe_opt('no_sin_enc', False) and not stages and not o.keep_sine_rows
                   and not o.pe_rows_in_waves)
    pe_cache = bool(o.pe_cache) and kind == 'S' and pe_cache_ok
    pe_cache_views = bool(o.pe_cache_views) and kind == 'T' and pe_cache_ok
    forked = kind == 'T' and (o.prof is None or use_graph) and bool(o.fork_qg) and not exact
    return Route(
        kind=kind, exact=exact, lo8=lo8, pe_pos=pe_pos, group_tab=group, q_order=bool(o.q_order), map_dtype=map_dtype, stages=stages,
        pe_x3=pe_x3, conv_x3=exact and 'conv' not in skip, attn_lo=exact and 'attn' not in skip, pe_at_pos=pe_pos and pe_x3 and not stages,
        pe_rows_in_waves=bool(o.pe_rows_in_waves), keep_sine_rows=bool(o.keep_sine_rows), grouped=group and not debug,
        xattn_fused=(kind == 'S' if o.fuse_xattn is None else bool(o.fuse_xattn)) and not debug, xattn_fused_forced=bool(o.fuse_xattn),
        fuse_maps=o.fuse_maps, xattn_waves=int(o.xattn_waves), fold_sa0=bool(o.fold_sa0), forked=forked,
        masked=bool(o.masked_transpose) and not forked and not o.keep_sine_rows and not stages,
        last_stage_heads=bool(o.last_stage_heads) and not stages, debug_attn=debug, stop_before_decoder=bool(o.stop_before_decoder),
        force_nc=o.force_nc, ablate_zero_lo=frozenset(o.ablate_zero_lo) if exact else frozenset(),
        qg_tail_fused=bool(o.fuse_qg_tail) and not stages, pe_cache=pe_cache, pe_cache_views=pe_cache_views,
        xattn_deal=int(o.xattn_deal))
```

Measured before the change: 10910 samples/s.

## Add 12-wave fused cross-attention variant with slimmer LDS and raw e4m3 lo tiles

Adds a QB=12 instantiation of the fused cross-attention kernel for e4m3 lo rows. It cuts per-wave LDS from 16 KB to 12 KB by staging the lo key bytes raw and expanding them at MFMA time, and splits the WA/WB weight register loads into two halves to lower register pressure. It also delays the V lo-row load until after the score MFMAs and adds lane remapping. The goal is more query waves per block and better overlap of gathers with compute, at the cost of extra permutes and more complex indexing. A new entry point and a qb option are plumbed through; the host default may pick 12 (MV2D_XF_QB_BATCH), though the selection code is truncated.

```diff
diff --git a/include/mv2d_hip.h b/include/mv2d_hip.h
--- a/include/mv2d_hip.h
+++ b/include/mv2d_hip.h
@@ -202,6 +202,9 @@
 int mv2d_xattn_fused_fwd_p(const float* q, const void* WA_hi, const void* WA_lo, const void* WB_hi, const void* WB_lo, const float* bv, const void* Xk,
                            const void* Xv, const void* Xk_lo, const void* Xv_lo, const int* row_ptr, const int* col_idx, float* ctx, int R, int empty_nan,
                            const int* order, int lo_fmt, int deal, void* stream);
+int mv2d_xattn_fused_fwd_q(const float* q, const void* WA_hi, const void* WA_lo, const void* WB_hi, const void* WB_lo, const float* bv, const void* Xk,
+                           const void* Xv, const void* Xk_lo, const void* Xv_lo, const int* row_ptr, const int* col_idx, float* ctx, int R, int empty_nan,
+                           const int* order, int lo_fmt, int deal, int qb, void* stream);
 int mv2d_xattn_group_max(int R, int n_samples);
 int mv2d_xattn_group_tables(const int* row_ptr, const int* col_idx, const int* order, const int* grp_start, int n_samples, int R, int ng_max, int* g_slot,
                             int* g_cnt, int* g_ptr, int* g_len, int* ucol, unsigned char* umask, int ucap, int* u_total, int* flags, void* stream);
diff --git a/mv2d_amd/_lib.py b/mv2d_amd/_lib.py
--- a/mv2d_amd/_lib.py
+++ b/mv2d_amd/_lib.py
@@ -102,6 +102,7 @@
     'mv2d_xattn_tile_fwd_ordered': (I, [P, P, P, P, P, P, P, P, P, LL, I, I, I, P, I, P]),
     'mv2d_xattn_fused_fwd': (I, [P, P, P, P, P, P, P, P, P, P, P, P, P, I, I, P, I, P]),
     'mv2d_xattn_fused_fwd_p': (I, [P, P, P, P, P, P, P, P, P, P, P, P, P, I, I, P, I, I, P]),
+    'mv2d_xattn_fused_fwd_q': (I, [P, P, P, P, P, P, P, P, P, P, P, P, P, I, I, P, I, I, I, P]),
     'mv2d_xattn_group_max': (I, [I, I]),
     'mv2d_xattn_group_tables': (I, [P, P, P, P, I, I, I, P, P, P, P, P, P, I, P, P, P]),
     'mv2d_xattn_group_fwd': (I, [P] * 19 + [I, I, P]),
diff --git a/mv2d_amd/csrc/xattn_fused.hip b/mv2d_amd/csrc/xattn_fused.hip
--- a/mv2d_amd/csrc/xattn_fused.hip
+++ b/mv2d_amd/csrc/xattn_fused.hip
@@ -2,6 +2,9 @@
 #include <stdlib.h>
 #ifndef MV2D_XF_QB_DEFAULT
 #define MV2D_XF_QB_DEFAULT 8
+#endif
+#ifndef MV2D_XF_QB_BATCH
+#define MV2D_XF_QB_BATCH 12
 #endif
 enum { XF_DEAL_ROUNDS = 1, XF_DEAL_FULL = 2 };
 #ifndef MV2D_XF_DEAL_DEFAULT
@@ -18,7 +21,14 @@
 
 namespace {
 
-constexpr int WAVE_LDS = 16384;
+template <int XLO, int QB> constexpr bool XF_SLIM = XLO == 2 && QB > 8;
+template <int XLO, int QB> constexpr int WAVE_LDS = XF_SLIM<XLO, QB> ? 12288 : 16384;
+
+template <int XLO, int QB>
+__device__ __forceinline__ int xf_slot(int n) {
+    if constexpr ((QB & (QB - 1)) == 0) return n & (QB - 1);
+    else return n < QB ? n : 0;
+}
 
 template <int XLO, int QB>
 __global__ __launch_bounds__(64 * QB, 2) void xattn_fused_kernel(const float* __restrict__ q, const uint4* __restrict__ WA_hi, const uint4* __restrict__ WA_lo,
@@ -27,11 +37,13 @@
                                                                 const unsigned short* __restrict__ Xk_lo, const unsigned short* __restrict__ Xv_lo,
                                                                 const int* __restrict__ row_ptr, const int* __restrict__ col_idx, float* __restrict__ ctx,
                                                                 int R, int empty_nan, const int* __restrict__ order, int nblk) {
-    constexpr int SMEM = QB * WAVE_LDS + QB * 512 + QB * HEADS * 4 + 3 * QB * 4;
+    constexpr int SMEM = QB * WAVE_LDS<XLO, QB> + QB * 512 + QB * HEADS * 4 + 3 * QB * 4;
     __shared__ __attribute__((aligned(16))) unsigned char smem[SMEM];
-    const int tid = threadIdx.x, lane = tid & 63, wave = tid >> 6, n = lane & 15, g = lane >> 4;
-    float* lsum = reinterpret_cast<float*>(smem + QB * WAVE_LDS + QB * 512);
-    int* rq = reinterpret_cast<int*>(smem + QB * WAVE_LDS + QB * 512 + QB * HEADS * 4);
+    constexpr bool SLIM = XF_SLIM<XLO, QB>;
+    const int tid = threadIdx.x, lane = SLIM ? (int)__lane_id() : tid & 63, wave = SLIM ? __builtin_amdgcn_readfirstlane(tid >> 6) : tid >> 6;
+    const int n = lane & 15, g = lane >> 4;
+    float* lsum = reinterpret_cast<float*>(smem + QB * WAVE_LDS<XLO, QB> + QB * 512);
+    int* rq = reinterpret_cast<int*>(smem + QB * WAVE_LDS<XLO, QB> + QB * 512 + QB * HEADS * 4);
     int* rbeg = rq + QB;
     int* rend = rq + 2 * QB;
     const int blk = xcd_chunked(blockIdx.x, nblk);
@@ -47,50 +59,59 @@
     }
     __syncthreads();
     XF_STAMP(1);
-    const int beg = rbeg[wave], end = rend[wave];
+    const int beg = SLIM ? __builtin_amdgcn_readfirstlane(rbeg[wave]) : rbeg[wave], end = SLIM ? __builtin_amdgcn_readfirstlane(rend[wave]) : rend[wave];
     const int ntile = wave < nq ? (end - beg + 15) >> 4 : 0;
     int idx_next = ntile > 0 ? col_idx[min(beg + n, end - 1)] : 0;
-    typedef XattnWalk<XLO, false> Walk;
-    Walk walk(Xk, Xv, Xk_lo, Xv_lo, lane, beg, end, reinterpret_cast<uint4*>(smem + wave * WAVE_LDS), reinterpret_cast<uint4*>(smem + wave * WAVE_LDS) + 512,
-           reinterpret_cast<float*>(smem + QB * WAVE_LDS) + wave * 128);
+    typedef XattnWalk<XLO, false, XF_SLIM<XLO, QB>> Walk;
+    Walk walk(Xk, Xv, Xk_lo, Xv_lo, lane, beg, end, reinterpret_cast<uint4*>(smem + wave * WAVE_LDS<XLO, QB>), reinterpret_cast<uint4*>(smem + wave * WAVE_LDS<XLO, QB>) + 512,
+           reinterpret_cast<float*>(smem + QB * WAVE_LDS<XLO, QB>) + wave * 128);
     typename Walk::KRows k0;
+    constexpr int NP = QB > 8 ? 2 : 1, TP = 16 / NP, UP = 8 / NP;
+    if (QB > HEADS && wave >= HEADS && ntile > 0) walk.request_k(idx_next, k0);
     for (int h = wave; h < HEADS; h += QB) {
-        const int r = rq[n & (QB - 1)];
+        const int r = rq[xf_slot<XLO, QB>(n)];
         const float* qp = q + (long long)r * C + 32 * h + 8 * g;
         const float4 q0 = *reinterpret_cast<const float4*>(qp), q1 = *reinterpret_cast<const float4*>(qp + 4);
         const uint4* wh = WA_hi + (long long)h * 16 * 64 + lane;
         const uint4* wl = WA_lo + (long long)h * 16 * 64 + lane;
-        uint4* qt = reinterpret_cast<uint4*>(smem + (n & (QB - 1)) * WAVE_LDS) + h * 64;
-        u32x4 wa_h[16], wa_l[16];
-#pragma unroll
-        for (int t = 0; t < 16; ++t) {
-            wa_h[t] = *reinterpret_cast<const u32x4*>(wh + t * 64);
-            wa_l[t] = *reinterpret_cast<const u32x4*>(wl + t * 64);
-        }
-        __builtin_amdgcn_sched_barrier(0);
-        XF_STAMP(20);
+        uint4* qt = reinterpret_cast<uint4*>(smem + xf_slot<XLO, QB>(n) * WAVE_LDS<XLO, QB>) + h * 64;
         Frag bh, bl;
-        split8(q0, q1, bh, bl);
-#pragma unroll
-        for (int u = 0; u < 8; ++u) {
-            if (u == 1) XF_STAMP(21);
-            if (u == 4) XF_STAMP(22);
-            f32x4_t a[2];
-#pragma unroll
-            for (int k = 0; k < 2; ++k) {
-                f32x4_t c = {0.f, 0.f, 0.f, 0.f};
-                c = mfma_q16_16x16x32(wa_l[2 * u + k], bh.v, c);
-                c = mfma_q16_16x16x32(wa_h[2 * u + k], bl.v, c);
-                c = mfma_q16_16x16x32(wa_h[2 * u + k], bh.v, c);
-                a[k] = c;
-            }
-            Frag hi, lo;
-            split8_k16(make_float4(a[0][0], a[0][1], a[0][2], a[0][3]), make_float4(a[1][0], a[1][1], a[1][2], a[1][3]), hi, lo);
-            if (n < QB) {
-                qt[u * 8 + g * 2] = hi.u;
-                qt[u * 8 + g * 2 + 1] = lo.u;
-            }
-            if (u == (XLO ? 5 : 3) && h == wave && ntile > 0) walk.request_k(idx_next, k0);
+#pragma unroll
+        for (int part = 0; part < NP; ++part) {
+            u32x4 wa_h[TP], wa_l[TP];
+#pragma unroll
+            for (int t = 0; t < TP; ++t) {
+                wa_h[t] = *reinterpret_cast<const u32x4*>(wh + (part * TP + t) * 64);
+                wa_l[t] = *reinterpret_cast<const u32x4*>(wl + (part * TP + t) * 64);
+            }
+            __builtin_amdgcn_sched_barrier(0);
+            if (part == 0) {
+                XF_STAMP(20);
+                split8(q0, q1, bh, bl);
+            }
+#pragma unroll
+            for (int uu = 0; uu < UP; ++uu) {
+                const int u = part * UP + uu;
+                if (u == 1) XF_STAMP(21);
+                if (u == 4) XF_STAMP(22);
+                f32x4_t a[2];
+#pragma unroll
+                for (int k = 0; k < 2; ++k) {
+                    f32x4_t c = {0.f, 0.f, 0.f, 0.f};
+                    c = mfma_q16_16x16x32(wa_l[2 * uu + k], bh.v, c);
+                    c = mfma_q16_16x16x32(wa_h[2 * uu + k], bl.v, c);
+                    c = mfma_q16_16x16x32(wa_h[2 * uu + k], bh.v, c);
+                    a[k] = c;
+                }
+                Frag hi, lo;
+                split8_k16(make_float4(a[0][0], a[0][1], a[0][2], a[0][3]), make_float4(a[1][0], a[1][1], a[1][2], a[1][3]), hi, lo);
+                if (n < QB) {
+                    qt[u * 8 + g * 2] = hi.u;
+                    qt[u * 8 + g * 2 + 1] = lo.u;
+                }
+                if (u == (XLO ? 5 : 3) && h == wave && ntile > 0) walk.request_k(idx_next, k0);
+            }
+            if (NP > 1) __builtin_amdgcn_sched_barrier(0);
         }
     }
     XF_STAMP(23);
@@ -98,7 +119,8 @@
     __builtin_amdgcn_s_barrier();
     XF_STAMP(2);
     {
-        const uint4* qp = reinterpret_cast<const uint4*>(smem + wave * WAVE_LDS) + (n & 7) * 64 + g * 2 + (n >> 3);
+        const int nb = SLIM ? walk.n : n, gb = SLIM ? walk.g : g;
+        const uint4* qp = reinterpret_cast<const uint4*>(smem + wave * WAVE_LDS<XLO, QB>) + (nb & 7) * 64 + gb * 2 + (nb >> 3);
 #pragma unroll
         for (int s = 0; s < 8; ++s) walk.qa[s].u = qp[s * 8];
     }
@@ -107,69 +129,78 @@
 #pragma nounroll
     for (int tt = 0; tt < ntile; ++tt) {
         const int myidx = idx_next;
-        if (tt + 1 < ntile) idx_next = col_idx[min(beg + 16 * (tt + 1) + n, end - 1)];
+        if (tt + 1 < ntile) idx_next = col_idx[min(beg + 16 * (tt + 1) + (SLIM ? walk.n : n), end - 1)];
         typename Walk::VRows v;
         walk.gather(myidx, tt > 0, v);
         XF_STAMP(3 + 2 * min(tt, 5));
-        walk.compute(tt, v);
+        walk.compute(tt, v, myidx);
         XF_STAMP(4 + 2 * min(tt, 5));
     }
     walk.row_sums();
-    if (n == 0 && g < 2) {
-#pragma unroll
-        for (int i = 0; i < 4; ++i) lsum[wave * HEADS + 4 * g + i] = walk.l_run[i];
-    }
-    walk.store_z(reinterpret_cast<float*>(smem + wave * WAVE_LDS));
+    {
+        const int nb = SLIM ? walk.n : n, gb = SLIM ? walk.g : g;
+        if (nb == 0 && gb < 2) {
+#pragma unroll
+            for (int i = 0; i < 4; ++i) lsum[wave * HEADS + 4 * gb + i] = walk.l_run[i];
+        }
+    }
+    walk.store_z(reinterpret_cast<float*>(smem + wave * WAVE_LDS<XLO, QB>));
     XF_STAMP(15);
     __syncthreads();
     XF_STAMP(16);
+    const int lc = SLIM ? Walk::fresh(walk.lane) : lane, nc = SLIM ? lc & 15 : n, gc = SLIM ? lc >> 4 : g;
     for (int h = wave; h < HEADS; h += QB) {
-        const int j = n & (QB - 1);
-        const float* zp = reinterpret_cast<const float*>(smem + j * WAVE_LDS) + h * C + 8 * g;
+        const int j = xf_slot<XLO, QB>(nc);
+        const float* zp = reinterpret_cast<const float*>(smem + j * WAVE_LDS<XLO, QB>) + h * C + 8 * gc;
         const float rl = __builtin_amdgcn_rcpf(lsum[j * HEADS + h]);
-        const uint4* wh = WB_hi + (long long)h * 16 * 64 + lane;
-        const uint4* wl = WB_lo + (long long)h * 16 * 64 + lane;
+        const uint4* wh = WB_hi + (long long)h * 16 * 64 + lc;
+        const uint4* wl = WB_lo + (long long)h * 16 * 64 + lc;
         f32x4_t acc[2] = {{0.f, 0.f, 0.f, 0.f}, {0.f, 0.f, 0.f, 0.f}};
-        u32x4 wb_h[16], wb_l[16];
-#pragma unroll
-        for (int t = 0; t < 16; ++t) {
-            wb_h[t] = *reinterpret_cast<const u32x4*>(wh + t * 64);
-            wb_l[t] = *reinterpret_cast<const u32x4*>(wl + t * 64);
-        }
         int rr_[4], rp0_[4], rp1_[4];
 #pragma unroll
         for (int i = 0; i < 4; ++i) {
-            rr_[i] = rq[(4 * g + i) & (QB - 1)];
-            rp0_[i] = rbeg[(4 * g + i) & (QB - 1)];
-            rp1_[i] = rend[(4 * g + i) & (QB - 1)];
-        }
-        const float bv0 = bv[32 * h + n], bv1 = bv[32 * h + 16 + n];
-        __builtin_amdgcn_sched_barrier(0);
-#pragma unroll
-        for (int s = 0; s < 8; ++s) {
-            float4 x0 = *reinterpret_cast<const float4*>(zp + 32 * s);
-            float4 x1 = *reinterpret_cast<const float4*>(zp + 32 * s + 4);
-            x0 = make_float4(x0.x * rl, x0.y * rl, x0.z * rl, x0.w * rl);
-            x1 = make_float4(x1.x * rl, x1.y * rl, x1.z * rl, x1.w * rl);
-            Frag ah, al;
-            split8(x0, x1, ah, al);
-#pragma unroll
-            for (int nt = 0; nt < 2; ++nt) {
-                acc[nt] = mfma_q16_16x16x32(al.v, wb_h[s * 2 + nt], acc[nt]);
-                acc[nt] = mfma_q16_16x16x32(ah.v, wb_l[s * 2 + nt], acc[nt]);
-                acc[nt] = mfma_q16_16x16x32(ah.v, wb_h[s * 2 + nt], acc[nt]);
-            }
-        }
-        if (4 * g < QB) {
+            rr_[i] = rq[xf_slot<XLO, QB>(4 * gc + i)];
+            rp0_[i] = rbeg[xf_slot<XLO, QB>(4 * gc + i)];
+            rp1_[i] = rend[xf_slot<XLO, QB>(4 * gc + i)];
+        }
+        const float bv0 = bv[32 * h + nc], bv1 = bv[32 * h + 16 + nc];
+#pragma unroll
+        for (int part = 0; part < NP; ++part) {
+            u32x4 wb_h[TP], wb_l[TP];
+#pragma unroll
+            for (int t = 0; t < TP; ++t) {
+                wb_h[t] = *reinterpret_cast<const u32x4*>(wh + (part * TP + t) * 64);
+                wb_l[t] = *reinterpret_cast<const u32x4*>(wl + (part * TP + t) * 64);
+            }
+            __builtin_amdgcn_sched_barrier(0);
+#pragma unroll
+            for (int ss = 0; ss < UP; ++ss) {
+                const int s = part * UP + ss;
+                float4 x0 = *reinterpret_cast<const float4*>(zp + 32 * s);
+                float4 x1 = *reinterpret_cast<const float4*>(zp + 32 * s + 4);
+                x0 = make_float4(x0.x * rl, x0.y * rl, x0.z * rl, x0.w * rl);
+                x1 = make_float4(x1.x * rl, x1.y * rl, x1.z * rl, x1.w * rl);
+                Frag ah, al;
+                split8(x0, x1, ah, al);
+#pragma unroll
+                for (int nt = 0; nt < 2; ++nt) {
+                    acc[nt] = mfma_q16_16x16x32(al.v, wb_h[ss * 2 + nt], acc[nt]);
+                    acc[nt] = mfma_q16_16x16x32(ah.v, wb_l[ss * 2 + nt], acc[nt]);
+                    acc[nt] = mfma_q16_16x16x32(ah.v, wb_h[ss * 2 + nt], acc[nt]);
+                }
+            }
+            if (NP > 1) __builtin_amdgcn_sched_barrier(0);
+        }
+        if (4 * gc < QB) {
 #pragma unroll
             for (int i = 0; i < 4; ++i) {
-                const int js = 4 * g + i;
+                const int js = 4 * gc + i;
                 if (js < nq) {
                     const int rr = rr_[i];
                     const bool empty = rp1_[i] <= rp0_[i];
 #pragma unroll
                     for (int nt = 0; nt < 2; ++nt) {
-                        const int col = 32 * h + 16 * nt + n;
+                        const int col = 32 * h + 16 * nt + nc;
                         float v = acc[nt][i] + (nt ? bv1 : bv0);
                         if (empty) v = empty_nan ? __uint_as_float(0x7fc00000u) : 0.f;
                         ctx[(long long)rr * C + col] = v;
@@ -187,10 +218,11 @@
 extern "C" int mv2d_xf_trace_read(long long* host, int n) { return hipMemcpyFromSymbol(host, HIP_SYMBOL(g_xf_trace), n * sizeof(long long)) == hipSuccess ? 0 : -2; }
 #endif
 
-extern "C" int mv2d_xattn_fused_fwd_p(const float* q, const void* WA_hi, const void* WA_lo, const void* WB_hi, const void* WB_lo, const float* bv,
+extern "C" int mv2d_xattn_fused_fwd_q(const float* q, const void* WA_hi, const void* WA_lo, const void* WB_hi, const void* WB_lo, const float* bv,
                                       const void* Xk, const void* Xv, const void* Xk_lo, const void* Xv_lo, const int* row_ptr, const int* col_idx,
-                                      float* ctx, int R, int empty_nan, const int* order, int lo_fmt, int deal, void* stream) {
-    MV2D_CHECK_ARG(deal >= 0 && deal <= 2, "mv2d_xattn_fused_fwd_p: deal is 0 (default), 1 (whole rounds) or 2 (full blocks)");
+                                      float* ctx, int R, int empty_nan, const int* order, int lo_fmt, int deal, int qb, void* stream) {
+    MV2D_CHECK_ARG(deal >= 0 && deal <= 2, "mv2d_xattn_fused_fwd_q: deal is 0 (default), 1 (whole rounds) or 2 (full blocks)");
+    MV2D_CHECK_ARG(qb == 0 || qb == 4 || qb == 8 || (qb == 12 && Xk_lo && lo_fmt == 1), "mv2d_xattn_fused_fwd_q: qb is 0 (default), 4 or 8, or 12 with e4m3 lo rows");
     MV2D_CHECK_ARG(lo_fmt == 0 || (lo_fmt == 1 && Xk_lo), "mv2d_xattn_fused_fwd: lo_fmt is 0 (key16 lo rows) or 1 (e4m3 lo rows; needs the lo rows)");
     MV2D_CHECK_ARG(q && WA_hi && WA_lo && WB_hi && WB_lo && bv && Xk && Xv && row_ptr && col_idx && ctx && R >= 0, "mv2d_xattn_fused_fwd: bad args");
     MV2D_CHECK_ARG((Xk_lo == nullptr) == (Xv_lo == nullptr), "mv2d_xattn_fused_fwd: Xk_lo and Xv_lo come together");
@@ -205,7 +237,9 @@
         n_cu = (hipGetDevice(&dev) == hipSuccess && hipGetDeviceProperties(&prop, dev) == hipSuccess && prop.multiProcessorCount > 0) ? prop.multiProcessorCount : 256;
     }
     static const int qb_env = [] { const char* e = getenv("MV2D_XF_QB"); return e ? atoi(e) : 0; }();
-    const int QB = qb_env == 4 || qb_env == 8 ? qb_env : MV2D_XF_QB_DEFAULT;
+    const bool lo8 = Xk_lo && lo_fmt == 1;
+    int QB = qb ? qb : (qb_env == 4 || qb_env == 8 || (qb_env == 12 && lo8) ? qb_env : 0);
+    if (QB == 0) QB = lo8 && (R + MV2D_XF_QB_DEFAULT - 1) / MV2D_XF_QB_DEFAULT > n_cu ? MV2D_XF_QB_BATCH : MV2D_XF_QB_DEFAULT;
     const int slots = n_cu * (QB == 4 ? 2 : 1);
     int nblk = (R + QB - 1) / QB;
     if (nblk > slots) {
@@ -223,7 +257,7 @@
 #define MV2D_XF(XLO_, QB_) hipLaunchKernelGGL((xattn_fused_kernel<XLO_, QB_>), grid, block, 0, (hipStream_t)stream, q, (const uint4*)WA_hi, (const uint4*)WA_lo, \
                                               (const uint4*)WB_hi, (const uint4*)WB_lo, bv, (const unsigned short*)Xk, (const unsigned short*)Xv,                     \
                                               (const unsigned short*)Xk_lo, (const unsigned short*)Xv_lo, row_ptr, col_idx, ctx, R, empty_nan, order, nblk)
-    if (Xk_lo && lo_fmt == 1) { if (QB == 4) MV2D_XF(2, 4); else MV2D_XF(2, 8); }
+    if (lo8) { if (QB == 4) MV2D_XF(2, 4); else if (QB == 12) MV2D_XF(2, 12); else MV2D_XF(2, 8); }
     else if (Xk_lo) { if (QB == 4) MV2D_XF(1, 4); else MV2D_XF(1, 8); }
     else { if (QB == 4) MV2D_XF(0, 4); else MV2D_XF(0, 8); }
 #undef MV2D_XF
@@ -231,6 +265,12 @@
     return MV2D_OK;
 }
 
+extern "C" int mv2d_xattn_fused_fwd_p(const float* q, const void* WA_hi, const void* WA_lo, const void* WB_hi, const void* WB_lo, const float* bv,
+                                      const void* Xk, const void* Xv, const void* Xk_lo, const void* Xv_lo, const int* row_ptr, const int* col_idx,
+                                      float* ctx, int R, int empty_nan, const int* order, int lo_fmt, int deal, void* stream) {
+    return mv2d_xattn_fused_fwd_q(q, WA_hi, WA_lo, WB_hi, WB_lo, bv, Xk, Xv, Xk_lo, Xv_lo, row_ptr, col_idx, ctx, R, empty_nan, order, lo_fmt, deal, 0, stream);
+}
+
 extern "C" int mv2d_xattn_fused_fwd(const float* q, const void* WA_hi, const void* WA_lo, const void* WB_hi, const void* WB_lo, const float* bv,
                                     const void* Xk, const void* Xv, const void* Xk_lo, const void* Xv_lo, const int* row_ptr, const int* col_idx,
                                     float* ctx, int R, int empty_nan, const int* order, int lo_fmt, void* stream) {
diff --git a/mv2d_amd/csrc/xattn_walk.h b/mv2d_amd/csrc/xattn_walk.h
--- a/mv2d_amd/csrc/xattn_walk.h
+++ b/mv2d_amd/csrc/xattn_walk.h
@@ -41,14 +41,16 @@
     return v;
 }
 
-template <int XLO, bool DBG>
+template <int XLO, bool DBG, bool LO8B = false>
 struct XattnWalk {
+    static_assert(!LO8B || XLO == 2, "LO8B: the e4m3 lo rows only");
     typedef std::conditional_t<XLO == 2, u32x2, u32x4> lo_t;
     struct KRows { u32x4 hi[8]; lo_t lo[XLO ? 8 : 1]; };
     struct VRows { u32x4 hi[4][2]; lo_t lo[XLO ? 4 : 1][2]; };
 
     const unsigned short *Xk, *Xv, *Xk_lo, *Xv_lo;
-    int lane, n, g, beg, end;
+    int lane, n, g;
+    int beg, end;
     uint4 *kt, *kt2;
     float* pl;
     float* dbg_logits;
@@ -63,6 +65,20 @@
         : Xk(Xk_), Xv(Xv_), Xk_lo(Xk_lo_), Xv_lo(Xv_lo_), lane(lane_), n(lane_ & 15), g(lane_ >> 4), beg(beg_), end(end_), kt(kt_), kt2(kt2_), pl(pl_),
           dbg_logits(dbg_logits_), dbg_stride(dbg_stride_) {}
 
+    __device__ __forceinline__ static int fresh(int x) {
+        if constexpr (LO8B) asm volatile("" : "+v"(x));
+        return x;
+    }
+    __device__ __forceinline__ static int shfl(int v, int src) {
+        if constexpr (LO8B) return __builtin_amdgcn_ds_bpermute(src << 2, v);
+        else return __shfl(v, src, 64);
+    }
+    __device__ __forceinline__ void relane() {
+        lane = fresh(lane);
+        n = lane & 15;
+        g = lane >> 4;
+    }
+
     __device__ __forceinline__ void reset() {
 #pragma unroll
         for (int i = 0; i < 4; ++i) { m_run[i] = -INFINITY; l_run[i] = 0.f; }
@@ -73,7 +89,7 @@
     __device__ __forceinline__ void load_v(const unsigned short* V_, int myidx, u32x4 (&dst)[4][2]) const {
 #pragma unroll
         for (int e = 0; e < 4; ++e) {
-            const unsigned int vidx = (unsigned int)__shfl(myidx, 4 * g + e, 64);
+            const unsigned int vidx = (unsigned int)shfl(myidx, 4 * g + e);
             const char* vp = reinterpret_cast<const char*>(V_) + ((vidx << 9) + 16u * (unsigned)n);
             dst[e][0] = *reinterpret_cast<const u32x4*>(vp);
             dst[e][1] = *reinterpret_cast<const u32x4*>(vp + 256);
@@ -82,7 +98,7 @@
     __device__ __forceinline__ void load_k(const unsigned short* K_, int myidx, u32x4 (&dst)[8]) const {
 #pragma unroll
         for (int i = 0; i < 8; ++i) {
-            const unsigned int ridx = (unsigned int)__shfl(myidx, 2 * i + (lane >> 5), 64);
+            const unsigned int ridx = (unsigned int)shfl(myidx, 2 * i + (lane >> 5));
             dst[i] = *reinterpret_cast<const u32x4*>(reinterpret_cast<const char*>(K_) + ((ridx << 9) + (unsigned)(lane & 31) * 16u));
         }
     }
@@ -96,7 +112,7 @@
     __device__ __forceinline__ void load_v8(const unsigned short* V_, int myidx, u32x2 (&dst)[4][2]) const {
 #pragma unroll
         for (int e = 0; e < 4; ++e) {
-            const unsigned int vidx = (unsigned int)__shfl(myidx, 4 * g + e, 64);
+            const unsigned int vidx = (unsigned int)shfl(myidx, 4 * g + e);
             const char* vp = reinterpret_cast<const char*>(V_) + ((vidx << 8) + 8u * (unsigned)n);
             dst[e][0] = *reinterpret_cast<const u32x2*>(vp);
             dst[e][1] = *reinterpret_cast<const u32x2*>(vp + 128);
@@ -105,7 +121,7 @@
     __device__ __forceinline__ void load_k8(const unsigned short* K_, int myidx, u32x2 (&dst)[8]) const {
 #pragma unroll
         for (int i = 0; i < 8; ++i) {
-            const unsigned int ridx = (unsigned int)__shfl(myidx, 2 * i + (lane >> 5), 64);
+            const unsigned int ridx = (unsigned int)shfl(myidx, 2 * i + (lane >> 5));
             dst[i] = *reinterpret_cast<const u32x2*>(reinterpret_cast<const char*>(K_) + ((ridx << 8) + (unsigned)(lane & 31) * 8u));
         }
     }
@@ -113,17 +129,22 @@
 #pragma unroll
         for (int i = 0; i < 8; ++i) {
             const int rowi = 2 * i + (lane >> 5);
-            tile[rowi * 32 + ((lane & 31) ^ (rowi & 15))] = lo8_chunk(make_uint2(src[i].x, src[i].y));
-        }
-    }
-    __device__ __forceinline__ void request_k(int myidx, KRows& k) const {
+            if constexpr (LO8B) reinterpret_cast<u32x2*>(tile)[rowi * 32 + ((lane & 31) ^ (2 * rowi))] = src[i];
+            else tile[rowi * 32 + ((lane & 31) ^ (rowi & 15))] = lo8_chunk(make_uint2(src[i].x, src[i].y));
+        }
+    }
+    __device__ __forceinline__ void request_k(int myidx, KRows& k) {
+        if constexpr (LO8B) relane();
         load_k(Xk, myidx, k.hi);
         if constexpr (XLO == 1) load_k(Xk_lo, myidx, k.lo);
+        if constexpr (LO8B) relane();
         if constexpr (XLO == 2) load_k8(Xk_lo, myidx, k.lo);
     }
-    __device__ __forceinline__ void stage_k(const KRows& k) const {
+    __device__ __forceinline__ void stage_k(const KRows& k) {
+        if constexpr (LO8B) relane();
         store_k(kt, k.hi);
         if constexpr (XLO == 1) store_k(kt2, k.lo);
+        if constexpr (LO8B) relane();
         if constexpr (XLO == 2) store_k8(kt2, k.lo);
     }
     __device__ __forceinline__ void request_v(int myidx, VRows& v) const {
@@ -132,14 +153,19 @@
         if constexpr (XLO == 2) load_v8(Xv_lo, myidx, v.lo);
     }
 
-    __device__ __forceinline__ void gather(int myidx, bool with_k, VRows& v) const {
+    __device__ __forceinline__ void gather(int myidx, bool with_k, VRows& v) {
         if constexpr (XLO != 0) {
             if (with_k) {
                 KRows k;
                 request_k(myidx, k);
                 stage_k(k);
             }
-            request_v(myidx, v);
+            if constexpr (LO8B) {
+                relane();
+                load_v(Xv, myidx, v.hi);
+            } else {
+                request_v(myidx, v);
+            }
         } else if (with_k) {
             KRows k;
             request_k(myidx, k);
@@ -151,8 +177,9 @@
         __builtin_amdgcn_wave_barrier();
     }
 
-    __device__ __forceinline__ void compute(int tt, const VRows& v) {
+    __device__ __forceinline__ void compute(int tt, VRows& v, int myidx = 0) {
         const int kbase = beg + 16 * tt;
+        if constexpr (LO8B) relane();
         f32x4_t sacc = {0.f, 0.f, 0.f, 0.f};
 #pragma unroll
         for (int s = 0; s < 8; ++s) {
@@ -161,10 +188,17 @@
             sacc = mfma_k16_16x16x32(qa[s].u, kb.u, sacc);
             if (XLO) {
                 Frag kl, qh;
-                kl.u = kt2[n * 32 + ((4 * s + g) ^ n)];
+                if constexpr (LO8B) kl.u = lo8_chunk(reinterpret_cast<const uint2*>(kt2)[n * 32 + ((4 * s + g) ^ (2 * n))]);
+                else kl.u = kt2[n * 32 + ((4 * s + g) ^ n)];
                 qh.u = n < 8 ? qa[s].u : make_uint4(0u, 0u, 0u, 0u);
                 sacc = mfma_k16_16x16x32(qh.u, kl.u, sacc);
             }
+        }
+        if constexpr (LO8B) {
+            __builtin_amdgcn_sched_barrier(0);
+            relane();
+            load_v8(Xv_lo, myidx, v.lo);
+            __builtin_amdgcn_sched_barrier(0);
         }
         const bool valid = kbase + n < end;
         float sv[4], p[4], alpha[4];
@@ -230,12 +264,24 @@
                     zc = mfma_k16_16x16x16(pah, vl, zc);
                 }
                 Z[H * 8 + w] = zc;
+                if constexpr (LO8B) { if (w & 1) __builtin_amdgcn_sched_barrier(0); }
             }
         }
         __builtin_amdgcn_wave_barrier();
     }
 
     __device__ __forceinline__ void row_sums() {
+        if constexpr (LO8B) {
+            relane();
+#pragma unroll
+            for (int i = 0; i < 4; ++i) {
+                float l = l_run[i];
+#pragma unroll
+                for (int m = 1; m < 16; m *= 2) l += __int_as_float(__builtin_amdgcn_ds_bpermute((lane ^ m) << 2, __float_as_int(l)));
+                l_run[i] = l;
+            }
+            return;
+        }
 #pragma unroll
         for (int i = 0; i < 4; ++i) {
             float l = l_run[i];
diff --git a/mv2d_amd/engine.py b/mv2d_amd/engine.py
--- a/mv2d_amd/engine.py
+++ b/mv2d_amd/engine.py
@@ -919,7 +919,7 @@
                 if rt.grouped:
                     o.xattn_group(ws['q'], mapA, mapB, bv, xk_rows, xv_rows, ws['row_ptr'], ws['grp_tab'], out=ws['ctx'], R=R, **rows)
                 elif rt.xattn_fused:
-                    o.xattn_fused(ws['q'], mapA, mapB, bv, xk_rows, xv_rows, ws['row_ptr'], ws['col_idx'], out=ws['ctx'], R=R, deal=rt.xattn_deal, **rows)
+                    o.xattn_fused(ws['q'], mapA, mapB, bv, xk_rows, xv_rows, ws['row_ptr'], ws['col_idx'], out=ws['ctx'], R=R, deal=rt.xattn_deal, qb=rt.xattn_qb or None, **rows)
                 else:
                     o.xattn_qmap(ws['q'], mapA, ws['Qt'], R=R)
                     tile_attn(i)
diff --git a/mv2d_amd/ops.py b/mv2d_amd/ops.py
--- a/mv2d_amd/ops.py
+++ b/mv2d_amd/ops.py
@@ -918,7 +918,7 @@
     return out
 
 
-def xattn_fused(q, WA, WB, bv, Xk, Xv, row_ptr, col_idx, out=None, R=None, empty_nan=True, Xk_lo=None, Xv_lo=None, order=None, deal=0):
+def xattn_fused(q, WA, WB, bv, Xk, Xv, row_ptr, col_idx, out=None, R=None, empty_nan=True, Xk_lo=None, Xv_lo=None, order=None, deal=0, qb=None):
     _req(q, torch.float32, 'q'); _req(bv, torch.float32, 'bv'); _req(row_ptr, torch.int32, 'row_ptr'); _req(col_idx, torch.int32, 'col_idx')
     for t, n_ in ((WA[0], 'WA_hi'), (WA[1], 'WA_lo'), (WB[0], 'WB_hi'), (WB[1], 'WB_lo')):
         _req(t, q16_dtype(), n_)
@@ -928,9 +928,9 @@
     if out is None:
         out = torch.empty((R, 256), device=q.device, dtype=torch.float32)
     _req(out, torch.float32, 'out')
-    check(_lib.load().mv2d_xattn_fused_fwd_p(_p(q), _p(WA[0]), _p(WA[1]), _p(WB[0]), _p(WB[1]), _p(bv), _p(Xk), _p(Xv), _p(Xk_lo), _p(Xv_lo), _p(row_ptr),
-                                             _p(col_idx), _p(out), R, 1 if empty_nan else 0, _p(order), lo_fmt, int(deal), _stream()),
-          'mv2d_xattn_fused_fwd_p')
+    check(_lib.load().mv2d_xattn_fused_fwd_q(_p(q), _p(WA[0]), _p(WA[1]), _p(WB[0]), _p(WB[1]), _p(bv), _p(Xk), _p(Xv), _p(Xk_lo), _p(Xv_lo), _p(row_ptr),
+                                             _p(col_idx), _p(out), R, 1 if empty_nan else 0, _p(order), lo_fmt, int(deal), int(qb or 0), _stream()),
+          'mv2d_xattn_fused_fwd_q')
     return out
 
 
diff --git a/mv2d_amd/route.py b/mv2d_amd/route.py
--- a/mv2d_amd/route.py
+++ b/mv2d_amd/route.py
@@ -14,7 +14,8 @@
         exact_skip=frozenset({'conv'}), lo8_rows=True, pe_at_positions=env('MV2D_PE_AT_POS', '1') != '0', pe_rows_in_waves=False,
         ablate_zero_lo=frozenset(), keep_sine_rows=False, stop_before_decoder=False, force_nc=None, debug_attn=False,
         fuse_qg_tail=env('MV2D_QG_TAIL', '1') != '0', pe_cache=env('MV2D_PE_CACHE', '1') != '0', pe_cache_views=env('MV2D_PE_CACHE_VIEWS', '0') == '1',
-        xattn_deal=0)
+        xattn_deal=0,
+        xattn_qb=0)
 
 
 OPTIONS = tuple(default_options())
@@ -52,6 +53,7 @@
     pe_cache: bool
     pe_cache_views: bool
     xattn_deal: int
+    xattn_qb: int
 
     @property
     def storage(self):
@@ -89,6 +91,8 @@
     assert not (debug and use_graph), 'debug_attn: eager runs only'
     if int(o.xattn_deal) not in (0, 1, 2):
         raise ValueError('mv2d engine: xattn_deal is 0 (the library\'s policy), 1 (whole rounds) or 2 (full blocks)')
+    if int(o.xattn_qb) not in (0, 4, 8, 12):
+        raise ValueError('mv2d engine: xattn_qb is 0 (the library\'s choice), 4, 8 or 12')
     pe_pos = kind == 'S' and exact and bool(o.pe_at_positions)
     pe_opt = lambda key, shipped: (pe_options or {}).get(key, shipped)
     pe_cache_ok = (pe_x3 and bool(pe_opt('with_fpe', True)) and not pe_opt('no_sin_enc', False) and not stages and not o.keep_sine_rows
@@ -106,4 +110,4 @@
         last_stage_heads=bool(o.last_stage_heads) and not stages, debug_attn=debug, stop_before_decoder=bool(o.stop_before_decoder),
         force_nc=o.force_nc, ablate_zero_lo=frozenset(o.ablate_zero_lo) if exact else frozenset(),
         qg_tail_fused=bool(o.fuse_qg_tail) and not stages, pe_cache=pe_cache, pe_cache_views=pe_cache_views,
-        xattn_deal=int(o.xattn_deal))
+        xattn_deal=int(o.xattn_deal), xattn_qb=int(o.xattn_qb))
```

After: 11100 samples/s (median of 6 runs). 1.02x the previous value.
